# moxime/joint-vae

Measured on AMD Instinct MI355X. Metric: training_images_per_sec, higher is better.
Workload: dtype f32

## Files before the change

### include/jvae_hip.h

```cpp
#ifndef JVAE_HIP_H
#define JVAE_HIP_H

#include <stddef.h>

#ifdef __cplusplus
extern "C" {
#endif

const char* jvae_version(void);

int jvae_gemm_f32(int M, int N, int K, int batch,
                  const float* A, long sAm, long sAk, long sAb,
                  const float* B, long sBk, long sBn, long sBb,
                  float* C, long sCm, long sCn, long sCb,
                  const float* bias, int bias_mode, int flags, int splitk, void* stream);

int jvae_splitk_fold_f32(const float* part, const float* bias, float* y, int S, long MN, int N, int relu, int accumulate,
                         void* stream);

typedef struct JvaeGemmDesc {
    int M, N, K, batch;
    const float* A; long sAm, sAk, sAb;
    const float* B; long sBk, sBn, sBb;
    float* C; long sCm, sCn, sCb;
    const float* bias; int bias_mode, flags, splitk;
    int want_splits; long sCsplit; int* splits;
} JvaeGemmDesc;
int jvae_gemm_group_f32(const JvaeGemmDesc* descs, int n, void* stream);

typedef struct JvaeGemmRoute {
    int variant;
    int gx, gy, gz;
    int slices, kchunk;
    int vecA, vecB;
    int lds;
} JvaeGemmRoute;
int jvae_gemm_route(const JvaeGemmDesc* d, JvaeGemmRoute* out);
const char* jvae_gemm_variant_name(int variant);

typedef struct JvaeFoldDesc {
    const float* part; const float* bias; float* y;
    int S; long MN; int N, relu, accumulate;
} JvaeFoldDesc;
int jvae_splitk_fold_group_f32(const JvaeFoldDesc* descs, int n, void* stream);

size_t jvae_conv2d_workspace_bytes(int N, int Cin, int H, int W, int Cout, int KH, int KW, int S, int P, int OP,
                                   int transposed);
int jvae_conv2d_set_split_bf16(int mode);
int jvae_conv2d_set_split_shape16(int on);
int jvae_conv2d_out_shape(int H, int W, int KH, int KW, int S, int P, int OP, int transposed, int* OH, int* OW);
int jvae_conv2d_route(int dir, int layout, int bias, int stats, int y_f32, int aff_kind,
                      int N, int Cin, int H, int W, int Cout, int KH, int KW, int S, int P, int OP, int transposed,
                      int* kernel, int* swap, size_t* ws_bytes, int* splits, int* aff_ok);
const char* jvae_conv2d_kernel_name(int kernel);
int jvae_conv2d_fwd_f32(const float* x, const float* w, const float* bias, float* y,
                        int N, int Cin, int H, int W, int Cout, int KH, int KW, int S, int P, int OP, int transposed,
                        void* ws, size_t ws_bytes, void* stream);
int jvae_conv2d_stats_splits(int N, int Cin, int H, int W, int Cout, int KH, int KW, int S, int P, int OP, int transposed);
int jvae_conv2d_fwd_stats_f32(const float* x, const float* w, const float* bias, float* y, float* stats, int* nsplit,
                              int N, int Cin, int H, int W, int Cout, int KH, int KW, int S, int P, int OP, int transposed,
                              void* ws, size_t ws_bytes, void* stream);
int jvae_conv2d_dgrad_f32(const float* dy, const float* w, float* dx,
                          int N, int Cin, int H, int W, int Cout, int KH, int KW, int S, int P, int OP, int transposed,
                          void* ws, size_t ws_bytes, void* stream);
int jvae_conv2d_wgrad_f32(const float* x, const float* dy, float* dw, float* dbias, int accumulate,
                          int N, int Cin, int H, int W, int Cout, int KH, int KW, int S, int P, int OP, int transposed,
                          void* ws, size_t ws_bytes, void* stream);

int jvae_pack_cache_configure(void* buf, size_t bytes);
int jvae_pack_cache_begin(void* stream, long long owner, const void* const* weights, int n);
int jvae_pack_cache_end(void);
int jvae_pack_cache_pin(void);
int jvae_pack_cache_reset(void);
int jvae_pack_cache_stats(int* entries, long long* hits, long long* misses, long long* refreshes);

size_t jvae_channel_sum_workspace_bytes(int C);
int jvae_channel_sum_f32(const float* t, float* out, int N, int C, int P, int accumulate, void* ws, size_t ws_bytes,
                         void* stream);

size_t jvae_bn_workspace_bytes(int C);
int jvae_bn_plan(int N, int C, int P, int* nsplit, int* nchunk);
int jvae_image_range(int N, int parts, int j, int* nb, int* ne);
int jvae_bn_fwd_f32(const float* x, const float* gamma, const float* beta,
                    float* running_mean, float* running_var, long long* num_batches_tracked,
                    float* y, float* save_mean, float* save_invstd,
                    int N, int C, int P, float momentum, float eps, int training, int relu,
                    void* ws, size_t ws_bytes, void* stream);
int jvae_bn_fwd_ext_f32(const float* x, const float* gamma, const float* beta,
                        float* running_mean, float* running_var, long long* num_batches_tracked,
                        float* y, float* save_mean, float* save_invstd,
                        int N, int C, int P, float momentum, float eps, int training, int relu,
                        const float* ext_stats, int ext_nsplit, const float* ext_pivot,
                        void* ws, size_t ws_bytes, void* stream);
int jvae_bn_bwd_f32(const float* dy, const float* x, const float* gamma, const float* beta,
                    const float* save_mean, const float* save_invstd,
                    float* dx, float* dgamma, float* dbeta, int accumulate,
                    int N, int C, int P, int relu, void* ws, size_t ws_bytes, void* stream);
int jvae_bn_eval_bwd_f32(const float* dy, const float* x, const float* gamma, const float* beta,
                         const float* running_mean, const float* running_var, float* dx,
                         int N, int C, int P, float eps, int relu, void* stream);

int jvae_bn_finalize_f32(const float* x, const float* gamma, const float* beta,
                         float* running_mean, float* running_var, long long* num_batches_tracked,
                         float* save_mean, float* save_invstd, float* scale, float* shift,
                         int N, int C, int P, float momentum, float eps, int training,
                         const float* ext_stats, int ext_nsplit, const float* ext_pivot,
                         void* ws, size_t ws_bytes, void* stream);
int jvae_conv2d_affine_ok(int N, int Cin, int H, int W, int Cout, int KH, int KW, int S, int P, int OP, int transposed);
int jvae_conv2d_fwd_aff_f32(const float* x, const float* w, const float* bias, float* y, float* stats, int* nsplit,
                            const float* in_scale, const float* in_shift, int in_relu,
                            int N, int Cin, int H, int W, int Cout, int KH, int KW, int S, int P, int OP, int transposed,
                            void* ws, size_t ws_bytes, void* stream);
int jvae_conv2d_wgrad_aff_f32(const float* x, const float* dy, float* dw, float* dbias, int accumulate,
                              const float* in_scale, const float* in_shift, int in_relu,
                              int N, int Cin, int H, int W, int Cout, int KH, int KW, int S, int P, int OP, int transposed,
                              void* ws, size_t ws_bytes, void* stream);

int jvae_bn_sums_f32(const float* x, const float* pivot, float* sums, int N, int C, int P,
                     void* ws, size_t ws_bytes, void* stream);
int jvae_bn_fwd_sync_f32(const float* x, const float* gamma, const float* beta,
                         float* running_mean, float* running_var, long long* num_batches_tracked,
                         float* y, float* save_mean, float* save_invstd,
                         int N, int C, int P, float momentum, float eps, int relu,
                         const float* global_sums, const float* pivot, int world,
                         void* ws, size_t ws_bytes, void* stream);
int jvae_bn_bwd_sums_f32(const float* dy, const float* x, const float* gamma, const float* beta,
                         const float* save_mean, const float* save_invstd, float* local_sums,
                         int N, int C, int P, int relu, void* ws, size_t ws_bytes, void* stream);
int jvae_bn_bwd_sync_f32(const float* dy, const float* x, const float* gamma, const float* beta,
                         const float* save_mean, const float* save_invstd,
                         const float* local_sums, const float* global_sums, int world,
                         float* dx, float* dgamma, float* dbeta, int accumulate,
                         int N, int C, int P, int relu, void* stream);

int jvae_b8_pack_f32(const float* x, void* y, int N, int C, long HW, void* stream);
int jvae_b8_unpack_f32(const void* y, float* x, int N, int C, long HW, int accumulate, void* stream);
int jvae_conv2d_native_b8(int N, int Cin, int H, int W, int Cout, int KH, int KW, int S, int P, int OP, int transposed);
size_t jvae_conv2d_workspace_bytes_b8(int N, int Cin, int H, int W, int Cout, int KH, int KW, int S, int P, int OP,
                                      int transposed);
int jvae_conv2d_stats_splits_b8(int N, int Cin, int H, int W, int Cout, int KH, int KW, int S, int P, int OP, int transposed);
int jvae_conv2d_fwd_b8(const void* x, const float* w, const float* bias, void* y, int y_f32, float* stats, int* nsplit,
                       int N, int Cin, int H, int W, int Cout, int KH, int KW, int S, int P, int OP, int transposed,
                       void* ws, size_t ws_bytes, void* stream);
int jvae_conv2d_dgrad_b8(const void* dy, const float* w, void* dx,
                         int N, int Cin, int H, int W, int Cout, int KH, int KW, int S, int P, int OP, int transposed,
                         void* ws, size_t ws_bytes, void* stream);
int jvae_conv2d_wgrad_b8(const void* x, const void* dy, float* dw, float* dbias, int accumulate,
                         int N, int Cin, int H, int W, int Cout, int KH, int KW, int S, int P, int OP, int transposed,
                         void* ws, size_t ws_bytes, void* stream);
size_t jvae_bn_workspace_bytes_b8(int C);
int jvae_bn_plan_b8(int N, int C, long HW, int* nsplit, int* nchunk);
int jvae_bn_fwd_b8(const void* x, const float* gamma, const float* beta,
                   float* running_mean, float* running_var, long long* num_batches_tracked,
                   void* y, float* save_mean, float* save_invstd,
                   int N, int C, long HW, float momentum, float eps, int training, int relu,
                   const float* ext_stats, int ext_nsplit, const float* ext_pivot,
                   void* ws, size_t ws_bytes, void* stream);
int jvae_bn_bwd_b8(const void* dy, const void* x, const float* gamma, const float* beta,
                   const float* save_mean, const float* save_invstd,
                   void* dx, float* dgamma, float* dbeta, int accumulate,
                   int N, int C, long HW, int relu, void* ws, size_t ws_bytes, void* stream);
int jvae_bn_finalize_b8(const void* x, const float* gamma, const float* beta,
                        float* running_mean, float* running_var, long long* num_batches_tracked,
                        float* save_mean, float* save_invstd, float* coef,
                        int N, int C, long HW, float momentum, float eps, int training,
                        const float* ext_stats, int ext_nsplit, const float* ext_pivot,
                        void* ws, size_t ws_bytes, void* stream);
int jvae_bn_sums_b8(const void* x, const float* pivot, float* sums, int N, int C, long HW,
                    void* ws, size_t ws_bytes, void* stream);
int jvae_bn_fwd_sync_b8(const void* x, const float* gamma, const float* beta,
                        float* running_mean, float* running_var, long long* num_batches_tracked,
                        void* y, float* save_mean, float* save_invstd,
                        int N, int C, long HW, float momentum, float eps, int relu,
                        const float* global_sums, const float* pivot, int world,
                        void* ws, size_t ws_bytes, void* stream);
int jvae_bn_bwd_sums_b8(const void* dy, const void* x, const float* gamma, const float* beta,
                        const float* save_mean, const float* save_invstd, float* local_sums,
                        int N, int C, long HW, int relu, void* ws, size_t ws_bytes, void* stream);
int jvae_bn_bwd_sync_b8(const void* dy, const void* x, const float* gamma, const float* beta,
                        const float* save_mean, const float* save_invstd,
                        const float* local_sums, const float* global_sums, int world,
                        void* dx, float* dgamma, float* dbeta, int accumulate,
                        int N, int C, long HW, int relu, void* ws, size_t ws_bytes, void* stream);
int jvae_conv2d_affine_ok_b8(int N, int Cin, int H, int W, int Cout, int KH, int KW, int S, int P, int OP, int transposed);
int jvae_conv2d_fwd_aff_b8(const void* x, const float* w, const float* bias, void* y, int y_f32, float* stats, int* nsplit,
                           const float* in_scale, const float* in_shift, int in_relu,
                           int N, int Cin, int H, int W, int Cout, int KH, int KW, int S, int P, int OP, int transposed,
                           void* ws, size_t ws_bytes, void* stream);
int jvae_conv2d_wgrad_aff_b8(const void* x, const void* dy, float* dw, float* dbias, int accumulate,
                             const float* in_scale, const float* in_shift, int in_relu,
                             int N, int Cin, int H, int W, int Cout, int KH, int KW, int S, int P, int OP, int transposed,
                             void* ws, size_t ws_bytes, void* stream);
int jvae_relu_fwd_b8(const void* x, void* y, long units, void* stream);
int jvae_relu_bwd_b8(const void* dy, const void* y, void* dx, long units, void* stream);

int jvae_act_fwd_f32(const float* x, float* y, long n, int kind, void* stream);
int jvae_act_bwd_f32(const float* dy, const float* y, float* dx, long n, int kind, void* stream);

int jvae_dict_stats_f32(const float* means, float* dict, int C, int K, void* stream);
int jvae_latent_fwd_f32(const float* mu, const float* lv_raw, const float* eps, const long long* y,
                        const float* means, const float* T, const float* dict,
                        float* lv, float* z, float* kl, float* zdist, float* var_kl, float* dzdist,
                        int N, int K, int L, int C, int prior, int var_dim, float tau, float alpha, float w,
                        int sampled, int has_forced, float forced_lv, void* stream);
int jvae_latent_bwd_f32(const float* mu, const float* lv_raw, const float* lv, const float* eps, const long long* y,
                        const float* means, const float* T,
                        const float* gz, const float* g_kl, const float* g_zdist, const float* g_vkl,
                        const float* gmu_direct, const float* glv_direct,
                        float* gmu, float* glv_raw, float* gmeans, float* gT,
                        int N, int K, int L, int C, int prior, int var_dim, float tau, float alpha, float w,
                        int sampled, int has_forced, void* ws, size_t ws_bytes, void* stream);
int jvae_latent_fwd_wdev_f32(const float* mu, const float* lv_raw, const float* eps, const long long* y,
                             const float* means, const float* T, const float* dict,
                             float* lv, float* z, float* kl, float* zdist, float* var_kl, float* dzdist,
                             int N, int K, int L, int C, int prior, int var_dim, float tau, float alpha, float w,
                             int sampled, int has_forced, float forced_lv, const float* w_dev, void* stream);
int jvae_latent_bwd_wdev_f32(const float* mu, const float* lv_raw, const float* lv, const float* eps, const long long* y,
                             const float* means, const float* T,
                             const float* gz, const float* g_kl, const float* g_zdist, const float* g_vkl,
                             const float* gmu_direct, const float* glv_direct,
                             float* gmu, float* glv_raw, float* gmeans, float* gT,
                             int N, int K, int L, int C, int prior, int var_dim, float tau, float alpha, float w,
                             int sampled, int has_forced, const float* w_dev, void* ws, size_t ws_bytes, void* stream);
int jvae_latent_mixed_fwd_f32(const float* mu, const float* lv_raw, const float* eps, const long long* y,
                              const float* means_a, const float* T_a, const float* dict, const float* means_b, const float* T_b,
                              float* lv, float* z, float* kl, float* zdist, float* var_kl, float* dzdist,
                              int N, int K, int L, int split,
                              int C_a, int prior_a, int var_dim_a, float tau_a, float alpha_a,
                              int C_b, int prior_b, int var_dim_b, float tau_b, float alpha_b,
                              float w, int sampled, int has_forced, float forced_lv, void* stream);
int jvae_latent_mixed_bwd_f32(const float* mu, const float* lv_raw, const float* lv, const float* eps, const long long* y,
                              const float* means_a, const float* T_a, const float* means_b, const float* T_b,
                              const float* gz, const float* g_kl, const float* g_zdist, const float* g_vkl,
                              const float* gmu_direct, const float* glv_direct,
                              float* gmu, float* glv_raw, float* gmeans, float* gT,
                              int N, int K, int L, int split,
                              int C_a, int prior_a, int var_dim_a, float tau_a, float alpha_a,
                              int C_b, int prior_b, int var_dim_b, float tau_b, float alpha_b,
                              float w, int sampled, int has_forced, void* ws, size_t ws_bytes, void* stream);
int jvae_latent_refine_f32(float* mu, float* lv_raw, float* lv, const float* eps_cur, const float* eps_next,
                           const long long* y, const float* means, const float* T, const float* dz,
                           float* m_mu, float* v_mu, float* m_lv, float* v_lv,
                           float* z_next, float* kl, float* zdist, float* var_kl,
                           int N, int K, int L, int C, int prior, int var_dim, float tau, float alpha,
                           int sampled, int has_forced, float forced_lv, float lr, long step, int flags, void* stream);

int jvae_recon_fwd_f32(const float* x_reco, const float* x, const float* sigma, int sigma_is_log,
                       float* wmse, int L, int N, int D, void* stream);
int jvae_recon_bwd_f32(const float* x_reco, const float* x, const float* sigma, int sigma_is_log, const float* sigma_fwd,
                       const float* g_wmse, const float* wmse, float* g_x_reco, float* gsigma, int accumulate_sigma,
                       int L, int N, int D, void* ws, size_t ws_bytes, void* stream);

int jvae_mse_rows_fwd_f32(const float* rows, const float* x, float* wmse, int L, int N, int D, void* stream);
int jvae_mse_rows_bwd_f32(const float* rows, const float* x, const float* g_wmse, float* g_rows, int L, int N, int D, void* stream);

int jvae_elbo_fwd_f32(const float* wmse_s, const float* kl, const float* ce, const float* sigma, int sigma_is_log,
                      float* wmse, float* cross_x, float* total, float* mse, int L, int N, int D, float beta, float cw,
                      void* stream);
int jvae_elbo_bwd_f32(const float* g_wmse, const float* g_cx, const float* g_tot, const float* sigma, int sigma_is_log,
                      float* g_wmse_s, float* g_kl, float* g_ce, float* gsigma, int accumulate_sigma,
                      int L, int N, int D, float beta, float cw, void* ws, size_t ws_bytes, void* stream);
int jvae_elbo_fwd_wdev_f32(const float* wmse_s, const float* kl, const float* ce, const float* sigma, int sigma_is_log,
                           float* wmse, float* cross_x, float* total, float* mse, int L, int N, int D, float beta, float cw,
                           const float* cw_dev, void* stream);
int jvae_elbo_bwd_wdev_f32(const float* g_wmse, const float* g_cx, const float* g_tot, const float* sigma, int sigma_is_log,
                           float* g_wmse_s, float* g_kl, float* g_ce, float* gsigma, int accumulate_sigma,
                           int L, int N, int D, float beta, float cw, const float* cw_dev, void* ws, size_t ws_bytes,
                           void* stream);

int jvae_dropout_f32(const float* x, float* y, long n, float p, long seed, void* stream);
int jvae_dropout_dev_f32(const float* x, float* y, long n, float p, const long long* seed_dev, long salt, void* stream);

int jvae_iws_f32(const float* wmse_s, const float* eps, const float* log_var, const float* log_pz, const float* sigma,
                 int sigma_is_log, int L, int N, int K, int C, int D, float* rows, float* iws, void* stream);

int jvae_measures_f32(const float* sumsq_x, long nx, const float* wmse, const float* zdist, const float* var_kl, int N, int Nz,
                      const float* sigma, int sigma_is_log, const float* means, int C, int K, const int* flag,
                      const float* prev, int batch, float* out, void* stream);
int jvae_measures_dev_f32(const float* sumsq_x, long nx, const float* wmse, const float* zdist, const float* var_kl, int N, int Nz,
                          const float* sigma, int sigma_is_log, const float* means, int C, int K, const int* flag,
                          float* run, int* counter, void* stream);

int jvae_loss_sums_f32(const float* const* rows, const long* lens, int nrows, float* acc, void* stream);

int jvae_xent_fwd_f32(const float* logits, const long long* y, float* ce, int R, int N, int C, void* stream);
int jvae_xent_bwd_f32(const float* logits, const long long* y, const float* g_ce, float* g_logits, int R, int N, int C,
                      void* stream);

size_t jvae_sqnorm_workspace_bytes(void);
int jvae_sqnorm_accum_f32(const float* g, long n, float* acc, int reset, void* ws, size_t ws_bytes, void* stream);
int jvae_clip_scale_f32(float* g, long n, const float* sqnorm, float max_norm, void* stream);
int jvae_adam_step_f32(float* p, const float* g, float* m, float* v, long n,
                       float lr, float beta1, float beta2, float eps, float weight_decay, long step,
                       float max_norm, const float* sqnorm, int* nonfinite_flag, void* stream);
int jvae_adam_step_dev_f32(float* p, const float* g, float* m, float* v, long n, float* hyper, int advance,
                           float eps, float weight_decay, float max_norm, const float* sqnorm, int* nonfinite_flag,
                           void* stream);

int jvae_sgd_step_f32(float* p, const float* g, float* buf, long n, float lr, float momentum, int nesterov,
                      float weight_decay, int first_step, float max_norm, const float* sqnorm, int* nonfinite_flag,
                      void* stream);

int jvae_pool2d_out_shape(int H, int W, int K, int S, int P, int* OH, int* OW);
int jvae_pool2d_fwd_f32(const float* x, float* y, int* idx, long planes, int H, int W, int K, int S, int P, int mode,
                        void* stream);
int jvae_pool2d_bwd_f32(const float* dy, const int* idx, float* dx, long planes, int H, int W, int K, int S, int P,
                        int mode, void* stream);
int jvae_upsample_nearest_fwd_f32(const float* x, float* y, long planes, int H, int W, int scale, void* stream);
int jvae_upsample_nearest_bwd_f32(const float* dy, float* dx, long planes, int H, int W, int scale, void* stream);
int jvae_pool2d_fwd_b8(const void* x, void* y, int* idx, long blocks, int H, int W, int K, int S, int P, int mode, void* stream);
int jvae_pool2d_bwd_b8(const void* dy, const int* idx, void* dx, long blocks, int H, int W, int K, int S, int P, int mode,
                       void* stream);
int jvae_upsample_nearest_fwd_b8(const void* x, void* y, long blocks, int H, int W, int scale, void* stream);
int jvae_upsample_nearest_bwd_b8(const void* dy, void* dx, long blocks, int H, int W, int scale, void* stream);

int jvae_augment_u8_f32(const unsigned char* in, const unsigned char* flip, const int* dy, const int* dx,
                        float* out, int N, int C, int H, int W, int pad, int nhwc, void* stream);

int jvae_imageset_desc_words(void);
int jvae_imageset_batch_u8_f32(const unsigned char* data, const long long* idx, const long long* targets, const long long* lut,
                               const int* desc, const int* coef_h, const int* bounds_h, const int* coef_v, const int* bounds_v,
                               const unsigned char* flip, const int* dy, const int* dx, float* x, long long* y, long n, int N,
                               void* stream);

int jvae_imageset_mix_leaf_bytes(void);
int jvae_imageset_mixed_u8_f32(const void* leaves_host, const void* leaves_dev, int n_leaves, const int* leaf,
                               const long long* index, const long long* tag, const long long* pos, const float* u, int u_dims,
                               float* x, long long* tagout, long long* y, int N, int vec, void* stream);

size_t jvae_roc_workspace_bytes(int M, long n_in, long n_out);
int jvae_roc_curve_f32(const float* ins, const float* outs, const double* kept_tpr, const int* two_sided,
                       double* auc, double* kept_fpr, double* kept_tpr_out, double* thr_low, double* thr_up, int* status,
                       int M, long n_in, long n_out, int K, void* ws, size_t ws_bytes, void* stream);

size_t jvae_pr_workspace_bytes(int M, long n_in, long n_out);
int jvae_pr_metrics_f32(const float* ins, const float* outs, const int* modes, double* figures, int* status,
                        int M, long n_in, long n_out, void* ws, size_t ws_bytes, void* stream);

int jvae_scod_scores_f32(const float* const* r_src, const float* const* r_aux, const float* const* g_src,
                         const float* const* g_alt, const int* kinds, const float* weights, const long long* y_est,
                         float* out, long out_stride, int M, int C, long N, int* status, void* stream);
size_t jvae_scod_workspace_bytes(int M, long n);
int jvae_scod_curve_f32(const float* scores, const long long* y_true, const long long* y_est, float* curves, double* figures,
                        int* status, int M, long n, long n_in, void* ws, size_t ws_bytes, void* stream);

int jvae_misclass_scores_f32(const float* src, const int* kinds, const float* temps, const int* rows, float* out,
                             int R, int C, long N, long out_stride, void* stream);
size_t jvae_misclass_split_workspace_bytes(long N);
int jvae_misclass_split_f32(const float* scores, const unsigned char* mask, float* out, int* n_correct, int M, long N,
                            void* ws, size_t ws_bytes, void* stream);
int jvae_misclass_confusion_f32(const float* scores, const unsigned char* mask, const double* thr, int* tp, int* fp,
                                int M, long N, int K, void* stream);

int jvae_odin_head_f32(const float* logits, const float* temps, float* scores, float* dlogits,
                       int F, int L, int N, int C, long stride_f, long stride_l, void* stream);
int jvae_odin_perturb_f32(float* acc, const float* g, const float* x, const float* eps, float* out, long numel, int E,
                          void* stream);

int jvae_wim_scores_f32(const float* const* srcs, const float* const* alts, const float* factors, int S, const long long* y_est,
                        const int* specs, int R, float* out, long out_stride, int C, long N, int* status, void* stream);
int jvae_group_tally_f32(const float* values, const int* group, double* sums, long long* counts, int R, int N, int G,
                         void* stream);

int jvae_prior_sample_f32(const float* eps, const long long* y, const float* means, const float* T, float* z, int* status,
                          long R, int K, int C, float t, int mode, void* stream);
int jvae_image_grid_f32(const float* x_in, const float* x_out, const int* specs, const int* specs_host, int Ncol, float* grid_f32,
                        unsigned char* grid_u8, int N, int D, int H, int W, int Rr, void* stream);

int jvae_class_posterior_f32(const float* z, const float* means, const float* T, const float* log_det, const float* temps, int nT,
                             float* logp, float* P, long R, int K, int C, int var_dim, void* stream);
size_t jvae_latent_mi_workspace_bytes(int nT, int L0, long N);
int jvae_latent_mi_f32(const float* P0, const float* P1, float* Im, int nT, int C, int L0, int L1, long N, void* ws, size_t ws_bytes,
                       void* stream);
int jvae_aggregate_scores_f32(const void* const* srcs, const float* factors, int E, int mode, const float* temps, int nT, float* post,
                              float* a, float* amax, long long* argmax, int slot, int C, long N, int* status, void* stream);

size_t jvae_cascade_mse_workspace_bytes(int M, long N, long D);
int jvae_cascade_mse_f32(const float* x, const void* const* stages, int M, float* mse, int L, long N, long D, void* ws,
                         size_t ws_bytes, void* stream);
// ... 98 lines not shown
```

### joint-vae_amd/csrc/conv_api.hip

```cpp
#include "common.h"
#include "jvae_internal.h"
#include "conv_dispatch.h"

namespace {

inline ConvRoute route(const ConvGeom& g, int transposed, ConvDir dir, CallFlags f = {}) {
    return jvae_conv_route(g, transposed, dir, CONV_F32, f);
}

bool affine_ok(const ConvGeom& g, int transposed, ConvDir other, const ConvRoute& r) {
    return r.aff_ok && route(g, transposed, other, {false, false, false, 1}).aff_ok;
}

int fwd_f32(const float* x, const float* w, const float* bias, float* y, float* stats, int* nsplit, const InAff* aff,
            int N, int Cin, int H, int W, int Cout, int KH, int KW, int S, int P, int OP, int transposed,
            void* ws, size_t ws_bytes, void* stream) {
    ConvGeom g; int oh, ow;
    if (nsplit) *nsplit = 0;
    if (!jvae_make_geom(N, Cin, H, W, Cout, KH, KW, S, P, OP, transposed, &g, &oh, &ow)) return JVAE_EINVAL;
    const ConvRoute r = route(g, transposed, CONV_FWD, {bias != nullptr, stats != nullptr, false, jvae_aff_kind(aff)});
    if (aff && !affine_ok(g, transposed, CONV_WGRAD, r)) return JVAE_ENOTSUP;
    if (N == 0) return 0;
    if (jvae_ws_short(r, ws, ws_bytes)) return JVAE_EWORKSPACE;
    return jvae_conv_run_fwd(r, g, x, w, bias, y, (float*)ws, ws_bytes, (hipStream_t)stream, stats, nsplit, aff);
}

int wgrad_f32(const float* x, const float* dy, float* dw, float* dbias, int accumulate, const InAff* aff,
              int N, int Cin, int H, int W, int Cout, int KH, int KW, int S, int P, int OP, int transposed,
              void* ws, size_t ws_bytes, void* stream) {
    ConvGeom g; int oh, ow;
    if (!dw || (N > 0 && (!x || !dy))) return JVAE_EINVAL;
    if (!jvae_make_geom(N, Cin, H, W, Cout, KH, KW, S, P, OP, transposed, &g, &oh, &ow)) return JVAE_EINVAL;
    const ConvRoute r = route(g, transposed, CONV_WGRAD, {false, false, false, jvae_aff_kind(aff)});
    if (aff && !affine_ok(g, transposed, CONV_FWD, r)) return JVAE_ENOTSUP;
    if (N > 0 && jvae_ws_short(r, ws, ws_bytes)) return JVAE_EWORKSPACE;
    hipStream_t st = (hipStream_t)stream;
    if (!accumulate) {
        hipError_t e = hipMemsetAsync(dw, 0, sizeof(float) * (size_t)Cin * Cout * KH * KW, st);
        if (e != hipSuccess) return (int)e;
    }
    if (N == 0) {
        if (dbias && !accumulate) {
            hipError_t e = hipMemsetAsync(dbias, 0, sizeof(float) * (size_t)Cout, st);
            if (e != hipSuccess) return (int)e;
        }
        return 0;
    }
    int rc = jvae_conv_run_wgrad(r, g, transposed, x, dy, dw, (float*)ws, ws_bytes, st, aff);
    if (rc) return rc;
    if (dbias) rc = jvae_channel_sum(dy, dbias, N, Cout, oh * ow, accumulate, (float*)ws, ws_bytes, st);
    return rc;
}

}

extern "C" {

int jvae_conv2d_set_split_bf16(int mode) { return jvae_conv5_x3_set(mode); }
int jvae_conv2d_set_split_shape16(int on) { return jvae_conv5_x3_set_shape16(on); }

size_t jvae_conv2d_workspace_bytes(int N, int Cin, int H, int W, int Cout, int KH, int KW, int S, int P, int OP,
                                   int transposed) {
    ConvGeom g; int oh, ow;
    if (!jvae_make_geom(N, Cin, H, W, Cout, KH, KW, S, P, OP, transposed, &g, &oh, &ow)) return 0;
    return jvae_conv_ws(g, transposed);
}

int jvae_conv2d_route(int dir, int layout, int bias, int stats, int y_f32, int aff_kind,
                      int N, int Cin, int H, int W, int Cout, int KH, int KW, int S, int P, int OP, int transposed,
                      int* kernel, int* swap, size_t* ws_bytes, int* splits, int* aff_ok) {
    ConvGeom g; int oh, ow;
    if (dir != CONV_FWD && dir != CONV_DGRAD && dir != CONV_WGRAD) return JVAE_EINVAL;
    if ((layout != CONV_F32 && layout != CONV_B8) || aff_kind < 0 || aff_kind > 2) return JVAE_EINVAL;
    if (!jvae_make_geom(N, Cin, H, W, Cout, KH, KW, S, P, OP, transposed, &g, &oh, &ow)) return JVAE_EINVAL;
    const ConvRoute r = jvae_conv_route(g, transposed, (ConvDir)dir, (ConvLayout)layout,
                                        {bias != 0, stats != 0, y_f32 != 0, aff_kind});
    if (kernel) *kernel = (int)r.k;
    if (swap) *swap = r.swap ? 1 : 0;
    if (ws_bytes) *ws_bytes = r.ws;
    if (splits) *splits = r.splits;
    if (aff_ok) *aff_ok = r.aff_ok ? 1 : 0;
    return 0;
}

const char* jvae_conv2d_kernel_name(int kernel) {
    switch (kernel) {
#define JVAE_CK_NAME(k) case k: return #k;
        JVAE_CK_NAME(CK_NONE) JVAE_CK_NAME(CK_GENERIC) JVAE_CK_NAME(CK_POINT) JVAE_CK_NAME(CK_SMALLCO)
        JVAE_CK_NAME(CK_SMALLCI) JVAE_CK_NAME(CK_FWD5) JVAE_CK_NAME(CK_FWD5_X3) JVAE_CK_NAME(CK_T2) JVAE_CK_NAME(CK_T2_X3)
        JVAE_CK_NAME(CK_WG5) JVAE_CK_NAME(CK_WG5_X3) JVAE_CK_NAME(CK_B8) JVAE_CK_NAME(CK_T2_B8) JVAE_CK_NAME(CK_WG_B8)
        JVAE_CK_NAME(CK_WG_B8X) JVAE_CK_NAME(CK_SMALLCO_DG)
#undef JVAE_CK_NAME
        default: return nullptr;
    }
}

int jvae_conv2d_out_shape(int H, int W, int KH, int KW, int S, int P, int OP, int transposed, int* OH, int* OW) {
    ConvGeom g;
    if (!OH || !OW) return JVAE_EINVAL;
    return jvae_make_geom(1, 1, H, W, 1, KH, KW, S, P, OP, transposed, &g, OH, OW) ? 0 : JVAE_EINVAL;
}

int jvae_conv2d_fwd_f32(const float* x, const float* w, const float* bias, float* y,
                        int N, int Cin, int H, int W, int Cout, int KH, int KW, int S, int P, int OP, int transposed,
                        void* ws, size_t ws_bytes, void* stream) {
    if (!w || (N > 0 && (!x || !y))) return JVAE_EINVAL;
    return fwd_f32(x, w, bias, y, nullptr, nullptr, nullptr, N, Cin, H, W, Cout, KH, KW, S, P, OP, transposed, ws, ws_bytes,
                   stream);
}

int jvae_conv2d_stats_splits(int N, int Cin, int H, int W, int Cout, int KH, int KW, int S, int P, int OP, int transposed) {
    ConvGeom g; int oh, ow;
    if (!jvae_make_geom(N, Cin, H, W, Cout, KH, KW, S, P, OP, transposed, &g, &oh, &ow)) return 0;
    return route(g, transposed, CONV_FWD, {false, true, false, 0}).splits;
}

int jvae_conv2d_fwd_stats_f32(const float* x, const float* w, const float* bias, float* y, float* stats, int* nsplit,
                              int N, int Cin, int H, int W, int Cout, int KH, int KW, int S, int P, int OP, int transposed,
                              void* ws, size_t ws_bytes, void* stream) {
    if (!w || !nsplit || (N > 0 && (!x || !y))) return JVAE_EINVAL;
    return fwd_f32(x, w, bias, y, stats, nsplit, nullptr, N, Cin, H, W, Cout, KH, KW, S, P, OP, transposed, ws, ws_bytes, stream);
}

int jvae_conv2d_affine_ok(int N, int Cin, int H, int W, int Cout, int KH, int KW, int S, int P, int OP, int transposed) {
    ConvGeom g; int oh, ow;
    if (!jvae_make_geom(N, Cin, H, W, Cout, KH, KW, S, P, OP, transposed, &g, &oh, &ow)) return 0;
    return affine_ok(g, transposed, CONV_WGRAD, route(g, transposed, CONV_FWD, {false, false, false, 1})) ? 1 : 0;
}

int jvae_conv2d_fwd_aff_f32(const float* x, const float* w, const float* bias, float* y, float* stats, int* nsplit,
                            const float* in_scale, const float* in_shift, int in_relu,
                            int N, int Cin, int H, int W, int Cout, int KH, int KW, int S, int P, int OP, int transposed,
                            void* ws, size_t ws_bytes, void* stream) {
    if (!w || !in_scale || !in_shift || (N > 0 && (!x || !y))) return JVAE_EINVAL;
    if (stats && !nsplit) return JVAE_EINVAL;
    const InAff aff{in_scale, in_shift, in_relu};
    return fwd_f32(x, w, bias, y, stats, nsplit, &aff, N, Cin, H, W, Cout, KH, KW, S, P, OP, transposed, ws, ws_bytes, stream);
}

int jvae_conv2d_wgrad_aff_f32(const float* x, const float* dy, float* dw, float* dbias, int accumulate,
                              const float* in_scale, const float* in_shift, int in_relu,
                              int N, int Cin, int H, int W, int Cout, int KH, int KW, int S, int P, int OP, int transposed,
                              void* ws, size_t ws_bytes, void* stream) {
    if (!in_scale || !in_shift) return JVAE_EINVAL;
    const InAff aff{in_scale, in_shift, in_relu};
    return wgrad_f32(x, dy, dw, dbias, accumulate, &aff, N, Cin, H, W, Cout, KH, KW, S, P, OP, transposed, ws, ws_bytes, stream);
}

int jvae_conv2d_dgrad_f32(const float* dy, const float* w, float* dx,
                          int N, int Cin, int H, int W, int Cout, int KH, int KW, int S, int P, int OP, int transposed,
                          void* ws, size_t ws_bytes, void* stream) {
    ConvGeom g; int oh, ow;
    if (!w || (N > 0 && (!dy || !dx))) return JVAE_EINVAL;
    if (!jvae_make_geom(N, Cin, H, W, Cout, KH, KW, S, P, OP, transposed, &g, &oh, &ow)) return JVAE_EINVAL;
    if (N == 0) return 0;
    const ConvRoute r = route(g, transposed, CONV_DGRAD);
    if (jvae_ws_short(r, ws, ws_bytes)) return JVAE_EWORKSPACE;
    return jvae_conv_run_fwd(r, g, dy, w, nullptr, dx, (float*)ws, ws_bytes, (hipStream_t)stream);
}

int jvae_conv2d_wgrad_f32(const float* x, const float* dy, float* dw, float* dbias, int accumulate,
                          int N, int Cin, int H, int W, int Cout, int KH, int KW, int S, int P, int OP, int transposed,
                          void* ws, size_t ws_bytes, void* stream) {
    return wgrad_f32(x, dy, dw, dbias, accumulate, nullptr, N, Cin, H, W, Cout, KH, KW, S, P, OP, transposed, ws, ws_bytes, stream);
}

size_t jvae_channel_sum_workspace_bytes(int C) { return jvae_channel_sum_ws_bytes(C); }

int jvae_channel_sum_f32(const float* t, float* out, int N, int C, int P, int accumulate, void* ws, size_t ws_bytes,
                         void* stream) {
    if (!t || !out || N < 0 || C <= 0 || P <= 0) return JVAE_EINVAL;
    return jvae_channel_sum(t, out, N, C, P, accumulate, (float*)ws, ws_bytes, (hipStream_t)stream);
}

}
```

### joint-vae_amd/csrc/conv_dispatch.h

```cpp
#pragma once
#include "common.h"
#include "jvae_internal.h"

size_t jvae_conv_generic_ws(const ConvGeom& g);
int jvae_fold_fwd(const ConvGeom& g, const float* xb, const float* w, const float* bias, float* ys,
                  float* ws, size_t ws_bytes, hipStream_t st);
int jvae_fold_bwd(const ConvGeom& g, const float* ys, const float* w, const float* bias, float* xb,
                  float* ws, size_t ws_bytes, hipStream_t st);
int jvae_fold_wgrad(const ConvGeom& g, const float* xb, const float* ys, float* dw,
                    float* ws, size_t ws_bytes, hipStream_t st);
size_t jvae_channel_sum_ws_bytes(int C);
int jvae_channel_sum(const float* t, float* out, int N, int C, int P, int accumulate, float* ws, size_t ws_bytes,
                     hipStream_t st);

bool jvae_conv5_fwd_ok(int Cin, int H, int W, int Cout, int OH, int OW, int S, int P);
size_t jvae_conv5_pack_floats(int Cin, int Cout);
int jvae_conv5_fwd(const float* in, const float* w, int swap, int flip, const float* bias, float* out,
                   int N, int Cin, int H, int W, int Cout, int OW, int S, int P, float* ws, hipStream_t st,
                   float* stats = nullptr, int* nsplit = nullptr, const InAff* aff = nullptr);
int jvae_conv5_fwd_max_splits(int N, int OW);

int jvae_conv5_pack(const float* w, float* wp, int C, int O, int swap, int flip, hipStream_t st);

bool jvae_conv5_x3_ok(int Cin, int H, int W, int Cout, int OH, int OW, int S, int P);
size_t jvae_conv5_x3_pack_bytes(int Cin, int Cout);
int jvae_conv5_x3_set(int mode);
int jvae_conv5_x3_set_shape16(int on);
bool jvae_conv5_x3_enabled();
int jvae_conv5_x3_wpack(const float* w, float* ws, int C, int O, int swap, int flip, hipStream_t st);
bool jvae_convt2_x3_ok(int N, int C, int WS, int O);
int jvae_convt2_x3(const float* in, const float* w, const float* bias, float* out, int N, int C, int WS, int O, float* ws,
                   hipStream_t st, float* stats = nullptr, int* nsplit = nullptr, const InAff* aff = nullptr);
int jvae_conv5_x3_fwd(const float* in, const float* w, int swap, int flip, const float* bias, float* out,
                      int N, int Cin, int H, int W, int Cout, int OW, int S, int P, float* ws, hipStream_t st,
                      float* stats = nullptr, int* nsplit = nullptr, const InAff* aff = nullptr);

bool jvae_convt2_ok(int C, int HS, int WS, int O, int HB, int WB, int KH, int KW, int S, int P);
int jvae_convt2(const float* in, const float* wpacked, const float* bias, float* out, int N, int C, int WS, int O,
                hipStream_t st, float* stats = nullptr, int* nsplit = nullptr, const InAff* aff = nullptr);

bool jvae_conv5_smallco_ok(int Cin, int H, int W, int Cout, int KH, int KW, int S, int P);
int jvae_conv5_smallco(const float* in, const float* w, const float* bias, float* out, int N, int Cin, int W, int Cout,
                       hipStream_t st, const InAff* aff = nullptr);
int jvae_conv5_smallco_dgrad(const float* dy, const float* w, float* dx, int N, int Cy, int W, int Cx, hipStream_t st);

bool jvae_conv5_smallci_ok(int Cin, int H, int W, int Cout, int OW, int S, int P, bool dgrad_role);
int jvae_conv5_smallci(const float* in, const float* w, int swap, int flip, const float* bias, float* out,
                       int N, int Cin, int W, int Cout, float* ws, hipStream_t st, float* stats = nullptr, int* nsplit = nullptr);

bool jvae_conv5_wgrad_ok(int Ca, int HS, int WS, int Cb, int HB, int WB, int S, int P);
size_t jvae_conv5_wgrad_ws_floats(int N, int Ca, int Cb, int S, int WS);
int jvae_conv5_wgrad(const float* ps, const float* q, float* dw, int accumulate, int swapflip,
                     int N, int Ca, int WS, int Cb, int S, int P, float* ws, hipStream_t st,
                     const InAff* aff_p = nullptr, const InAff* aff_q = nullptr);

bool jvae_conv5_wgrad_x3_ok(int Ca, int HS, int WS, int Cb, int HB, int WB, int S, int P);
size_t jvae_conv5_wgrad_x3_ws_floats(int N, int Ca, int Cb, int S);
int jvae_conv5_wgrad_x3(const float* ps, const float* q, float* dw, int accumulate, int swapflip,
                        int N, int Ca, int WS, int Cb, int S, int P, float* ws, hipStream_t st,
                        const InAff* aff_p = nullptr, const InAff* aff_q = nullptr);

bool jvae_make_geom(int N, int Cin, int H, int W, int Cout, int KH, int KW, int S, int P, int OP, int transposed,
                    ConvGeom* g, int* OH, int* OW);

enum ConvDir { CONV_FWD = 1, CONV_DGRAD = 2, CONV_WGRAD = 4 };
enum ConvLayout { CONV_F32, CONV_B8 };
enum ConvKernel {
    CK_NONE,
    CK_GENERIC, CK_POINT,
    CK_SMALLCO, CK_SMALLCI, CK_FWD5, CK_FWD5_X3, CK_T2, CK_T2_X3, CK_WG5, CK_WG5_X3,
    CK_B8, CK_T2_B8, CK_WG_B8, CK_WG_B8X,
    CK_SMALLCO_DG,
};
struct CallFlags {
    bool bias, stats;
    bool y_f32;
    int aff;
};
struct ConvRoute {
    ConvKernel k;
    bool swap;
    int S, P;
    size_t ws;
    int splits;
    bool aff_ok;
};
ConvRoute jvae_conv_route(const ConvGeom& g, int transposed, ConvDir dir, ConvLayout layout, CallFlags f);
inline int jvae_aff_kind(const InAff* aff) { return !aff ? 0 : (aff->relu == JVAE_ACT_LEAKY ? 2 : 1); }
inline bool jvae_ws_short(const ConvRoute& r, const void* ws, size_t ws_bytes) { return r.ws && (!ws || ws_bytes < r.ws); }
template <class T>
inline void jvae_wgrad_operands(const ConvRoute& r, int transposed, T* x, T* dy, const InAff* aff, T** ps, T** q,
                                const InAff** aff_p, const InAff** aff_q) {
    const bool p_is_x = r.swap != (transposed != 0);
    *ps = p_is_x ? x : dy;
    *q = p_is_x ? dy : x;
    *aff_p = p_is_x ? aff : nullptr;
    *aff_q = p_is_x ? nullptr : aff;
}

size_t jvae_conv_ws(const ConvGeom& g, int transposed);
int jvae_conv_run_fwd(const ConvRoute& r, const ConvGeom& g, const float* in, const float* w, const float* bias, float* out,
                      float* ws, size_t ws_bytes, hipStream_t st, float* stats = nullptr, int* nsplit = nullptr,
                      const InAff* aff = nullptr);
int jvae_conv_run_wgrad(const ConvRoute& r, const ConvGeom& g, int transposed, const float* x, const float* dy, float* dw,
                        float* ws, size_t ws_bytes, hipStream_t st, const InAff* aff = nullptr);
```

### joint-vae_amd/csrc/conv_generic.hip

```cpp
#include "common.h"
#include "jvae_internal.h"

namespace {

__global__ __launch_bounds__(256) void unfold_kernel(const float* __restrict__ xb, float* __restrict__ col,
                                                     ConvGeom g, int n0, int nimg, long sn, long sk, long sq,
                                                     int kfast) {
    const int Kd = g.Cb * g.KH * g.KW, Ps = g.Hs * g.Ws;
    const long total = (long)nimg * Kd * Ps;
    for (long i = (long)blockIdx.x * blockDim.x + threadIdx.x; i < total; i += (long)gridDim.x * blockDim.x) {
        int n, k, q;
        if (kfast) { k = (int)(i % Kd); long r = i / Kd; n = (int)(r % nimg); q = (int)(r / nimg); }
        else       { q = (int)(i % Ps); long r = i / Ps; k = (int)(r % Kd);  n = (int)(r / Kd); }
        const int kw = k % g.KW, kh = (k / g.KW) % g.KH, cb = k / (g.KW * g.KH);
        const int hs = q / g.Ws, ws = q % g.Ws;
        const int hb = hs * g.S + kh - g.P, wb = ws * g.S + kw - g.P;
        float v = 0.f;
        if (hb >= 0 && hb < g.Hb && wb >= 0 && wb < g.Wb)
            v = xb[(((long)(n0 + n) * g.Cb + cb) * g.Hb + hb) * g.Wb + wb];
        col[(long)n * sn + (long)k * sk + (long)q * sq] = v;
    }
}

template <bool KFAST>
__global__ __launch_bounds__(256) void unfold4_kernel(const float* __restrict__ xb, float* __restrict__ col,
                                                      ConvGeom g, int n0, int nimg) {
    const unsigned Kd = g.Cb * g.KH * g.KW, Ps = g.Hs * g.Ws, KK = g.KH * g.KW;
    const unsigned inner4 = (KFAST ? Kd : Ps) / 4;
    const unsigned total = (KFAST ? Ps * (unsigned)nimg : (unsigned)nimg * Kd) * inner4;
    for (unsigned i = blockIdx.x * blockDim.x + threadIdx.x; i < total; i += gridDim.x * blockDim.x) {
        const unsigned row = i / inner4, e4 = (i - row * inner4) * 4;
        unsigned n, k, q;
        if (KFAST) { q = row / nimg; n = row - q * nimg; k = e4; }
        else       { n = row / Kd;   k = row - n * Kd;   q = e4; }
        unsigned cb = k / KK, t = k - cb * KK;
        unsigned kh = t / g.KW, kw = t - kh * g.KW;
        const unsigned hs = q / g.Ws, ws = q - hs * g.Ws;
        const float* src = xb + (long)(n0 + n) * g.Cb * g.Hb * g.Wb;
        f32x4 v;
#pragma unroll
        for (int e = 0; e < 4; ++e) {
            const int hb = (int)(hs * g.S + kh) - g.P;
            const int wb = (int)((KFAST ? ws : ws + e) * g.S + kw) - g.P;
            v[e] = (hb >= 0 && hb < g.Hb && wb >= 0 && wb < g.Wb) ? src[((long)cb * g.Hb + hb) * g.Wb + wb] : 0.f;
            if (KFAST && ++kw == (unsigned)g.KW) { kw = 0; if (++kh == (unsigned)g.KH) { kh = 0; ++cb; } }
        }
        *reinterpret_cast<f32x4*>(col + (long)i * 4) = v;
    }
}

__global__ __launch_bounds__(256) void fold_kernel(const float* __restrict__ col, float* __restrict__ xb,
                                                   const float* __restrict__ bias, ConvGeom g, int n0, int nimg,
                                                   long sn, long sk, long sq) {
    const unsigned total = (unsigned)nimg * g.Cb * g.Hb * g.Wb;
    for (unsigned i = blockIdx.x * blockDim.x + threadIdx.x; i < total; i += gridDim.x * blockDim.x) {
        unsigned r = i / (unsigned)g.Wb;
        const int wb = (int)(i - r * g.Wb);
        unsigned r2 = r / (unsigned)g.Hb;
        const int hb = (int)(r - r2 * g.Hb);
        const int n = (int)(r2 / (unsigned)g.Cb);
        const int cb = (int)(r2 - (unsigned)n * g.Cb);
        float acc = bias ? bias[cb] : 0.f;
        if (g.Hs * g.Ws < g.KH * g.KW) {
            for (int hs = 0; hs < g.Hs; ++hs) {
                const int kh = hb + g.P - hs * g.S;
                if (kh < 0 || kh >= g.KH) continue;
                for (int ws = 0; ws < g.Ws; ++ws) {
                    const int kw = wb + g.P - ws * g.S;
                    if (kw < 0 || kw >= g.KW) continue;
                    const int k = (cb * g.KH + kh) * g.KW + kw;
                    acc += col[(long)n * sn + (long)k * sk + (long)(hs * g.Ws + ws) * sq];
                }
            }
            xb[(((long)(n0 + n) * g.Cb + cb) * g.Hb + hb) * g.Wb + wb] = acc;
            continue;
        }
        for (int kh = 0; kh < g.KH; ++kh) {
            const int th = hb + g.P - kh;
            if (th < 0 || th % g.S) continue;
            const int hs = th / g.S;
            if (hs >= g.Hs) continue;
            for (int kw = 0; kw < g.KW; ++kw) {
                const int tw = wb + g.P - kw;
                if (tw < 0 || tw % g.S) continue;
                const int ws = tw / g.S;
                if (ws >= g.Ws) continue;
                const int k = (cb * g.KH + kh) * g.KW + kw;
                acc += col[(long)n * sn + (long)k * sk + (long)(hs * g.Ws + ws) * sq];
            }
        }
        xb[(((long)(n0 + n) * g.Cb + cb) * g.Hb + hb) * g.Wb + wb] = acc;
    }
}

__global__ __launch_bounds__(256) void channel_sum_kernel(const float* __restrict__ t, float* __restrict__ partial,
                                                          int N, int C, int P, int nsplit) {
    __shared__ float red[17];
    const int c = blockIdx.x, sp = blockIdx.y;
    const ImageRange ir = image_range(N, nsplit, sp);
    const int nb = ir.nb, ne = ir.ne;
    float s = 0.f;
    if ((P & 3) == 0) {
        const int P4 = P >> 2;
        const long cnt = (long)(ne - nb) * P4;
        for (long i = threadIdx.x; i < cnt; i += blockDim.x) {
            const long n = nb + i / P4, q = i % P4;
            const f32x4 v = *reinterpret_cast<const f32x4*>(t + (n * C + c) * (long)P + q * 4);
            s += (v[0] + v[1]) + (v[2] + v[3]);
        }
    } else {
        const long cnt = (long)(ne - nb) * P;
        for (long i = threadIdx.x; i < cnt; i += blockDim.x) {
            const long n = nb + i / P, q = i % P;
            s += t[(n * C + c) * (long)P + q];
        }
    }
    s = block_sum(s, red);
    if (threadIdx.x == 0) partial[(long)c * nsplit + sp] = s;
}

__global__ void channel_fold_kernel(const float* __restrict__ partial, float* __restrict__ out, int C, int nsplit,
                                    int accumulate) {
    const int c = blockIdx.x * blockDim.x + threadIdx.x;
    if (c >= C) return;
    float s = 0.f;
    for (int k = 0; k < nsplit; ++k) s += partial[(long)c * nsplit + k];
    out[c] = (accumulate ? out[c] : 0.f) + s;
}

inline int fold_slab_images(const ConvGeom& g) {
    const long per = (long)g.Cb * g.Hb * g.Wb;
    long n = ((1L << 31) - 1) / (per > 0 ? per : 1);
    if (const char* e = getenv("JVAE_FOLD_SLAB")) { const long v = atol(e); if (v > 0 && v < n) n = v; }
    return (int)(n < 1 ? 1 : (n > g.N ? (g.N > 0 ? g.N : 1) : n));
}

inline int grid_for(long total) {
    long b = (total + 255) / 256;
    return (int)(b > 8192 ? 8192 : (b < 1 ? 1 : b));
}

inline int grid_for4(long total4) {
    long b = (total4 + 255) / 256;
    return (int)(b > 16384 ? 16384 : (b < 1 ? 1 : b));
}

int launch_unfold(const float* xb, float* col, const ConvGeom& g, int n0, int nimg, bool kfast, hipStream_t st) {
    const long Kd = (long)g.Cb * g.KH * g.KW, Ps = (long)g.Hs * g.Ws, total = (long)nimg * Kd * Ps;
    const bool vec = total < (1L << 31) && (kfast ? Kd % 4 == 0 : g.Ws % 4 == 0) && ((uintptr_t)col & 15) == 0;
    if (vec && kfast)
        hipLaunchKernelGGL(unfold4_kernel<true>, dim3(grid_for4(total / 4)), dim3(256), 0, st, xb, col, g, n0, nimg);
    else if (vec)
        hipLaunchKernelGGL(unfold4_kernel<false>, dim3(grid_for4(total / 4)), dim3(256), 0, st, xb, col, g, n0, nimg);
    else if (kfast)
        hipLaunchKernelGGL(unfold_kernel, dim3(grid_for(total)), dim3(256), 0, st, xb, col, g, n0, nimg, Kd, 1L, (long)nimg * Kd, 1);
    else
        hipLaunchKernelGGL(unfold_kernel, dim3(grid_for(total)), dim3(256), 0, st, xb, col, g, n0, nimg, Kd * Ps, Ps, 1L, 0);
    JVAE_LAUNCH_CHECK();
    return 0;
}

inline bool pixel_batched(const ConvGeom& g) { return g.Hs * g.Ws <= 48; }

inline bool wgrad_joint(const ConvGeom& g) { return pixel_batched(g) && g.Hs * g.Ws > 1; }
inline int wgrad_slices(const ConvGeom& g) {
    const long Kd = (long)g.Cb * g.KH * g.KW, K = (long)g.Hs * g.Ws * g.N;
    const long tiles = (long)cdiv(g.Cs, 64) * cdiv(Kd, 64);
    for (int S = 16; S > 1; S >>= 1)
        if (tiles * S <= 2048 && K % S == 0 && K / S >= 256) return S;
    return 1;
}

inline int fwd_slices(const ConvGeom& g) {
    if (!pixel_batched(g)) return 1;
    const long Kd = (long)g.Cb * g.KH * g.KW;
    const long tiles = (long)cdiv(g.N, 64) * cdiv(g.Cs, 64) * g.Hs * g.Ws;
    if (tiles < 1 || tiles >= 512 || Kd < 1024) return 1;
    int s = (int)(1024 / tiles);
    return s > 8 ? 8 : (s < 1 ? 1 : s);
}

__global__ __launch_bounds__(256) void small_transpose_kernel(const float* __restrict__ ys, float* __restrict__ yt,
                                                              int N, int Cs, int Ps) {
    const long total = (long)N * Cs * Ps;
    for (long i = (long)blockIdx.x * blockDim.x + threadIdx.x; i < total; i += (long)gridDim.x * blockDim.x) {
        const int cs = (int)(i % Cs);
        const long r = i / Cs;
        const int n = (int)(r % N), q = (int)(r / N);
        yt[i] = ys[((long)n * Cs + cs) * Ps + q];
    }
}

inline long col_floats_per_image(const ConvGeom& g) { return (long)g.Cb * g.KH * g.KW * g.Hs * g.Ws; }

inline long wgrad_part_floats(const ConvGeom& g) { return (long)g.Cs * g.Cb * g.KH * g.KW; }

}

size_t jvae_conv_generic_ws(const ConvGeom& g) {
    const long per = (col_floats_per_image(g) + (pixel_batched(g) ? 0 : wgrad_part_floats(g))) * 4;
    long imgs = (1L << 30) / (per > 0 ? per : 1);
    if (imgs < 1) imgs = 1;
    if (imgs > g.N) imgs = g.N;
    if (pixel_batched(g)) imgs = g.N;
    size_t bytes = (size_t)(imgs * per);
    size_t extra = 0;
    if (wgrad_joint(g))
        extra = 4 * ((size_t)g.N * g.Cs * g.Hs * g.Ws + (size_t)wgrad_slices(g) * g.Cs * g.Cb * g.KH * g.KW);
    const size_t fwd_extra = fwd_slices(g) > 1 ? 4 * (size_t)fwd_slices(g) * g.N * g.Cs * g.Hs * g.Ws : 0;
    return bytes + (extra > fwd_extra ? extra : fwd_extra);
}

static int chunk_images(const ConvGeom& g, size_t ws_bytes) {
    const long per = col_floats_per_image(g) * 4;
    long imgs = (long)(ws_bytes / (size_t)(per > 0 ? per : 1));
    if (imgs > g.N) imgs = g.N;
    return (int)imgs;
}

int jvae_fold_fwd(const ConvGeom& g, const float* xb, const float* w, const float* bias, float* ys,
                  float* ws, size_t ws_bytes, hipStream_t st) {
    const int Kd = g.Cb * g.KH * g.KW, Ps = g.Hs * g.Ws;
    if (pixel_batched(g)) {
        if (ws_bytes < (size_t)col_floats_per_image(g) * 4 * g.N) return JVAE_EWORKSPACE;
        { const int rc = launch_unfold(xb, ws, g, 0, g.N, true, st); if (rc) return rc; }
        const int want = fwd_slices(g);
        if (want > 1) {
            const long colf = (long)col_floats_per_image(g) * g.N, outf = (long)g.N * g.Cs * Ps;
            if (ws_bytes < 4 * (size_t)(colf + want * outf)) return JVAE_EWORKSPACE;
            float* part = ws + colf;
            int S = 0;
            int rc = jvae_gemm_launch_part(g.N, g.Cs, Kd, Ps, ws, Kd, 1, (long)g.N * Kd, w, 1, Kd, 0,
                                           part, g.Cs, 1, (long)g.N * g.Cs, outf, want, &S, st);
            if (rc) return rc;
            return jvae_splitk_fold_qn(part, bias, ys, S, g.N, g.Cs, Ps, st);
        }
        return jvae_gemm_launch(g.N, g.Cs, Kd, Ps, ws, Kd, 1, (long)g.N * Kd, w, 1, Kd, 0,
                                ys, (long)g.Cs * Ps, Ps, 1, bias, bias ? 1 : 0, 0, 1, st);
    }
    const int chunk = chunk_images(g, ws_bytes);
    if (chunk < 1) return JVAE_EWORKSPACE;
    for (int n0 = 0; n0 < g.N; n0 += chunk) {
        const int ni = (g.N - n0 < chunk) ? g.N - n0 : chunk;
        { const int rc = launch_unfold(xb, ws, g, n0, ni, false, st); if (rc) return rc; }
        int rc = jvae_gemm_launch(g.Cs, Ps, Kd, ni, w, Kd, 1, 0, ws, Ps, 1, (long)Kd * Ps,
                                  ys + (long)n0 * g.Cs * Ps, Ps, 1, (long)g.Cs * Ps, bias, bias ? 2 : 0, 0, 1, st);
        if (rc) return rc;
    }
    return 0;
}

int jvae_fold_bwd(const ConvGeom& g, const float* ys, const float* w, const float* bias, float* xb,
                  float* ws, size_t ws_bytes, hipStream_t st) {
    const int Kd = g.Cb * g.KH * g.KW, Ps = g.Hs * g.Ws;
    if (pixel_batched(g)) {
        if (ws_bytes < (size_t)col_floats_per_image(g) * 4 * g.N) return JVAE_EWORKSPACE;
        const long colf = (long)col_floats_per_image(g) * g.N, ytf = (long)g.N * g.Cs * Ps;
        int rc;
        if (Ps > 1 && ws_bytes >= 4 * (size_t)(colf + ytf)) {
            float* yt = ws + colf;
            hipLaunchKernelGGL(small_transpose_kernel, dim3(grid_for(ytf)), dim3(256), 0, st, ys, yt, g.N, g.Cs, Ps);
            JVAE_LAUNCH_CHECK();
            rc = jvae_gemm_launch(g.N, Kd, g.Cs, Ps, yt, g.Cs, 1, (long)g.N * g.Cs, w, Kd, 1, 0,
                                  ws, Kd, 1, (long)g.N * Kd, nullptr, 0, 0, 1, st);
        } else {
            rc = jvae_gemm_launch(g.N, Kd, g.Cs, Ps, ys, (long)g.Cs * Ps, Ps, 1, w, Kd, 1, 0,
                                  ws, Kd, 1, (long)g.N * Kd, nullptr, 0, 0, 1, st);
        }
        if (rc) return rc;
        const int slab = fold_slab_images(g);
        for (int n0 = 0; n0 < g.N; n0 += slab) {
            const int ni = (g.N - n0 < slab) ? g.N - n0 : slab;
            hipLaunchKernelGGL(fold_kernel, dim3(grid_for((long)ni * g.Cb * g.Hb * g.Wb)), dim3(256), 0, st,
                               ws + (long)n0 * Kd, xb, bias, g, n0, ni, (long)Kd, 1L, (long)g.N * Kd);
            JVAE_LAUNCH_CHECK();
        }
        return 0;
    }
    const int chunk = chunk_images(g, ws_bytes);
    if (chunk < 1) return JVAE_EWORKSPACE;
    for (int n0 = 0; n0 < g.N; n0 += chunk) {
        const int ni = (g.N - n0 < chunk) ? g.N - n0 : chunk;
        int rc = jvae_gemm_launch(Kd, Ps, g.Cs, ni, w, 1, Kd, 0, ys + (long)n0 * g.Cs * Ps, Ps, 1, (long)g.Cs * Ps,
                                  ws, Ps, 1, (long)Kd * Ps, nullptr, 0, 0, 1, st);
        if (rc) return rc;
        const int slab = fold_slab_images(g);
        for (int m0 = 0; m0 < ni; m0 += slab) {
            const int mi = (ni - m0 < slab) ? ni - m0 : slab;
            hipLaunchKernelGGL(fold_kernel, dim3(grid_for((long)mi * g.Cb * g.Hb * g.Wb)), dim3(256), 0, st,
                               ws + (long)m0 * Kd * Ps, xb, bias, g, n0 + m0, mi, (long)Kd * Ps, (long)Ps, 1L);
            JVAE_LAUNCH_CHECK();
        }
    }
    return 0;
}

int jvae_fold_wgrad(const ConvGeom& g, const float* xb, const float* ys, float* dw,
                    float* ws, size_t ws_bytes, hipStream_t st) {
    const int Kd = g.Cb * g.KH * g.KW, Ps = g.Hs * g.Ws;
    if (pixel_batched(g)) {
        if (ws_bytes < (size_t)col_floats_per_image(g) * 4 * g.N) return JVAE_EWORKSPACE;
        { const int rc = launch_unfold(xb, ws, g, 0, g.N, true, st); if (rc) return rc; }
        if (wgrad_joint(g)) {
            const int S = wgrad_slices(g);
            const long colf = (long)col_floats_per_image(g) * g.N, ytf = (long)g.N * g.Cs * Ps;
            if (ws_bytes < 4 * (size_t)(colf + ytf + (long)S * g.Cs * Kd)) return JVAE_EWORKSPACE;
            float* yt = ws + colf;
            float* part = yt + ytf;
            hipLaunchKernelGGL(small_transpose_kernel, dim3(grid_for(ytf)), dim3(256), 0, st, ys, yt, g.N, g.Cs, Ps);
            JVAE_LAUNCH_CHECK();
            const long Ks = (long)Ps * g.N / S;
            int rc = jvae_gemm_launch(g.Cs, Kd, (int)Ks, S, yt, 1, g.Cs, Ks * g.Cs, ws, Kd, 1, Ks * Kd,
                                      part, Kd, 1, (long)g.Cs * Kd, nullptr, 0, 0, 1, st);
            if (rc) return rc;
            return jvae_splitk_fold(part, nullptr, dw, S, (long)g.Cs * Kd, Kd, 0, 1, st);
        }
        for (int q = 0; q < Ps; ++q) {
            int rc = jvae_gemm_launch(g.Cs, Kd, g.N, 1, ys + q, Ps, (long)g.Cs * Ps, 0, ws + (long)q * g.N * Kd, Kd, 1, 0,
                                      dw, Kd, 1, 0, nullptr, 0, 1, 1, st);
            if (rc) return rc;
        }
        return 0;
    }
    const long colf = col_floats_per_image(g), partf = wgrad_part_floats(g);
    long chunk = (long)(ws_bytes / (size_t)(4 * (colf + partf)));
    if (chunk > g.N) chunk = g.N;
    if (chunk < 1) {
        if (chunk_images(g, ws_bytes) < 1) return JVAE_EWORKSPACE;
        chunk = 1;
    }
    float* part = ws + chunk * colf;
    for (int n0 = 0; n0 < g.N; n0 += (int)chunk) {
        const int ni = (g.N - n0 < chunk) ? g.N - n0 : (int)chunk;
        { const int rc = launch_unfold(xb, ws, g, n0, ni, false, st); if (rc) return rc; }
        const float* a = ys + (long)n0 * g.Cs * Ps;
        if (ni == 1) {
            const int rc = jvae_gemm_launch(g.Cs, Kd, Ps, 1, a, Ps, 1, 0, ws, 1, Ps, 0, dw, Kd, 1, 0, nullptr, 0, 1, 1, st);
            if (rc) return rc;
            continue;
        }
        int rc = jvae_gemm_launch(g.Cs, Kd, Ps, ni, a, Ps, 1, (long)g.Cs * Ps, ws, 1, Ps, (long)Kd * Ps,
                                  part, Kd, 1, partf, nullptr, 0, 0, 1, st);
        if (rc) return rc;
        rc = jvae_splitk_fold(part, nullptr, dw, ni, partf, Kd, 0, 1, st);
        if (rc) return rc;
    }
    return 0;
}

size_t jvae_channel_sum_ws_bytes(int C) { return sizeof(float) * (size_t)(C > 0 ? C : 1) * 64; }

int jvae_channel_sum(const float* t, float* out, int N, int C, int P, int accumulate, float* ws, size_t ws_bytes,
                     hipStream_t st) {
    if (C <= 0) return 0;
    if (N <= 0) {
        if (!accumulate) {
            hipError_t e = hipMemsetAsync(out, 0, sizeof(float) * (size_t)C, st);
            if (e != hipSuccess) return (int)e;
        }
        return 0;
    }
    if (!ws || ws_bytes < jvae_channel_sum_ws_bytes(C)) return JVAE_EWORKSPACE;
    long work = (long)N * P;
    int ns = (int)(work / 4096);
    const int cap = (1024 + C - 1) / C;
    if (ns > cap) ns = cap;
    if (ns > 64) ns = 64;
    if (ns > N) ns = N;
    if (ns < 1) ns = 1;
    hipLaunchKernelGGL(channel_sum_kernel, dim3(C, ns), dim3(256), 0, st, t, ws, N, C, P, ns);
    JVAE_LAUNCH_CHECK();
    hipLaunchKernelGGL(channel_fold_kernel, dim3(cdiv(C, 64)), dim3(64), 0, st, (const float*)ws, out, C, ns, accumulate);
    JVAE_LAUNCH_CHECK();
    return 0;
}
```

### joint-vae_amd/csrc/gemm.hip

```cpp
#include <stdio.h>
#include <stdlib.h>
#include <utility>
#include "common.h"
#include "jvae_hip.h"
#include "conv_x3.h"
#include "jvae_internal.h"
#include "conv_dispatch.h"

namespace {

constexpr int BK = 32;

struct GemmP {
    const float* A; long sAm, sAk, sAb;
    const float* B; long sBk, sBn, sBb;
    float* C; long sCm, sCn, sCb;
    const float* bias;
    int bias_mode;
    int bias_div;
    int M, N, K;
    int splitk;
    int kchunk;
    int flags;
    long sCsplit;
    int vecA, vecB;
    int xcd;
};

struct TileCtx {
    int m0, n0;
    int batch, split, kbeg, kend;
    const float* A; const float* B; float* C;
    __device__ __forceinline__ TileCtx(const GemmP& p, int BM, int BN, unsigned bx, unsigned by, unsigned bz)
        : m0(by * BM), n0(bx * BN), batch(bz / p.splitk), split(bz % p.splitk), kbeg(split * p.kchunk),
          kend(min(p.K, kbeg + p.kchunk)), A(p.A + (long)batch * p.sAb), B(p.B + (long)batch * p.sBb),
          C(p.C + (long)batch * p.sCb + ((p.flags & 8) ? (long)split * p.sCsplit : 0L)) {}
};

__device__ __forceinline__ void gemm_store(const GemmP& p, float* dst, float v) {
    if (p.flags & 8) {
        *dst = v;
    } else if (p.flags & 4) {
        atomicAdd(dst, v);
    } else {
        if (p.flags & 1) v += *dst;
        if (p.flags & 2) v = fmaxf(v, 0.f);
        *dst = v;
    }
}

template <bool VEC>
__device__ __forceinline__ f32x4 load4(const float* p, long stride, int i0, int lim, bool row_ok) {
    f32x4 v = {0.f, 0.f, 0.f, 0.f};
    if (!row_ok) return v;
    if (VEC) {
        if (i0 + 3 < lim) return *reinterpret_cast<const f32x4*>(p);
    }
#pragma unroll
    for (int j = 0; j < 4; ++j)
        if (i0 + j < lim) v[j] = p[j * stride];
    return v;
}

template <bool KC, int ROWS>
struct StageMap {
    static constexpr int Q = (KC ? BK : ROWS) / 4;
    static constexpr int G = ROWS * BK / 4 / 256;
    int fq, sl;
    __device__ __forceinline__ StageMap(int tid, int g) : fq(tid % Q), sl(tid / Q + g * (256 / Q)) {}
    __device__ __forceinline__ int row(int r0) const { return KC ? r0 + sl : r0 + fq * 4; }
    __device__ __forceinline__ int k(int k0) const { return KC ? k0 + fq * 4 : k0 + sl; }
};

template <bool KC, int ROWS, bool KFIRST>
__device__ __forceinline__ f32x4 stage_load(const float* base, long sR, long sK, int rows, int vec, int tid, int g, int r0, int k0, int kend) {
    const StageMap<KC, ROWS> s(tid, g);
    const int row = s.row(r0), k = s.k(k0);
    const float* src = KFIRST ? base + (long)k * sK + (long)row * sR : base + (long)row * sR + (long)k * sK;
    if (KC) return vec ? load4<true>(src, sK, k, kend, row < rows) : load4<false>(src, sK, k, kend, row < rows);
    return vec ? load4<true>(src, sR, row, rows, k < kend) : load4<false>(src, sR, row, rows, k < kend);
}

template <int BM, int BN>
struct TileLds {
    static constexpr int LDA = BM + 4, LDB = BN + 4;
    static constexpr int BYTES = BK * (LDA + LDB) * (int)sizeof(float);
};

template <bool KC, int ROWS, int LD>
__device__ __forceinline__ void tile_lstore(float* img, int tid, int g, const f32x4& v) {
    const StageMap<KC, ROWS> s(tid, g);
    if (KC) {
#pragma unroll
        for (int j = 0; j < 4; ++j) img[(s.fq * 4 + j) * LD + s.sl] = v[j];
    } else {
        *reinterpret_cast<f32x4*>(&img[s.sl * LD + s.fq * 4]) = v;
    }
}

template <int BM, int BN, bool AK, bool BNC>
__device__ __forceinline__ void gemm_tile_body(const GemmP& p, float* __restrict__ lds, unsigned bx, unsigned by, unsigned bz,
                                               unsigned gx, unsigned gy, unsigned gz) {
    constexpr int LDA = TileLds<BM, BN>::LDA, LDB = TileLds<BM, BN>::LDB;
    constexpr int WM = BM / 2, WN = BN / 2;
    constexpr int TM = WM / 32, TN = WN / 32;
    constexpr int GA = StageMap<AK, BM>::G, GB = StageMap<!BNC, BN>::G;
    float* As = lds;
    float* Bs = lds + BK * LDA;
    (void)gx; (void)gy; (void)gz;

    const int tid = threadIdx.x, lane = tid & 63, wave = tid >> 6;
    const int wm0 = (wave >> 1) * WM, wn0 = (wave & 1) * WN;
    const TileCtx t(p, BM, BN, bx, by, bz);
    const int m0 = t.m0, n0 = t.n0, kbeg = t.kbeg, kend = t.kend;
    const float* A = t.A; const float* B = t.B; float* C = t.C;

    f32x16 acc[TM][TN];
#pragma unroll
    for (int i = 0; i < TM; ++i)
#pragma unroll
        for (int j = 0; j < TN; ++j)
#pragma unroll
            for (int r = 0; r < 16; ++r) acc[i][j][r] = 0.f;

    f32x4 ra[GA], rb[GB];

    auto gload = [&](int k0) {
#pragma unroll
        for (int g = 0; g < GA; ++g) ra[g] = stage_load<AK, BM, false>(A, p.sAm, p.sAk, p.M, p.vecA, tid, g, m0, k0, kend);
#pragma unroll
        for (int g = 0; g < GB; ++g) rb[g] = stage_load<!BNC, BN, true>(B, p.sBn, p.sBk, p.N, p.vecB, tid, g, n0, k0, kend);
    };
    auto lstore = [&]() {
#pragma unroll
        for (int g = 0; g < GA; ++g) tile_lstore<AK, BM, LDA>(As, tid, g, ra[g]);
#pragma unroll
        for (int g = 0; g < GB; ++g) tile_lstore<!BNC, BN, LDB>(Bs, tid, g, rb[g]);
    };

    const int half = lane >> 5, l31 = lane & 31;
    if (kbeg < kend) gload(kbeg);
    for (int k0 = kbeg; k0 < kend; k0 += BK) {
        __syncthreads();
        lstore();
        __syncthreads();
        if (k0 + BK < kend) gload(k0 + BK);
#pragma unroll
        for (int kk = 0; kk < BK / 2; ++kk) {
            float a[TM], b[TN];
#pragma unroll
            for (int i = 0; i < TM; ++i) a[i] = As[(2 * kk + half) * LDA + wm0 + i * 32 + l31];
#pragma unroll
            for (int j = 0; j < TN; ++j) b[j] = Bs[(2 * kk + half) * LDB + wn0 + j * 32 + l31];
#pragma unroll
            for (int i = 0; i < TM; ++i)
#pragma unroll
                for (int j = 0; j < TN; ++j)
                    acc[i][j] = __builtin_amdgcn_mfma_f32_32x32x2f32(a[i], b[j], acc[i][j], 0, 0, 0);
        }
    }

    const bool lead = (t.split == 0) && !(p.flags & 8);
#pragma unroll
    for (int i = 0; i < TM; ++i)
#pragma unroll
        for (int j = 0; j < TN; ++j) {
            const int n = n0 + wn0 + j * 32 + l31;
            if (n >= p.N) continue;
            float bn = (p.bias_mode == 1 && lead) ? p.bias[n / p.bias_div] : 0.f;
#pragma unroll
            for (int r = 0; r < 16; ++r) {
                const int m = m0 + wm0 + i * 32 + (r & 3) + 8 * (r >> 2) + 4 * half;
                if (m >= p.M) continue;
                float v = acc[i][j][r] + bn;
                if (p.bias_mode == 2 && lead) v += p.bias[m];
                gemm_store(p, C + (long)m * p.sCm + (long)n * p.sCn, v);
            }
        }
}

template <int BM, int BN, bool AK, bool BNC>
__global__ __launch_bounds__(256) void gemm_kernel(GemmP p) {
    __shared__ float lds[TileLds<BM, BN>::BYTES / sizeof(float)];
    gemm_tile_body<BM, BN, AK, BNC>(p, lds, blockIdx.x, blockIdx.y, blockIdx.z, gridDim.x, gridDim.y, gridDim.z);
}

inline bool aligned16(const void* p) { return (reinterpret_cast<uintptr_t>(p) & 15) == 0; }

typedef __bf16 gx_bf16x8 __attribute__((ext_vector_type(8)));
typedef __bf16 gx_bf16x4 __attribute__((ext_vector_type(4)));
typedef unsigned int gx_u32x2 __attribute__((ext_vector_type(2)));
typedef unsigned int gx_u32x4 __attribute__((ext_vector_type(4)));
typedef __attribute__((address_space(3))) gx_bf16x4 gx_lds_bf16x4;
__device__ __forceinline__ void gx_split4(const f32x4& v, gx_u32x2 (&out)[3]) {
#pragma unroll
    for (int j = 0; j < 2; ++j) {
        unsigned h, m, l;
        x3_split2(x3_f32x2{v[2 * j], v[2 * j + 1]}, h, m, l);
        out[0][j] = h; out[1][j] = m; out[2][j] = l;
    }
}

template <bool KC>
struct GxImg {
    static constexpr int PITCH = KC ? (BK * 2 + 16) : (64 * 2 + 64);
    static constexpr int ROWS = KC ? 64 : BK;
    static constexpr int BYTES = PITCH * ROWS;
};

template <bool AK, bool BNC, int DEPTH>
__device__ __forceinline__ void gemm_x3_body(const GemmP& p, unsigned char* __restrict__ gx_lds, unsigned bx, unsigned by, unsigned bz,
                                             unsigned gx, unsigned gy, unsigned gz) {
    using IA = GxImg<AK>;
    using IB = GxImg<!BNC>;
    constexpr int BM = 64, BN = 64, G4 = StageMap<AK, BM>::G;
    unsigned char* As = gx_lds;
    unsigned char* Bs = gx_lds + 3 * IA::BYTES;

    const int tid = threadIdx.x, lane = tid & 63, wave = tid >> 6;
    const int half = lane >> 5, l31 = lane & 31;
    const int cg = (lane >> 4) & 1, q4 = (lane & 15) >> 2, pp = lane & 3;
    const int wm0 = (wave >> 1) * 32, wn0 = (wave & 1) * 32;
    if (p.xcd) {
        const unsigned lin = (unsigned)xcd_tile(bx + gx * (by + gy * bz), gx * gy * gz);
        bx = lin % gx; by = (lin / gx) % gy; bz = lin / (gx * gy);
    }
    const TileCtx t(p, BM, BN, bx, by, bz);
    const int m0 = t.m0, n0 = t.n0, kbeg = t.kbeg, kend = t.kend;
    const float* A = t.A; const float* B = t.B; float* C = t.C;

    f32x16 acc;
#pragma unroll
    for (int r = 0; r < 16; ++r) acc[r] = 0.f;
    f32x4 ra[DEPTH][G4], rb[DEPTH][G4];

    constexpr int QK = StageMap<true, 64>::Q, QR = StageMap<false, 64>::Q;
    auto coordA = [&](int g, int k0, int* fast, int* slow) {
        if (AK) { *fast = k0 + (tid % QK) * 4; *slow = m0 + tid / QK + g * (256 / QK); }
        else    { *fast = m0 + (tid % QR) * 4; *slow = k0 + tid / QR + g * (256 / QR); }
    };
    auto coordB = [&](int g, int k0, int* fast, int* slow) {
        if (BNC) { *fast = n0 + (tid % QR) * 4; *slow = k0 + tid / QR + g * (256 / QR); }
        else     { *fast = k0 + (tid % QK) * 4; *slow = n0 + tid / QK + g * (256 / QK); }
    };
    auto okA = [&](int fast, int slow) { return AK ? (fast < kend && slow < p.M) : (fast + 3 < p.M && slow < kend); };
    auto okB = [&](int fast, int slow) { return BNC ? (fast + 3 < p.N && slow < kend) : (fast < kend && slow < p.N); };

    auto gload = [&](int st, int k0) {
#pragma unroll
        for (int g = 0; g < G4; ++g) {
            if constexpr (DEPTH > 1) {
                int f, sl;
                coordA(g, k0, &f, &sl);
                const float* sa = AK ? A + (long)sl * p.sAm + f : A + (long)sl * p.sAk + f;
                ra[st][g] = *reinterpret_cast<const f32x4*>(okA(f, sl) ? sa : A);
                coordB(g, k0, &f, &sl);
                const float* sb = BNC ? B + (long)sl * p.sBk + f : B + (long)sl * p.sBn + f;
                rb[st][g] = *reinterpret_cast<const f32x4*>(okB(f, sl) ? sb : B);
                continue;
            }
            ra[st][g] = stage_load<AK, BM, false>(A, p.sAm, p.sAk, p.M, p.vecA, tid, g, m0, k0, kend);
            rb[st][g] = stage_load<!BNC, BN, true>(B, p.sBn, p.sBk, p.N, p.vecB, tid, g, n0, k0, kend);
        }
    };
    auto lstore = [&](int st, int k0) {
#pragma unroll
        for (int g = 0; g < G4; ++g) {
            const StageMap<AK, BM> ma(tid, g);
            const StageMap<!BNC, BN> mb(tid, g);
            f32x4 va = ra[st][g], vb = rb[st][g];
            if constexpr (DEPTH > 1) {
                int f, sl;
                coordA(g, k0, &f, &sl);
                if (!okA(f, sl)) va = f32x4{0.f, 0.f, 0.f, 0.f};
                coordB(g, k0, &f, &sl);
                if (!okB(f, sl)) vb = f32x4{0.f, 0.f, 0.f, 0.f};
            }
            gx_u32x2 sa[3], sb[3];
            gx_split4(va, sa);
            gx_split4(vb, sb);
#pragma unroll
            for (int pl = 0; pl < 3; ++pl) {
                *reinterpret_cast<gx_u32x2*>(As + pl * IA::BYTES + ma.sl * IA::PITCH + ma.fq * 8) = sa[pl];
                *reinterpret_cast<gx_u32x2*>(Bs + pl * IB::BYTES + mb.sl * IB::PITCH + mb.fq * 8) = sb[pl];
            }
        }
    };
    auto frag = [&](const unsigned char* img, bool kc, int pitch, int r0, int ks) -> gx_bf16x8 {
        if (kc)
            return __builtin_bit_cast(gx_bf16x8, *reinterpret_cast<const gx_u32x4*>(img + (r0 + l31) * pitch + (ks * 16 + half * 8) * 2));
        const unsigned char* q = img + (ks * 16 + half * 8 + q4) * pitch + (r0 + cg * 16 + pp * 4) * 2;
        const gx_bf16x4 lo = __builtin_amdgcn_ds_read_tr16_b64_v4bf16((gx_lds_bf16x4*)q);
        const gx_bf16x4 hi = __builtin_amdgcn_ds_read_tr16_b64_v4bf16((gx_lds_bf16x4*)(q + 4 * pitch));
        return __builtin_shufflevector(lo, hi, 0, 1, 2, 3, 4, 5, 6, 7);
    };

    auto multiply = [&]() {
#pragma unroll
        for (int ks = 0; ks < BK / 16; ++ks) {
            gx_bf16x8 a[3], b[3];
#pragma unroll
            for (int pl = 0; pl < 3; ++pl) {
                a[pl] = frag(As + pl * IA::BYTES, AK, IA::PITCH, wm0, ks);
                b[pl] = frag(Bs + pl * IB::BYTES, !BNC, IB::PITCH, wn0, ks);
            }
            constexpr int APL[6] = {0, 2, 1, 0, 1, 0}, BPL[6] = {2, 0, 1, 1, 0, 0};
#pragma unroll
            for (int t = 0; t < 6; ++t) acc = __builtin_amdgcn_mfma_f32_32x32x16_bf16(a[APL[t]], b[BPL[t]], acc, 0, 0, 0);
        }
    };
    if constexpr (DEPTH > 1) {
#pragma unroll
        for (int d = 0; d < DEPTH; ++d) gload(d, kbeg + d * BK);
        const int nst = (kend - kbeg + BK - 1) / BK;
        int k0 = kbeg;
        for (int it = 0; it < nst / DEPTH; ++it, k0 += DEPTH * BK) {
#pragma unroll
            for (int d = 0; d < DEPTH; ++d) {
                const int kk = k0 + d * BK;
                __syncthreads();
                lstore(d, kk);
                __syncthreads();
                gload(d, kk + DEPTH * BK);
                multiply();
            }
        }
#pragma unroll
        for (int d = 0; d < DEPTH - 1; ++d) {
            const int kk = k0 + d * BK;
            if (kk < kend) {
                __syncthreads();
                lstore(d, kk);
                __syncthreads();
                multiply();
            }
        }
    } else {
        if (kbeg < kend) gload(0, kbeg);
        for (int k0 = kbeg; k0 < kend; k0 += BK) {
            __syncthreads();
            lstore(0, k0);
            __syncthreads();
            if (k0 + BK < kend) gload(0, k0 + BK);
            multiply();
        }
    }

    const bool lead = (t.split == 0) && !(p.flags & 8);
    const int n = n0 + wn0 + l31;
    if (n >= p.N) return;
    const float bn = (p.bias_mode == 1 && lead) ? p.bias[n / p.bias_div] : 0.f;
#pragma unroll
    for (int r = 0; r < 16; ++r) {
        const int m = m0 + wm0 + (r & 3) + 8 * (r >> 2) + 4 * half;
        if (m >= p.M) continue;
        float v = acc[r] + bn;
        if (p.bias_mode == 2 && lead) v += p.bias[m];
        gemm_store(p, C + (long)m * p.sCm + (long)n * p.sCn, v);
    }
}

template <bool AK, bool BNC, int DEPTH = 1>
__global__ __launch_bounds__(256, 4) void gemm_x3_kernel(GemmP p) {
    extern __shared__ __attribute__((aligned(16))) unsigned char gx_lds[];
    gemm_x3_body<AK, BNC, DEPTH>(p, gx_lds, blockIdx.x, blockIdx.y, blockIdx.z, gridDim.x, gridDim.y, gridDim.z);
}

inline bool gemm_x3_on(int K) {
    return K >= 64 && jvae_conv5_x3_enabled();
}

struct Variant {
    bool x3; int bm; bool ak, bnc; int depth;
};
constexpr int NVAR = 16, VAR_X3 = 8;
constexpr Variant VARIANTS[NVAR] = {
    {false, 64, false, false, 1}, {false, 64, false, true, 1}, {false, 64, true, false, 1}, {false, 64, true, true, 1},
    {false, 128, false, false, 1}, {false, 128, false, true, 1}, {false, 128, true, false, 1}, {false, 128, true, true, 1},
    {true, 64, false, false, 1}, {true, 64, false, false, 3}, {true, 64, false, true, 1}, {true, 64, false, true, 3},
    {true, 64, true, false, 1}, {true, 64, true, false, 3}, {true, 64, true, true, 1}, {true, 64, true, true, 3},
};
constexpr int variant_index(bool x3, int bm, bool ak, bool bnc, int depth) {
    for (int v = 0; v < NVAR; ++v) {
        const Variant& d = VARIANTS[v];
        if (d.x3 == x3 && d.bm == bm && d.ak == ak && d.bnc == bnc && d.depth == depth) return v;
    }
    return -1;
}
constexpr int variant_lds(int v) {
    const Variant& d = VARIANTS[v];
    if (!d.x3) return d.bm == 128 ? TileLds<128, 128>::BYTES : TileLds<64, 64>::BYTES;
    return 3 * ((d.ak ? GxImg<true>::BYTES : GxImg<false>::BYTES) + (d.bnc ? GxImg<false>::BYTES : GxImg<true>::BYTES));
}
constexpr int set_lds(unsigned set) {
    int lds = 0;
    for (int v = 0; v < NVAR; ++v)
        if (((set >> v) & 1u) && variant_lds(v) > lds) lds = variant_lds(v);
    return lds;
}
template <class F, int... V>
inline void with_variant_seq(int v, F&& f, std::integer_sequence<int, V...>) {
    ((v == V ? (f(std::integral_constant<int, V>{}), 0) : 0), ...);
}
template <class F>
inline void with_variant(int v, F&& f) { with_variant_seq(v, f, std::make_integer_sequence<int, NVAR>{}); }

struct GemmPlan {
    GemmP p;
    int variant;
    unsigned gx, gy, gz;
    int lds;
};

int gemm_plan(const JvaeGemmDesc& a, int bias_div, GemmPlan* pl) {
    const bool part = a.want_splits > 0;
    if (a.M <= 0 || a.N <= 0 || a.batch <= 0) return 1;
    if (!a.A || !a.B || !a.C) return JVAE_EINVAL;
    if (part ? a.K <= 0 : a.K < 0) return JVAE_EINVAL;
    if (!part && a.bias_mode && !a.bias) return JVAE_EINVAL;
    GemmP& p = pl->p;
    p.A = a.A; p.sAm = a.sAm; p.sAk = a.sAk; p.sAb = a.sAb;
    p.B = a.B; p.sBk = a.sBk; p.sBn = a.sBn; p.sBb = a.sBb;
    p.C = a.C; p.sCm = a.sCm; p.sCn = a.sCn; p.sCb = a.sCb;
    p.bias = part ? nullptr : a.bias;
    p.bias_mode = part ? 0 : a.bias_mode;
    p.bias_div = (!part && bias_div > 0) ? bias_div : 1;
    p.M = a.M; p.N = a.N; p.K = a.K;
    int splitk = part ? a.want_splits : (a.splitk < 1 ? 1 : a.splitk);
    const int ktiles = cdiv(a.K, BK);
    if (splitk > ktiles) splitk = ktiles > 0 ? ktiles : 1;
    p.kchunk = cdiv(ktiles, splitk) * BK;
    splitk = a.K > 0 ? cdiv(a.K, p.kchunk) : 1;
    p.splitk = splitk;
    if (part) {
        p.flags = 8;
        p.sCsplit = a.sCsplit;
    } else {
        p.flags = a.flags & ~8;
        p.sCsplit = 0;
        if (splitk > 1) {
            if (a.flags & 2) return JVAE_EINVAL;
            p.flags |= 4;
        }
    }
    const bool ak = (a.sAk == 1), bnc = (a.sBn == 1);
    p.vecA = aligned16(a.A) && (a.sAb % 4 == 0) && (ak ? (a.sAm % 4 == 0) : (a.sAm == 1 && a.sAk % 4 == 0));
    p.vecB = aligned16(a.B) && (a.sBb % 4 == 0) && (bnc ? (a.sBk % 4 == 0) : (a.sBk == 1 && a.sBn % 4 == 0));
    p.xcd = 0;
    int bm = 64;
    if (gemm_x3_on(a.K)) {
        p.xcd = 1;
        const bool deep = p.vecA && p.vecB && p.K % 4 == 0 && (ak || p.M % 4 == 0) && (!bnc || p.N % 4 == 0);
        pl->variant = variant_index(true, 64, ak, bnc, deep ? 3 : 1);
    } else {
        const long tiles128 = (long)cdiv(a.M, 128) * cdiv(a.N, 128) * a.batch * splitk;
        if (!part && a.M > 64 && a.N > 64 && tiles128 >= 512) bm = 128;
        pl->variant = variant_index(false, bm, ak, bnc, 1);
    }
    pl->gx = cdiv(a.N, bm); pl->gy = cdiv(a.M, bm); pl->gz = (unsigned)a.batch * splitk;
    pl->lds = variant_lds(pl->variant);
    return part && !a.splits ? JVAE_EINVAL : 0;
}

template <typename F>
int set_lds_once(F kernel, int lds, bool* done) {
    if (!*done) {
        hipError_t e = hipFuncSetAttribute(reinterpret_cast<const void*>(kernel), hipFuncAttributeMaxDynamicSharedMemorySize, lds);
        if (e != hipSuccess) return (int)e;
        *done = true;
    }
    return 0;
}

template <int V>
int launch_variant(const GemmPlan& pl, hipStream_t st) {
    constexpr Variant d = VARIANTS[V];
    if constexpr (d.x3) {
        static bool attr_set = false;
        if (int rc = set_lds_once(&gemm_x3_kernel<d.ak, d.bnc, d.depth>, variant_lds(V), &attr_set)) return rc;
        hipLaunchKernelGGL((gemm_x3_kernel<d.ak, d.bnc, d.depth>), dim3(pl.gx, pl.gy, pl.gz), dim3(256), pl.lds, st, pl.p);
    } else {
        hipLaunchKernelGGL((gemm_kernel<d.bm, d.bm, d.ak, d.bnc>), dim3(pl.gx, pl.gy, pl.gz), dim3(256), 0, st, pl.p);
    }
    JVAE_LAUNCH_CHECK();
    return 0;
}

int launch_plan(const GemmPlan& pl, hipStream_t st) {
    int rc = JVAE_EINVAL;
    with_variant(pl.variant, [&](auto V) { rc = launch_variant<decltype(V)::value>(pl, st); });
    return rc;
}

constexpr int GROUP_MAX = 8;
struct GemmRec {
    GemmP p;
    int variant;
    unsigned gx, gy, gz;
    unsigned first;
};
struct GemmGroup {
    GemmRec rec[GROUP_MAX];
};

template <class G>
__device__ __forceinline__ unsigned group_record(const G& g, unsigned* local) {
    unsigned r = 0;
#pragma unroll
    for (unsigned i = 1; i < GROUP_MAX; ++i)
        if (blockIdx.x >= g.rec[i].first) r = i;
    *local = blockIdx.x - g.rec[r].first;
    return r;
}
template <class G>
void pad_records(G* g, int cnt) {
    for (int i = cnt; i < GROUP_MAX; ++i) { g->rec[i] = g->rec[0]; g->rec[i].first = 0xffffffffu; }
}

struct GroupTile { unsigned r, bx, by, bz; bool live; };
__device__ __forceinline__ GroupTile group_tile(const GemmGroup& g) {
    unsigned local;
    GroupTile t;
    t.r = group_record(g, &local);
    const GemmRec& rc = g.rec[t.r];
    t.live = local < rc.gx * rc.gy * rc.gz;
    t.bx = local % rc.gx; t.by = (local / rc.gx) % rc.gy; t.bz = local / (rc.gx * rc.gy);
    return t;
}

template <unsigned SET, int V>
__device__ __forceinline__ bool group_case(const GemmRec& rc, unsigned char* lds, const GroupTile& t) {
    constexpr Variant d = VARIANTS[V];
    if constexpr ((SET >> V) & 1u) {
        if (rc.variant == V) {
            if constexpr (d.x3) gemm_x3_body<d.ak, d.bnc, d.depth>(rc.p, lds, t.bx, t.by, t.bz, rc.gx, rc.gy, rc.gz);
            else gemm_tile_body<d.bm, d.bm, d.ak, d.bnc>(rc.p, reinterpret_cast<float*>(lds), t.bx, t.by, t.bz, rc.gx, rc.gy, rc.gz);
            return true;
        }
    }
    return false;
}
template <unsigned SET, bool STOP, int... V>
__device__ __forceinline__ void group_cases(const GemmGroup& g, unsigned char* lds, std::integer_sequence<int, V...>) {
    const GroupTile t = group_tile(g);
    if (!t.live) return;
    if constexpr (STOP) (void)(group_case<SET, V>(g.rec[t.r], lds, t) || ...);
    else (group_case<SET, V>(g.rec[t.r], lds, t), ...);
}

constexpr unsigned tile_set(bool big) {
    unsigned set = 0;
    for (int v = 0; v < VAR_X3; ++v)
        if (big || VARIANTS[v].bm == 64) set |= 1u << v;
    return set;
}
template <bool BIG>
__global__ __launch_bounds__(256) void gemm_group_tile_kernel(GemmGroup g) {
    extern __shared__ __attribute__((aligned(16))) unsigned char grp_lds[];
    group_cases<tile_set(BIG), true>(g, grp_lds, std::make_integer_sequence<int, NVAR>{});
}

constexpr unsigned x3_bit(bool ak, bool bnc, int depth) { return 1u << (variant_index(true, 64, ak, bnc, depth) - VAR_X3); }
constexpr unsigned X3_FWD = x3_bit(true, false, 3), X3_BWD = x3_bit(true, true, 3) | x3_bit(false, true, 3), X3_ALL = 0xffu;

template <unsigned MASK>
__global__ __launch_bounds__(256, 4) void gemm_group_x3_kernel(GemmGroup g) {
    extern __shared__ __attribute__((aligned(16))) unsigned char grp_lds[];
    group_cases<(MASK << VAR_X3), false>(g, grp_lds, std::make_integer_sequence<int, NVAR>{});
}

template <unsigned SET, class K>
int launch_group_set(K kernel, const GemmGroup& g, unsigned total, int lds, hipStream_t st) {
    static bool attr_set = false;
    if (int rc = set_lds_once(kernel, set_lds(SET), &attr_set)) return rc;
    hipLaunchKernelGGL(kernel, dim3(total), dim3(256), lds, st, g);
    JVAE_LAUNCH_CHECK();
    return 0;
}
template <bool BIG>
int launch_group_tile(const GemmGroup& g, unsigned total, int lds, hipStream_t st) {
    return launch_group_set<tile_set(BIG)>(&gemm_group_tile_kernel<BIG>, g, total, lds, st);
}
template <unsigned MASK>
int launch_group_x3(const GemmGroup& g, unsigned total, int lds, hipStream_t st) {
    return launch_group_set<(MASK << VAR_X3)>(&gemm_group_x3_kernel<MASK>, g, total, lds, st);
}

int launch_group_kind(const GemmPlan* plans, int n, bool x3, hipStream_t st) {
    GemmGroup g;
    int cnt = 0, lds = 0, last = -1;
    unsigned set = 0;
    unsigned long total = 0;
    for (int i = 0; i < n; ++i) {
        if (VARIANTS[plans[i].variant].x3 != x3) continue;
        GemmRec& rc = g.rec[cnt++];
        rc.p = plans[i].p; rc.variant = plans[i].variant;
        rc.gx = plans[i].gx; rc.gy = plans[i].gy; rc.gz = plans[i].gz;
        rc.first = (unsigned)total;
        total += ((unsigned long)rc.gx * rc.gy * rc.gz + 7) & ~7ul;
        if (total > 0x7fffffffUL) return JVAE_ENOTSUP;
        if (plans[i].lds > lds) lds = plans[i].lds;
        set |= 1u << rc.variant;
        last = i;
    }
    if (cnt == 0) return 0;
    if (cnt == 1) return launch_plan(plans[last], st);
    pad_records(&g, cnt);
    if (x3) {
        const unsigned mask = set >> VAR_X3;
        if ((mask & ~X3_FWD) == 0) return launch_group_x3<X3_FWD>(g, (unsigned)total, lds, st);
        if ((mask & ~X3_BWD) == 0) return launch_group_x3<X3_BWD>(g, (unsigned)total, lds, st);
        return launch_group_x3<X3_ALL>(g, (unsigned)total, lds, st);
    }
    if (set & ~tile_set(false)) return launch_group_tile<true>(g, (unsigned)total, lds, st);
    return launch_group_tile<false>(g, (unsigned)total, lds, st);
}

int launch_group(const GemmPlan* plans, int n, hipStream_t st) {
    if (int rc = launch_group_kind(plans, n, true, st)) return rc;
    return launch_group_kind(plans, n, false, st);
}

void plan_out_range(const GemmPlan& pl, uintptr_t* lo, uintptr_t* hi) {
    const GemmP& p = pl.p;
    const long batch = pl.gz / p.splitk;
    long neg = 0, pos = 0;
    auto span = [&](long stride, long count) {
        const long d = stride * (count - 1);
        if (d < 0) neg += d; else pos += d;
    };
    span(p.sCm, p.M); span(p.sCn, p.N); span(p.sCb, batch);
    if (p.flags & 8) span(p.sCsplit, p.splitk);
    *lo = reinterpret_cast<uintptr_t>(p.C + neg);
    *hi = reinterpret_cast<uintptr_t>(p.C + pos) + sizeof(float) - 1;
}

int plan_and_launch(const JvaeGemmDesc& d, int bias_div, hipStream_t st) {
    if (d.splits) *d.splits = 0;
    GemmPlan pl;
    const int rc = gemm_plan(d, bias_div, &pl);
    if (rc) return rc < 0 ? rc : 0;
    if (d.splits) *d.splits = pl.p.splitk;
    return launch_plan(pl, st);
}

}

int jvae_gemm_launch(int M, int N, int K, int batch,
                     const float* A, long sAm, long sAk, long sAb,
                     const float* B, long sBk, long sBn, long sBb,
                     float* C, long sCm, long sCn, long sCb,
                     const float* bias, int bias_mode, int flags, int splitk, hipStream_t st) {
    return jvae_gemm_launch_ex(M, N, K, batch, A, sAm, sAk, sAb, B, sBk, sBn, sBb, C, sCm, sCn, sCb, bias, bias_mode, 1,
                               flags, splitk, st);
}

int jvae_gemm_launch_ex(int M, int N, int K, int batch,
                        const float* A, long sAm, long sAk, long sAb,
                        const float* B, long sBk, long sBn, long sBb,
                        float* C, long sCm, long sCn, long sCb,
                        const float* bias, int bias_mode, int bias_div, int flags, int splitk, hipStream_t st) {
    JvaeGemmDesc d = {};
    d.M = M; d.N = N; d.K = K; d.batch = batch;
    d.A = A; d.sAm = sAm; d.sAk = sAk; d.sAb = sAb;
    d.B = B; d.sBk = sBk; d.sBn = sBn; d.sBb = sBb;
    d.C = C; d.sCm = sCm; d.sCn = sCn; d.sCb = sCb;
    d.bias = bias; d.bias_mode = bias_mode; d.flags = flags; d.splitk = splitk;
    return plan_and_launch(d, bias_div, st);
}

int jvae_gemm_launch_part(int M, int N, int K, int batch,
                          const float* A, long sAm, long sAk, long sAb,
                          const float* B, long sBk, long sBn, long sBb,
                          float* part, long sCm, long sCn, long sCb, long sCsplit, int want_splits, int* splits,
                          hipStream_t st) {
    JvaeGemmDesc d = {};
    d.M = M; d.N = N; d.K = K; d.batch = batch;
    d.A = A; d.sAm = sAm; d.sAk = sAk; d.sAb = sAb;
    d.B = B; d.sBk = sBk; d.sBn = sBn; d.sBb = sBb;
    d.C = part; d.sCm = sCm; d.sCn = sCn; d.sCb = sCb;
    d.want_splits = want_splits < 1 ? 1 : want_splits; d.sCsplit = sCsplit; d.splits = splits;
    return plan_and_launch(d, 1, st);
}

extern "C" int jvae_gemm_group_f32(const JvaeGemmDesc* descs, int n, void* stream) {
    if (n == 0) return 0;
    if (n < 0 || !descs) return JVAE_EINVAL;
    if (n > GROUP_MAX) return JVAE_ENOTSUP;
    GemmPlan plans[GROUP_MAX];
    uintptr_t lo[GROUP_MAX], hi[GROUP_MAX];
    int* splits[GROUP_MAX];
    int cnt = 0;
    for (int i = 0; i < n; ++i) {
        const JvaeGemmDesc& d = descs[i];
        if (d.splits) *d.splits = 0;
        const int rc = gemm_plan(d, 1, &plans[cnt]);
        if (rc < 0) return rc;
        if (rc) continue;
        plan_out_range(plans[cnt], &lo[cnt], &hi[cnt]);
        for (int j = 0; j < cnt; ++j)
            if (lo[cnt] <= hi[j] && lo[j] <= hi[cnt]) return JVAE_EINVAL;
        splits[cnt++] = d.splits;
    }
    for (int k = 0; k < cnt; ++k)
        if (splits[k]) *splits[k] = plans[k].p.splitk;
    return launch_group(plans, cnt, (hipStream_t)stream);
}

__device__ __forceinline__ void splitk_fold_body(const float* __restrict__ part, const float* __restrict__ bias, float* __restrict__ y,
                                                 int S, long MN, int N, int relu, int accumulate, int bias_div, unsigned block,
                                                 unsigned blocks) {
    for (long i = (long)block * blockDim.x + threadIdx.x; i < MN; i += (long)blocks * blockDim.x) {
        float v = bias ? bias[(i / bias_div) % N] : 0.f;
        for (int s = 0; s < S; ++s) v += part[(long)s * MN + i];
        if (accumulate) v += y[i];
        y[i] = relu ? fmaxf(v, 0.f) : v;
    }
}

__global__ __launch_bounds__(256) void splitk_fold_kernel(const float* __restrict__ part, const float* __restrict__ bias,
                                                          float* __restrict__ y, int S, long MN, int N, int relu,
                                                          int accumulate, int bias_div) {
    splitk_fold_body(part, bias, y, S, MN, N, relu, accumulate, bias_div, blockIdx.x, gridDim.x);
}

struct FoldRec {
    const float* part; const float* bias; float* y;
    long MN;
    int S, N, relu, accumulate, bias_div;
    unsigned first, blocks;
};
struct FoldGroup {
    FoldRec rec[GROUP_MAX];
};

__global__ __launch_bounds__(256) void splitk_fold_group_kernel(FoldGroup g) {
    unsigned local;
    const FoldRec& rc = g.rec[group_record(g, &local)];
    splitk_fold_body(rc.part, rc.bias, rc.y, rc.S, rc.MN, rc.N, rc.relu, rc.accumulate, rc.bias_div, local, rc.blocks);
}

inline int fold_blocks(long elems) { return (int)((elems + 255) / 256 > 4096 ? 4096 : (elems + 255) / 256); }

__global__ __launch_bounds__(256) void splitk_fold_qn_kernel(const float* __restrict__ part, const float* __restrict__ bias,
                                                             float* __restrict__ y, int S, int N, int Cs, int Ps) {
    const long total = (long)Ps * N * Cs;
    for (long i = (long)blockIdx.x * blockDim.x + threadIdx.x; i < total; i += (long)gridDim.x * blockDim.x) {
        const int cs = (int)(i % Cs);
        const long r = i / Cs;
        const int n = (int)(r % N), q = (int)(r / N);
        float v = bias ? bias[cs] : 0.f;
        for (int s = 0; s < S; ++s) v += part[(long)s * total + i];
        y[((long)n * Cs + cs) * Ps + q] = v;
    }
}

int jvae_splitk_fold_qn(const float* part, const float* bias, float* y, int S, int N, int Cs, int Ps, hipStream_t st) {
    const long total = (long)Ps * N * Cs;
    if (total == 0) return 0;
    hipLaunchKernelGGL(splitk_fold_qn_kernel, dim3(fold_blocks(total)), dim3(256), 0, st, part, bias, y, S, N, Cs, Ps);
    JVAE_LAUNCH_CHECK();
    return 0;
}

int jvae_splitk_fold(const float* part, const float* bias, float* y, int S, long MN, int N, int relu, int accumulate,
                     hipStream_t st, int bias_div) {
    if (MN == 0) return 0;
    hipLaunchKernelGGL(splitk_fold_kernel, dim3(fold_blocks(MN)), dim3(256), 0, st, part, bias, y, S, MN, N, relu, accumulate,
                       bias_div > 0 ? bias_div : 1);
    JVAE_LAUNCH_CHECK();
    return 0;
}

extern "C" int jvae_splitk_fold_f32(const float* part, const float* bias, float* y, int S, long MN, int N, int relu,
                                    int accumulate, void* stream) {
    if (!part || !y || S < 1 || MN < 0 || N < 1) return JVAE_EINVAL;
    return jvae_splitk_fold(part, bias, y, S, MN, N, relu, accumulate, (hipStream_t)stream);
}

extern "C" int jvae_splitk_fold_group_f32(const JvaeFoldDesc* descs, int n, void* stream) {
    if (n == 0) return 0;
    if (n < 0 || !descs) return JVAE_EINVAL;
    if (n > GROUP_MAX) return JVAE_ENOTSUP;
    FoldGroup g;
    int cnt = 0, last = -1;
    unsigned total = 0;
    for (int i = 0; i < n; ++i) {
        const JvaeFoldDesc& d = descs[i];
        if (!d.part || !d.y || d.S < 1 || d.MN < 0 || d.N < 1) return JVAE_EINVAL;
        for (int j = 0; j < i; ++j) {
            const JvaeFoldDesc& e = descs[j];
            if (d.MN > 0 && e.MN > 0 && d.y < e.y + e.MN && e.y < d.y + d.MN) return JVAE_EINVAL;
        }
        if (d.MN == 0) continue;
        FoldRec& rc = g.rec[cnt++];
        rc.part = d.part; rc.bias = d.bias; rc.y = d.y; rc.MN = d.MN;
        rc.S = d.S; rc.N = d.N; rc.relu = d.relu; rc.accumulate = d.accumulate; rc.bias_div = 1;
        rc.first = total; rc.blocks = (unsigned)fold_blocks(d.MN);
        total += rc.blocks;
        last = i;
    }
    if (cnt == 0) return 0;
    if (cnt == 1) {
        const JvaeFoldDesc& d = descs[last];
        return jvae_splitk_fold(d.part, d.bias, d.y, d.S, d.MN, d.N, d.relu, d.accumulate, (hipStream_t)stream);
    }
    pad_records(&g, cnt);
    hipLaunchKernelGGL(splitk_fold_group_kernel, dim3(total), dim3(256), 0, (hipStream_t)stream, g);
    JVAE_LAUNCH_CHECK();
    return 0;
}

extern "C" int jvae_gemm_f32(int M, int N, int K, int batch,
                             const float* A, long sAm, long sAk, long sAb,
                             const float* B, long sBk, long sBn, long sBb,
                             float* C, long sCm, long sCn, long sCb,
                             const float* bias, int bias_mode, int flags, int splitk, void* stream) {
    return jvae_gemm_launch(M, N, K, batch, A, sAm, sAk, sAb, B, sBk, sBn, sBb, C, sCm, sCn, sCb,
                            bias, bias_mode, flags, splitk, (hipStream_t)stream);
}

extern "C" int jvae_gemm_route(const JvaeGemmDesc* d, JvaeGemmRoute* out) {
    if (!d || !out) return JVAE_EINVAL;
    *out = JvaeGemmRoute{-1, 0, 0, 0, 0, 0, 0, 0, 0};
    GemmPlan pl;
    const int rc = gemm_plan(*d, 1, &pl);
    if (rc) return rc < 0 ? rc : 0;
    *out = JvaeGemmRoute{pl.variant, (int)pl.gx, (int)pl.gy, (int)pl.gz, pl.p.splitk, pl.p.kchunk, pl.p.vecA, pl.p.vecB, pl.lds};
    return 0;
}

extern "C" const char* jvae_gemm_variant_name(int variant) {
    struct Names {
        char s[NVAR][16];
        Names() {
            for (int v = 0; v < NVAR; ++v) {
                const Variant& d = VARIANTS[v];
                const char *a = d.ak ? "AK" : "AM", *b = d.bnc ? "BN" : "BK";
                if (d.x3) snprintf(s[v], sizeof s[v], "X3_%s_%s_D%d", a, b, d.depth);
                else snprintf(s[v], sizeof s[v], "TILE%d_%s_%s", d.bm, a, b);
            }
        }
    };
    static const Names names;
    return (variant >= 0 && variant < NVAR) ? names.s[variant] : nullptr;
}
```

### joint-vae_amd/csrc/jvae_internal.h

```cpp
#pragma once
#include <hip/hip_runtime.h>
#include <type_traits>
#include "common.h"

int jvae_gemm_launch(int M, int N, int K, int batch,
                     const float* A, long sAm, long sAk, long sAb,
                     const float* B, long sBk, long sBn, long sBb,
                     float* C, long sCm, long sCn, long sCb,
                     const float* bias, int bias_mode, int flags, int splitk, hipStream_t st);

int jvae_gemm_launch_ex(int M, int N, int K, int batch,
                        const float* A, long sAm, long sAk, long sAb,
                        const float* B, long sBk, long sBn, long sBb,
                        float* C, long sCm, long sCn, long sCb,
                        const float* bias, int bias_mode, int bias_div, int flags, int splitk, hipStream_t st);

int jvae_splitk_fold_qn(const float* part, const float* bias, float* y, int S, int N, int Cs, int Ps, hipStream_t st);
int jvae_splitk_fold(const float* part, const float* bias, float* y, int S, long MN, int N, int relu, int accumulate,
                     hipStream_t st, int bias_div = 1);

int jvae_gemm_launch_part(int M, int N, int K, int batch,
                          const float* A, long sAm, long sAk, long sAb,
                          const float* B, long sBk, long sBn, long sBb,
                          float* part, long sCm, long sCn, long sCb, long sCsplit, int want_splits, int* splits,
                          hipStream_t st);

struct InAff { const float* sc; const float* sh; int relu; };

inline int jvae_aff_inst(const InAff& a) { return !a.sc ? 0 : (a.relu == JVAE_ACT_LEAKY ? 2 : 1); }
template <class F>
inline void jvae_with_aff(int inst, F&& f) {
    if (inst == 2) f(std::integral_constant<int, 2>{});
    else if (inst == 1) f(std::integral_constant<int, 1>{});
    else f(std::integral_constant<int, 0>{});
}
template <class K>
inline int jvae_aff_lds_attr(bool& done, int bytes, K&& kernel) {
    for (int inst = 0; inst < 3 && !done; ++inst) {
        hipError_t e = hipSuccess;
        jvae_with_aff(inst, [&](auto A) {
            e = hipFuncSetAttribute(reinterpret_cast<const void*>(kernel(A)), hipFuncAttributeMaxDynamicSharedMemorySize, bytes);
        });
        if (e != hipSuccess) return (int)e;
    }
    done = true;
    return 0;
}

struct ConvGeom {
    int N;
    int Cb, Hb, Wb;
    int Cs, Hs, Ws;
    int KH, KW, S, P;
};

int jvae_wgrad_slab_reduce(const float* slab, float* dw, int G, int Ca, int Cb, int accumulate, int swapflip, hipStream_t st,
                           int tapmajor = 0, int taps = 25);
```

### joint-vae_amd/jvae_hip/lib.py

```python
import ctypes
import os
from ctypes import c_char_p, c_float, c_int, c_long, c_longlong, c_size_t, c_void_p, POINTER

import torch

_HERE = os.path.dirname(os.path.abspath(__file__))
LIB_PATH = os.environ.get('JVAE_HIP_LIB') or os.path.join(_HERE, 'libjvae_hip.so')

_lib = None

P = c_void_p


class GemmDesc(ctypes.Structure):
    _fields_ = ([('M', c_int), ('N', c_int), ('K', c_int), ('batch', c_int)]
                + [('A', P), ('sAm', c_long), ('sAk', c_long), ('sAb', c_long)]
                + [('B', P), ('sBk', c_long), ('sBn', c_long), ('sBb', c_long)]
                + [('C', P), ('sCm', c_long), ('sCn', c_long), ('sCb', c_long)]
                + [('bias', P), ('bias_mode', c_int), ('flags', c_int), ('splitk', c_int)]
                + [('want_splits', c_int), ('sCsplit', c_long), ('splits', POINTER(c_int))])


class FoldDesc(ctypes.Structure):
    _fields_ = [('part', P), ('bias', P), ('y', P), ('S', c_int), ('MN', c_long), ('N', c_int), ('relu', c_int),
                ('accumulate', c_int)]


class GemmRoute(ctypes.Structure):
    _fields_ = [(n, c_int) for n in ('variant', 'gx', 'gy', 'gz', 'slices', 'kchunk', 'vecA', 'vecB', 'lds')]


_SIGS = {
    'jvae_version': (c_char_p, []),
    'jvae_gemm_route': (c_int, [POINTER(GemmDesc), POINTER(GemmRoute)]),
    'jvae_gemm_variant_name': (c_char_p, [c_int]),
    'jvae_gemm_f32': (c_int, [c_int] * 4 + [P, c_long, c_long, c_long] * 3 + [P, c_int, c_int, c_int, P]),
    'jvae_splitk_fold_f32': (c_int, [P, P, P, c_int, c_long, c_int, c_int, c_int, P]),
    'jvae_gemm_group_f32': (c_int, [POINTER(GemmDesc), c_int, P]),
    'jvae_splitk_fold_group_f32': (c_int, [POINTER(FoldDesc), c_int, P]),
    'jvae_conv2d_workspace_bytes': (c_size_t, [c_int] * 11),
    'jvae_conv2d_set_split_bf16': (c_int, [c_int]),
    'jvae_conv2d_set_split_shape16': (c_int, [c_int]),
    'jvae_conv2d_out_shape': (c_int, [c_int] * 8 + [POINTER(c_int), POINTER(c_int)]),
    'jvae_conv2d_route': (c_int, [c_int] * 17 + [POINTER(c_int), POINTER(c_int), POINTER(c_size_t), POINTER(c_int), POINTER(c_int)]),
    'jvae_conv2d_kernel_name': (c_char_p, [c_int]),
    'jvae_conv2d_fwd_f32': (c_int, [P, P, P, P] + [c_int] * 11 + [P, c_size_t, P]),
    'jvae_conv2d_stats_splits': (c_int, [c_int] * 11),
    'jvae_conv2d_fwd_stats_f32': (c_int, [P, P, P, P, P, POINTER(c_int)] + [c_int] * 11 + [P, c_size_t, P]),
    'jvae_conv2d_dgrad_f32': (c_int, [P, P, P] + [c_int] * 11 + [P, c_size_t, P]),
    'jvae_conv2d_wgrad_f32': (c_int, [P, P, P, P, c_int] + [c_int] * 11 + [P, c_size_t, P]),
    'jvae_b8_pack_f32': (c_int, [P, P, c_int, c_int, c_long, P]),
    'jvae_b8_unpack_f32': (c_int, [P, P, c_int, c_int, c_long, c_int, P]),
    'jvae_conv2d_native_b8': (c_int, [c_int] * 11),
    'jvae_conv2d_workspace_bytes_b8': (c_size_t, [c_int] * 11),
    'jvae_conv2d_stats_splits_b8': (c_int, [c_int] * 11),
    'jvae_conv2d_fwd_b8': (c_int, [P, P, P, P, c_int, P, POINTER(c_int)] + [c_int] * 11 + [P, c_size_t, P]),
    'jvae_conv2d_dgrad_b8': (c_int, [P, P, P] + [c_int] * 11 + [P, c_size_t, P]),
    'jvae_conv2d_wgrad_b8': (c_int, [P, P, P, P, c_int] + [c_int] * 11 + [P, c_size_t, P]),
    'jvae_bn_workspace_bytes_b8': (c_size_t, [c_int]),
    'jvae_bn_plan_b8': (c_int, [c_int, c_int, c_long, POINTER(c_int), POINTER(c_int)]),
    'jvae_bn_fwd_b8': (c_int, [P] * 9 + [c_int, c_int, c_long, c_float, c_float, c_int, c_int, P, c_int, P, P, c_size_t, P]),
    'jvae_bn_bwd_b8': (c_int, [P] * 9 + [c_int, c_int, c_int, c_long, c_int, P, c_size_t, P]),
    'jvae_bn_finalize_b8': (c_int, [P] * 9 + [c_int, c_int, c_long, c_float, c_float, c_int, P, c_int, P, P, c_size_t, P]),
    'jvae_bn_sums_b8': (c_int, [P, P, P, c_int, c_int, c_long, P, c_size_t, P]),
    'jvae_bn_fwd_sync_b8': (c_int, [P] * 9 + [c_int, c_int, c_long, c_float, c_float, c_int, P, P, c_int, P, c_size_t, P]),
    'jvae_bn_bwd_sums_b8': (c_int, [P] * 7 + [c_int, c_int, c_long, c_int, P, c_size_t, P]),
    'jvae_bn_bwd_sync_b8': (c_int, [P] * 8 + [c_int, P, P, P, c_int, c_int, c_int, c_long, c_int, P, c_size_t, P]),
    'jvae_conv2d_affine_ok_b8': (c_int, [c_int] * 11),
    'jvae_conv2d_fwd_aff_b8': (c_int, [P, P, P, P, c_int, P, POINTER(c_int), P, P, c_int] + [c_int] * 11 + [P, c_size_t, P]),
    'jvae_conv2d_wgrad_aff_b8': (c_int, [P, P, P, P, c_int, P, P, c_int] + [c_int] * 11 + [P, c_size_t, P]),
    'jvae_relu_fwd_b8': (c_int, [P, P, c_long, P]),
    'jvae_relu_bwd_b8': (c_int, [P, P, P, c_long, P]),
    'jvae_bn_finalize_f32': (c_int, [P] * 10 + [c_int, c_int, c_int, c_float, c_float, c_int, P, c_int, P, P, c_size_t, P]),
    'jvae_conv2d_affine_ok': (c_int, [c_int] * 11),
    'jvae_conv2d_fwd_aff_f32': (c_int, [P, P, P, P, P, POINTER(c_int), P, P, c_int] + [c_int] * 11 + [P, c_size_t, P]),
    'jvae_conv2d_wgrad_aff_f32': (c_int, [P, P, P, P, c_int, P, P, c_int] + [c_int] * 11 + [P, c_size_t, P]),
    'jvae_pack_cache_configure': (c_int, [P, c_size_t]),
    'jvae_pack_cache_begin': (c_int, [P, c_longlong, P, c_int]),
    'jvae_pack_cache_end': (c_int, []),
    'jvae_pack_cache_pin': (c_int, []),
    'jvae_pack_cache_reset': (c_int, []),
    'jvae_pack_cache_stats': (c_int, [POINTER(c_int), POINTER(c_longlong), POINTER(c_longlong), POINTER(c_longlong)]),
    'jvae_channel_sum_workspace_bytes': (c_size_t, [c_int]),
    'jvae_channel_sum_f32': (c_int, [P, P, c_int, c_int, c_int, c_int, P, c_size_t, P]),
    'jvae_bn_workspace_bytes': (c_size_t, [c_int]),
    'jvae_bn_plan': (c_int, [c_int, c_int, c_int, POINTER(c_int), POINTER(c_int)]),
    'jvae_image_range': (c_int, [c_int, c_int, c_int, POINTER(c_int), POINTER(c_int)]),
    'jvae_bn_fwd_f32': (c_int, [P] * 9 + [c_int, c_int, c_int, c_float, c_float, c_int, c_int, P, c_size_t, P]),
    'jvae_bn_fwd_ext_f32': (c_int, [P] * 9 + [c_int, c_int, c_int, c_float, c_float, c_int, c_int, P, c_int, P, P, c_size_t, P]),
    'jvae_bn_sums_f32': (c_int, [P, P, P, c_int, c_int, c_int, P, c_size_t, P]),
    'jvae_bn_fwd_sync_f32': (c_int, [P] * 9 + [c_int, c_int, c_int, c_float, c_float, c_int, P, P, c_int, P, c_size_t, P]),
    'jvae_bn_bwd_sums_f32': (c_int, [P] * 7 + [c_int, c_int, c_int, c_int, P, c_size_t, P]),
    'jvae_bn_bwd_sync_f32': (c_int, [P] * 8 + [c_int, P, P, P, c_int, c_int, c_int, c_int, c_int, P]),
    'jvae_bn_bwd_f32': (c_int, [P] * 9 + [c_int, c_int, c_int, c_int, c_int, P, c_size_t, P]),
    'jvae_bn_eval_bwd_f32': (c_int, [P] * 7 + [c_int, c_int, c_int, c_float, c_int, P]),
    'jvae_act_fwd_f32': (c_int, [P, P, c_long, c_int, P]),
    'jvae_act_bwd_f32': (c_int, [P, P, P, c_long, c_int, P]),
    'jvae_dict_stats_f32': (c_int, [P, P, c_int, c_int, P]),
    'jvae_latent_fwd_f32': (c_int, [P] * 13 + [c_int] * 6 + [c_float] * 3 + [c_int, c_int, c_float, P]),
    'jvae_latent_bwd_f32': (c_int, [P] * 17 + [c_int] * 6 + [c_float] * 3 + [c_int, c_int, P, c_size_t, P]),
    'jvae_latent_fwd_wdev_f32': (c_int, [P] * 13 + [c_int] * 6 + [c_float] * 3 + [c_int, c_int, c_float, P, P]),
    'jvae_latent_bwd_wdev_f32': (c_int, [P] * 17 + [c_int] * 6 + [c_float] * 3 + [c_int, c_int, P, P, c_size_t, P]),
    'jvae_latent_mixed_fwd_f32': (c_int, [P] * 15 + [c_int] * 4 + ([c_int] * 3 + [c_float] * 2) * 2
                                  + [c_float, c_int, c_int, c_float, P]),
    'jvae_latent_mixed_bwd_f32': (c_int, [P] * 19 + [c_int] * 4 + ([c_int] * 3 + [c_float] * 2) * 2
                                  + [c_float, c_int, c_int, P, c_size_t, P]),
    'jvae_latent_refine_f32': (c_int, [P] * 17 + [c_int] * 6 + [c_float] * 2 + [c_int, c_int, c_float, c_float, c_long, c_int, P]),
    'jvae_recon_fwd_f32':(c_int, [P, P, P, c_int, P, c_int, c_int, c_int, P]),
    'jvae_recon_bwd_f32': (c_int, [P, P, P, c_int, P, P, P, P, P, c_int, c_int, c_int, c_int, P, c_size_t, P]),
    'jvae_mse_rows_fwd_f32': (c_int, [P, P, P, c_int, c_int, c_int, P]),
    'jvae_mse_rows_bwd_f32': (c_int, [P, P, P, P, c_int, c_int, c_int, P]),
    'jvae_elbo_fwd_f32': (c_int, [P, P, P, P, c_int, P, P, P, P, c_int, c_int, c_int, c_float, c_float, P]),
    'jvae_elbo_bwd_f32': (c_int, [P, P, P, P, c_int, P, P, P, P, c_int, c_int, c_int, c_int, c_float, c_float, P, c_size_t, P]),
    'jvae_elbo_fwd_wdev_f32': (c_int, [P, P, P, P, c_int, P, P, P, P, c_int, c_int, c_int, c_float, c_float, P, P]),
    'jvae_elbo_bwd_wdev_f32': (c_int, [P, P, P, P, c_int, P, P, P, P, c_int, c_int, c_int, c_int, c_float, c_float, P, P, c_size_t, P]),
    'jvae_measures_dev_f32': (c_int, [P, c_long, P, P, P, c_int, c_int, P, c_int, P, c_int, c_int, P, P, P, P]),
    'jvae_loss_sums_f32': (c_int, [P, P, c_int, P, P]),
    'jvae_measures_f32': (c_int, [P, c_long, P, P, P, c_int, c_int, P, c_int, P, c_int, c_int, P, P, c_int, P, P]),
    'jvae_dropout_f32': (c_int, [P, P, c_long, c_float, c_long, P]),
    'jvae_dropout_dev_f32': (c_int, [P, P, c_long, c_float, P, c_long, P]),
    'jvae_iws_f32': (c_int, [P, P, P, P, P, c_int, c_int, c_int, c_int, c_int, c_int, P, P, P]),
    'jvae_xent_fwd_f32': (c_int, [P, P, P, c_int, c_int, c_int, P]),
    'jvae_xent_bwd_f32': (c_int, [P, P, P, P, c_int, c_int, c_int, P]),
    'jvae_augment_u8_f32': (c_int, [P, P, P, P, P, c_int, c_int, c_int, c_int, c_int, c_int, P]),
    'jvae_imageset_desc_words': (c_int, []),
    'jvae_imageset_batch_u8_f32': (c_int, [P] * 4 + [POINTER(c_int)] + [P] * 9 + [c_long, c_int, P]),
    'jvae_imageset_mix_leaf_bytes': (c_int, []),
    'jvae_imageset_mixed_u8_f32': (c_int, [P, P, c_int] + [P] * 5 + [c_int] + [P] * 3 + [c_int, c_int, P]),
    'jvae_sqnorm_workspace_bytes': (c_size_t, []),
    'jvae_sqnorm_accum_f32': (c_int, [P, c_long, P, c_int, P, c_size_t, P]),
    'jvae_clip_scale_f32': (c_int, [P, c_long, P, c_float, P]),
    'jvae_adam_step_dev_f32': (c_int, [P, P, P, P, c_long, P, c_int, c_float, c_float, c_float, P, P, P]),
    'jvae_adam_step_f32': (c_int, [P, P, P, P, c_long] + [c_float] * 5 + [c_long, c_float, P, P, P]),
    'jvae_sgd_step_f32': (c_int, [P, P, P, c_long, c_float, c_float, c_int, c_float, c_int, c_float, P, P, P]),
    'jvae_pool2d_out_shape': (c_int, [c_int] * 5 + [POINTER(c_int), POINTER(c_int)]),
    'jvae_pool2d_fwd_f32': (c_int, [P, P, P, c_long] + [c_int] * 6 + [P]),
    'jvae_pool2d_bwd_f32': (c_int, [P, P, P, c_long] + [c_int] * 6 + [P]),
    'jvae_upsample_nearest_fwd_f32': (c_int, [P, P, c_long, c_int, c_int, c_int, P]),
    'jvae_upsample_nearest_bwd_f32': (c_int, [P, P, c_long, c_int, c_int, c_int, P]),
    'jvae_pool2d_fwd_b8': (c_int, [P, P, P, c_long] + [c_int] * 6 + [P]),
    'jvae_pool2d_bwd_b8': (c_int, [P, P, P, c_long] + [c_int] * 6 + [P]),
    'jvae_upsample_nearest_fwd_b8': (c_int, [P, P, c_long, c_int, c_int, c_int, P]),
    'jvae_upsample_nearest_bwd_b8': (c_int, [P, P, c_long, c_int, c_int, c_int, P]),
    'jvae_roc_workspace_bytes': (c_size_t, [c_int, c_long, c_long]),
    'jvae_roc_curve_f32': (c_int, [P] * 10 + [c_int, c_long, c_long, c_int, P, c_size_t, P]),
    'jvae_pr_workspace_bytes': (c_size_t, [c_int, c_long, c_long]),
    'jvae_pr_metrics_f32': (c_int, [P] * 5 + [c_int, c_long, c_long, P, c_size_t, P]),
    'jvae_scod_scores_f32': (c_int, [P] * 8 + [c_long, c_int, c_int, c_long, P, P]),
    'jvae_scod_workspace_bytes': (c_size_t, [c_int, c_long]),
    'jvae_scod_curve_f32': (c_int, [P] * 6 + [c_int, c_long, c_long, P, c_size_t, P]),
    'jvae_misclass_scores_f32': (c_int, [P] * 5 + [c_int, c_int, c_long, c_long, P]),
    'jvae_misclass_split_workspace_bytes': (c_size_t, [c_long]),
    'jvae_misclass_split_f32': (c_int, [P, P, P, P, c_int, c_long, P, c_size_t, P]),
    'jvae_misclass_confusion_f32': (c_int, [P] * 5 + [c_int, c_long, c_int, P]),
    'jvae_odin_head_f32': (c_int, [P, P, P, P, c_int, c_int, c_int, c_int, c_long, c_long, P]),
    'jvae_odin_perturb_f32': (c_int, [P, P, P, P, P, c_long, c_int, P]),
    'jvae_wim_scores_f32': (c_int, [P, P, P, c_int, P, P, c_int, P, c_long, c_int, c_long, P, P]),
    'jvae_group_tally_f32': (c_int, [P, P, P, P, c_int, c_int, c_int, P]),
    'jvae_prior_sample_f32': (c_int, [P] * 6 + [c_long, c_int, c_int, c_float, c_int, P]),
    'jvae_image_grid_f32': (c_int, [P, P, P, P, c_int, P, P] + [c_int] * 5 + [P]),
    'jvae_class_posterior_f32': (c_int, [P] * 5 + [c_int, P, P, c_long, c_int, c_int, c_int, P]),
    'jvae_latent_mi_workspace_bytes': (c_size_t, [c_int, c_int, c_long]),
    'jvae_latent_mi_f32': (c_int, [P, P, P, c_int, c_int, c_int, c_int, c_long, P, c_size_t, P]),
    'jvae_aggregate_scores_f32': (c_int, [P, P, c_int, c_int, P, c_int, P, P, P, P, c_int, c_int, c_long, P, P]),
    'jvae_cascade_mse_workspace_bytes': (c_size_t, [c_int, c_long, c_long]),
    'jvae_cascade_mse_f32': (c_int, [P, P, c_int, P, c_int, c_long, c_long, P, c_size_t, P]),
    'jvae_iterate_prior_f32': (c_int, [P, P, c_int, c_int, c_long, P]),
    'jvae_latent_moments_workspace_bytes': (c_size_t, [c_int, c_int, c_int]),
    'jvae_latent_moments_f32': (c_int, [P, P, P, P, P, c_int, c_int, c_int, P, c_size_t, P]),
    'jvae_nearest_centroid_f32': (c_int, [P, P, P, P, c_long, c_int, c_int, P]),
    'jvae_histogram_f32': (c_int, [P, P, P, P, P, c_long, c_int, c_int, P]),
    'jvae_pairwise_sqdist_f32': (c_int, [P, P, c_int, c_int, P]),
    'jvae_tsne_affinities_workspace_bytes': (c_size_t, [c_int]),
    'jvae_tsne_affinities_f32': (c_int, [P, P, P, P, c_float, c_int, P, c_size_t, P]),
    'jvae_tsne_gradient_workspace_bytes': (c_size_t, [c_int]),
    'jvae_tsne_gradient_f32': (c_int, [P, P, P, c_float, c_int, P, P, c_size_t, P]),
    'jvae_tsne_update_f32': (c_int, [P, P, P, P, c_float, c_float, c_int, P, P]),
    'jvae_pca_moments_workspace_bytes': (c_size_t, [c_long, c_int]),
    'jvae_pca_moments_f32': (c_int, [P, P, P, c_long, c_int, P, c_size_t, P]),
    'jvae_project_f32': (c_int, [P, P, P, P, c_long, c_int, c_int, P]),
    'jvae_knn_sqnorms_f32': (c_int, [P, P, c_long, c_int, P]),
    'jvae_knn_workspace_bytes': (c_size_t, [c_long, c_long, c_int, c_int, c_int]),
    'jvae_knn_f32': (c_int, [P] * 6 + [c_long, c_long, c_int, c_int, c_int, c_int, P, P, c_size_t, P]),
    'jvae_maha_moments_workspace_bytes': (c_size_t, [c_long, c_int, c_int]),
    'jvae_maha_moments_f32': (c_int, [P, P, c_long, c_int, c_int] + [P] * 6 + [P, c_size_t, P]),
    'jvae_maha_scores_f32': (c_int, [P] * 10 + [c_long, c_int, c_int, c_int, P, P]),
    'jvae_image_code_length_f32': (c_int, [P, c_long, c_int, c_int, c_int, P, c_long, P, P, P, P, P]),
    'jvae_kde_partition': (c_int, []),
    'jvae_kde_fit_workspace_bytes': (c_size_t, [c_long, c_int]),
    'jvae_kde_fit_f32': (c_int, [P, c_long, c_int, P] + [P] * 7 + [P, c_size_t, P]),
    'jvae_kde_workspace_bytes': (c_size_t, [c_long, c_long, c_int]),
    'jvae_kde_logdensity_f32': (c_int, [P] * 7 + [c_long, c_long, c_int, P, P, P, c_size_t, P]),
    'jvae_ssim_f32': (c_int, [P, P, c_long, c_long, c_int, c_int, c_int, P, P, P, P, P]),
    'jvae_ssim_strip_rows': (c_int, [c_int, c_int]),
    'jvae_aggpost_partition': (c_int, []),
    'jvae_aggpost_padded_rows': (c_long, [c_long]),
    'jvae_aggpost_prepare_f32': (c_int, [P] * 6 + [c_long, c_int, P]),
    'jvae_aggpost_workspace_bytes': (c_size_t, [c_long, c_long, c_int, c_int]),
    'jvae_aggpost_logdensity_f32': (c_int, [P] * 9 + [c_long, c_long, c_int, c_int, P, P, c_size_t, P]),
    'jvae_iw_bound_fwd_f32': (c_int, [P] * 8 + [c_int] * 3 + [c_float] + [c_int] * 5 + [P] * 5),
    'jvae_iw_bound_bwd_workspace_bytes': (c_size_t, [c_int, c_int]),
    'jvae_iw_bound_bwd_f32': (c_int, [P] * 7 + [c_int] * 3 + [c_float] + [c_int] * 5 + [P] * 7 + [c_size_t, P]),
    'jvae_tc_joint_partition': (c_int, []),
    'jvae_tc_keep_bytes': (c_size_t, [c_int] * 3),
    'jvae_tc_fwd_workspace_bytes': (c_size_t, [c_int] * 3),
    'jvae_tc_bwd_workspace_bytes': (c_size_t, [c_int] * 2),
    'jvae_tc_objective_fwd_f32': (c_int, [P] * 8 + [c_int] + [c_float] * 3 + [c_int] * 4 + [P] * 5 + [c_size_t, P, c_size_t, P]),
    'jvae_tc_objective_bwd_f32': (c_int, [P] * 7 + [c_int] + [c_float] * 3 + [c_int] * 4 + [P, c_size_t] + [P] * 6 + [c_size_t, P]),
    'jvae_semi_keep_bytes': (c_size_t, [c_int] * 2),
    'jvae_semi_fwd_workspace_bytes': (c_size_t, [c_int] * 2),
    'jvae_semi_class_marginal_fwd_f32': (c_int, [P] * 6 + [c_int, c_float] + [c_int] * 3 + [P] * 7 + [c_size_t, P, c_size_t, P]),
    'jvae_semi_class_marginal_bwd_f32': (c_int, [P] * 6 + [c_int, c_float] + [c_int] * 3 + [P, c_size_t] + [P] * 6),
}


class JvaeHipError(RuntimeError):
    pass


def load():
    global _lib
    if _lib is not None:
        return _lib
    if not os.path.exists(LIB_PATH):
        raise JvaeHipError(f'{LIB_PATH} is missing: build it with `python -c "import __graft_entry__ as g; g.build()"` '
                           'or `make -C joint-vae_amd/csrc` (there is no CPU/PyTorch fallback)')
    lib = ctypes.CDLL(LIB_PATH)
    for name, (res, args) in _SIGS.items():
        fn = getattr(lib, name)
        fn.restype = res
        fn.argtypes = args
    _lib = lib
    return lib


def exported_symbols():
    return list(_SIGS)


_ERR = {-1: 'invalid argument', -2: 'unsupported configuration', -3: 'workspace too small'}


def check(rc, what):
    if rc != 0:
        msg = _ERR.get(rc, f'hipError_t {rc}')
        raise JvaeHipError(f'{what} failed: {msg}')


_raw_stream = getattr(torch._C, '_cuda_getCurrentRawStream', None)


def stream_ptr(device_index=None):
    if _raw_stream is not None:
        return _raw_stream(torch.cuda.current_device() if device_index is None else device_index)
    return torch.cuda.current_stream().cuda_stream


def ptr(t):
    if t is None:
        return None
    if not t.is_cuda:
        raise JvaeHipError('jvae_hip ops need tensors resident on the GPU (no CPU fallback); got device '
                           + str(t.device))
    if not t.is_contiguous():
        raise JvaeHipError('jvae_hip ops need contiguous tensors')
    return t.data_ptr()


_workspaces = {}
_side_streams = {}


def side_stream(device):
    idx = device.index if device.index is not None else torch.cuda.current_device()
    st = _side_streams.get(idx)
    if st is None:
        _side_streams[idx] = st = torch.cuda.Stream(device=idx)
    return st


def join_side_stream(device=None):
    for idx, st in _side_streams.items():
        if device is None or device.index in (None, idx):
            torch.cuda.current_stream(idx).wait_stream(st)


def workspace(nbytes, device):
    idx = device.index if device.index is not None else torch.cuda.current_device()
    key = (idx, stream_ptr(idx))
    ws = _workspaces.get(key)
    if ws is None or ws.numel() < nbytes:
        _workspaces[key] = ws = torch.empty(max(int(nbytes), 1 << 20), dtype=torch.uint8, device=device)
    return ws


PACK_CACHE_BYTES = int(os.environ.get('JVAE_PACK_CACHE_MB', '64')) << 20
_pack_cache = {}
span_depth = 0
span_hold = 0


def pack_cache_begin(weights, device):
    if not PACK_CACHE_BYTES:
        return
    lib = load()
    idx = device.index if device.index is not None else torch.cuda.current_device()
    if idx not in _pack_cache:
        if _pack_cache:
            check(lib.jvae_pack_cache_configure(None, 0), 'jvae_pack_cache_configure')
            _pack_cache[idx] = None
        else:
            buf = torch.empty(PACK_CACHE_BYTES + 256, dtype=torch.uint8, device=device)
            off = (-buf.data_ptr()) % 256
            _pack_cache[idx] = buf
            check(lib.jvae_pack_cache_configure(buf.data_ptr() + off, PACK_CACHE_BYTES), 'jvae_pack_cache_configure')
    if _pack_cache[idx] is None:
        return
    addrs = tuple(w.data_ptr() for w in weights)
    arr = (ctypes.c_void_p * max(len(addrs), 1))(*addrs)
    check(lib.jvae_pack_cache_begin(stream_ptr(idx), hash(addrs), arr, len(addrs)), 'jvae_pack_cache_begin')


def pack_cache_end():
    if _lib is not None and _pack_cache:
        _lib.jvae_pack_cache_end()


def pack_cache_pin():
    if _lib is not None and _pack_cache and PACK_CACHE_BYTES:
        _lib.jvae_pack_cache_pin()


def pack_cache_stats():
    lib = load()
    e, h, m, r = c_int(), c_longlong(), c_longlong(), c_longlong()
    lib.jvae_pack_cache_stats(ctypes.byref(e), ctypes.byref(h), ctypes.byref(m), ctypes.byref(r))
    return {'entries': e.value, 'hits': h.value, 'misses': m.value, 'refreshes': r.value}
```

### joint-vae_amd/jvae_hip/ops.py

```python
import collections
import contextlib
import ctypes
import math
from ctypes import byref, c_int, c_size_t

import numpy as np
import torch

from . import lib as L

RELU, SIGMOID, IDENT, LEAKY = 1, 2, 0, 3
BN_ACT = {IDENT: 0, RELU: 1, LEAKY: 2}
OVERLAP_WGRAD = True
ACT_KIND = {'relu': RELU, 'sigmoid': SIGMOID, 'linear': IDENT, 'leaky': LEAKY, None: IDENT}


def _c(t):
    return t if t.is_contiguous() else t.contiguous()


def _f32(t, what):
    if t.dtype != torch.float32:
        raise L.JvaeHipError(f'{what}: fp32 expected, got {t.dtype}')
    return t


def _grad_slot(param):
    if param is None or not isinstance(param, torch.nn.Parameter):
        return None
    g = param.grad
    if g is None or not g.is_contiguous() or g.dtype != torch.float32 or g.shape != param.shape or not g.is_cuda:
        return None
    return g


def _join_after_backward():
    torch.autograd.Variable._execution_engine.queue_callback(L.join_side_stream)


def _close_span_after_backward():
    if not L.span_hold:
        torch.autograd.Variable._execution_engine.queue_callback(L.pack_cache_end)


def gemm(M, N, K, A, sA, B, sB, C, sC, bias=None, bias_mode=0, flags=0, splitk=1, batch=1):
    lib = L.load()
    rc = lib.jvae_gemm_f32(M, N, K, batch, L.ptr(A), *sA, L.ptr(B), *sB, L.ptr(C), *sC,
                           L.ptr(bias), bias_mode, flags, splitk, L.stream_ptr())
    L.check(rc, 'jvae_gemm_f32')


def gemm_desc(M, N, K, A, sA, B, sB, C, sC, bias=None, bias_mode=0, flags=0, splitk=1, batch=1):
    return (M, N, K, batch, A, sA, B, sB, C, sC, bias, bias_mode, flags, splitk)


def _fill_gemm_desc(d, rec, ptr):
    M, N, K, batch, A, sA, B, sB, C, sC, bias, bias_mode, flags, splitk = rec
    d.M, d.N, d.K, d.batch = M, N, K, batch
    d.A, (d.sAm, d.sAk, d.sAb) = ptr(A), sA
    d.B, (d.sBk, d.sBn, d.sBb) = ptr(B), sB
    d.C, (d.sCm, d.sCn, d.sCb) = ptr(C), sC
    d.bias, d.bias_mode, d.flags, d.splitk = ptr(bias), bias_mode, flags, splitk


def gemm_group(descs):
    lib = L.load()
    arr = (L.GemmDesc * max(len(descs), 1))()
    for d, rec in zip(arr, descs):
        _fill_gemm_desc(d, rec, L.ptr)
    L.check(lib.jvae_gemm_group_f32(arr, len(descs), L.stream_ptr()), 'jvae_gemm_group_f32')


GemmRoute = collections.namedtuple('GemmRoute', 'variant grid slices kchunk vecA vecB lds')


def gemm_route(M, N, K, A, sA, B, sB, C, sC, bias=None, bias_mode=0, flags=0, splitk=1, batch=1, want_splits=0, sCsplit=0):
    lib = L.load()
    addr = lambda t: t if t is None or isinstance(t, int) else t.data_ptr()
    d, r, made = L.GemmDesc(), L.GemmRoute(), c_int(0)
    _fill_gemm_desc(d, gemm_desc(M, N, K, A, sA, B, sB, C, sC, bias, bias_mode, flags, splitk, batch), addr)
    d.want_splits, d.sCsplit = want_splits, sCsplit
    if want_splits > 0:
        d.splits = ctypes.pointer(made)
    L.check(lib.jvae_gemm_route(byref(d), byref(r)), 'jvae_gemm_route')
    name = lib.jvae_gemm_variant_name(r.variant)
    return GemmRoute(name.decode() if name is not None else None, (r.gx, r.gy, r.gz), r.slices, r.kchunk, bool(r.vecA), bool(r.vecB),
                     r.lds)


def splitk_fold_group(jobs):
    lib = L.load()
    arr = (L.FoldDesc * max(len(jobs), 1))()
    for d, (part, bias, y, S, MN, N, relu, accumulate) in zip(arr, jobs):
        d.part, d.bias, d.y = L.ptr(part), L.ptr(bias), L.ptr(y)
        d.S, d.MN, d.N, d.relu, d.accumulate = S, MN, N, relu, accumulate
    L.check(lib.jvae_splitk_fold_group_f32(arr, len(jobs), L.stream_ptr()), 'jvae_splitk_fold_group_f32')


def _run_products(descs, folds):
    if len(descs) == 1:
        M, N, K, batch, A, sA, B, sB, C, sC, bias, bias_mode, flags, splitk = descs[0]
        gemm(M, N, K, A, sA, B, sB, C, sC, bias=bias, bias_mode=bias_mode, flags=flags, splitk=splitk, batch=batch)
    elif descs:
        gemm_group(descs)
    if len(folds) == 1:
        part, bias, y, S, MN, N, relu, accumulate = folds[0]
        L.check(L.load().jvae_splitk_fold_f32(L.ptr(part), L.ptr(bias), L.ptr(y), S, MN, N, relu, accumulate, L.stream_ptr()),
                'jvae_splitk_fold_f32')
    elif folds:
        splitk_fold_group(folds)


def channel_sum(t, N, C, P, out=None, accumulate=False):
    lib = L.load()
    if out is None:
        out = torch.empty(C, device=t.device, dtype=torch.float32)
    ws = L.workspace(lib.jvae_channel_sum_workspace_bytes(C), t.device)
    L.check(lib.jvae_channel_sum_f32(L.ptr(t), L.ptr(out), N, C, P, int(accumulate), L.ptr(ws), ws.numel(), L.stream_ptr()),
            'channel_sum')
    return out


def _linear_split(R, O, I):
    tiles = ((R + 63) // 64) * ((O + 63) // 64)
    if tiles >= 128 or I < 512:
        return 1
    for S in (32, 16, 8, 4, 2):
        if tiles * S <= 1024 and I % S == 0 and I // S >= 128:
            return S
    return 1


class _Linear(torch.autograd.Function):

    @staticmethod
    def forward(ctx, x, w, b, act):
        x2 = _c(_f32(x, 'linear').reshape(-1, x.shape[-1]))
        w_in = w
        w = _c(w)
        O = w.shape[0]
        descs, folds = [], []
        y = _linear_fwd_products(x2, w, b, act, descs, folds)
        _run_products(descs, folds)
        if act in (SIGMOID, LEAKY):
            L.check(L.load().jvae_act_fwd_f32(L.ptr(y), L.ptr(y), y.numel(), act, L.stream_ptr()), 'act_fwd')
        ctx.save_for_backward(x2, w, y if act != IDENT else None)
        ctx.act = act
        ctx.has_bias = b is not None
        ctx.xshape = x.shape
        ctx.w_ref, ctx.b_ref = w_in, b
        return y.reshape(*x.shape[:-1], O)

    @staticmethod
    def backward(ctx, gy):
        x2, w, y = ctx.saved_tensors
        lib = L.load()
        R, I = x2.shape
        O = w.shape[0]
        gy = _c(gy.reshape(R, O))
        if ctx.act != IDENT:
            g = torch.empty_like(gy)
            L.check(lib.jvae_act_bwd_f32(L.ptr(gy), L.ptr(y), L.ptr(g), gy.numel(), ctx.act, L.stream_ptr()), 'act_bwd')
            gy = g
        descs, folds = [], []
        gx, gw = _linear_bwd_products(gy, x2, w, ctx.w_ref, ctx.needs_input_grad[0], ctx.needs_input_grad[1], descs, folds)
        _run_products(descs, folds)
        if gx is not None:
            gx = gx.reshape(ctx.xshape)
        gb = _linear_bias_grad(gy, ctx.b_ref) if ctx.has_bias and ctx.needs_input_grad[2] else None
        return gx, gw, gb, None


def _linear_fwd_products(x2, w, b, act, descs, folds):
    R, I = x2.shape
    O = w.shape[0]
    y = torch.empty((R, O), device=x2.device, dtype=torch.float32)
    S = _linear_split(R, O, I)
    if S > 1:
        part = torch.empty((S, R, O), device=x2.device, dtype=torch.float32)
        Ks = I // S
        descs.append(gemm_desc(R, O, Ks, x2, (I, 1, Ks), w, (1, I, Ks), part, (O, 1, R * O), batch=S))
        folds.append((part, b, y, S, R * O, O, int(act == RELU), 0))
    else:
        descs.append(gemm_desc(R, O, I, x2, (I, 1, 0), w, (1, I, 0), y, (O, 1, 0), bias=b, bias_mode=1 if b is not None else 0,
                               flags=2 if act == RELU else 0))
    return y


def _linear_bwd_products(gy, x2, w, w_ref, need_x, need_w, descs, folds):
    R, I = x2.shape
    O = w.shape[0]
    gx = gw = None
    if need_x:
        gx = torch.empty((R, I), device=gy.device, dtype=torch.float32)
        descs.append(gemm_desc(R, I, O, gy, (O, 1, 0), w, (I, 1, 0), gx, (I, 1, 0)))
    if need_w:
        slot = _grad_slot(w_ref)
        gw = slot if slot is not None else torch.zeros((O, I), device=gy.device, dtype=torch.float32)
        S = _linear_split(O, I, R)
        if S > 1:
            part = torch.empty((S, O, I), device=gy.device, dtype=torch.float32)
            Rs = R // S
            descs.append(gemm_desc(O, I, Rs, gy, (1, O, Rs * O), x2, (I, 1, Rs * I), part, (I, 1, O * I), batch=S))
            folds.append((part, None, gw, S, O * I, I, 0, 1))
        else:
            descs.append(gemm_desc(O, I, R, gy, (1, O, 0), x2, (I, 1, 0), gw, (I, 1, 0), flags=1))
        if slot is not None:
            gw = None
    return gx, gw


def _linear_bias_grad(gy, b_ref):
    R, O = gy.shape
    slot = _grad_slot(b_ref)
    if slot is not None:
        channel_sum(gy, R, O, 1, out=slot, accumulate=True)
        return None
    return channel_sum(gy, R, O, 1)


def linear(x, w, b=None, act=IDENT):
    return _Linear.apply(x, w, b, act)


class _LinearPair(torch.autograd.Function):

    @staticmethod
    def forward(ctx, x, w0, b0, w1, b1):
        x2 = _c(_f32(x, 'linear_pair').reshape(-1, x.shape[-1]))
        ws = (_c(w0), _c(w1))
        descs, folds = [], []
        ys = [_linear_fwd_products(x2, w, b, IDENT, descs, folds) for w, b in zip(ws, (b0, b1))]
        _run_products(descs, folds)
        ctx.save_for_backward(x2, *ws)
        ctx.xshape = x.shape
        ctx.refs = ((w0, b0), (w1, b1))
        ctx.set_materialize_grads(False)
        return tuple(y.reshape(*x.shape[:-1], y.shape[1]) for y in ys)

    @staticmethod
    def backward(ctx, g0, g1):
        x2, *ws = ctx.saved_tensors
        R = x2.shape[0]
        descs, folds = [], []
        out = []
        gxs = []
        gys = []
        for h, g in enumerate((g0, g1)):
            if g is None:
                out += [None, None]
                gys.append(None)
                continue
            gy = _c(g.reshape(R, ws[h].shape[0]))
            gx, gw = _linear_bwd_products(gy, x2, ws[h], ctx.refs[h][0], ctx.needs_input_grad[0], ctx.needs_input_grad[1 + 2 * h],
                                          descs, folds)
            if gx is not None:
                gxs.append(gx)
            out += [gw, None]
            gys.append(gy)
        _run_products(descs, folds)
        for h, gy in enumerate(gys):
            b_ref = ctx.refs[h][1]
            if gy is not None and b_ref is not None and ctx.needs_input_grad[2 + 2 * h]:
                out[1 + 2 * h] = _linear_bias_grad(gy, b_ref)
        gx = None
        if gxs:
            gx = (gxs[0] if len(gxs) == 1 else torch.add(gxs[0], gxs[1])).reshape(ctx.xshape)
        return (gx, *out)


def linear_pair(x, w0, b0, w1, b1):
    if w0 is w1:
        return linear(x, w0, b0), linear(x, w1, b1)
    return _LinearPair.apply(x, w0, b0, w1, b1)


_GEOM_CACHE = {}


def _geom_query(name, geom):
    key = (name, geom)
    r = _GEOM_CACHE.get(key)
    if r is None:
        _GEOM_CACHE[key] = r = getattr(L.load(), name)(*geom)
    return r


class ConvSpec:
    __slots__ = ('cin', 'cout', 'k', 's', 'p', 'op', 'transposed')

    def __init__(self, cin, cout, k, s, p, op=0, transposed=False):
        self.cin, self.cout, self.k, self.s, self.p, self.op, self.transposed = cin, cout, k, s, p, op, bool(transposed)

    def out_hw(self, H, W):
        key = ('hw', self.k, self.s, self.p, self.op, self.transposed, H, W)
        r = _GEOM_CACHE.get(key)
        if r is None:
            oh, ow = c_int(), c_int()
            rc = L.load().jvae_conv2d_out_shape(H, W, self.k, self.k, self.s, self.p, self.op, int(self.transposed),
                                                byref(oh), byref(ow))
            L.check(rc, 'jvae_conv2d_out_shape')
            _GEOM_CACHE[key] = r = (oh.value, ow.value)
        return r

    def geom(self, N, H, W):
        return (N, self.cin, H, W, self.cout, self.k, self.k, self.s, self.p, self.op, int(self.transposed))


def _conv_ws(geom, device):
    nbytes = _geom_query('jvae_conv2d_workspace_bytes', geom)
    ws = L.workspace(nbytes, device)
    return ws, ws.numel()


def conv_fwd_raw(x, w, b, spec):
    N, _, H, W = x.shape
    oh, ow = spec.out_hw(H, W)
    y = torch.empty((N, spec.cout, oh, ow), device=x.device, dtype=torch.float32)
    geom = spec.geom(N, H, W)
    ws, nb = _conv_ws(geom, x.device)
    rc = L.load().jvae_conv2d_fwd_f32(L.ptr(x), L.ptr(w), L.ptr(b), L.ptr(y), *geom, L.ptr(ws), nb, L.stream_ptr())
    L.check(rc, 'jvae_conv2d_fwd_f32')
    return y


def conv_fwd_stats_raw(x, w, b, spec):
    lib = L.load()
    N, _, H, W = x.shape
    geom = spec.geom(N, H, W)
    cap = _geom_query('jvae_conv2d_stats_splits', geom)
    if cap <= 0:
        return conv_fwd_raw(x, w, b, spec), None, 0
    oh, ow = spec.out_hw(H, W)
    y = torch.empty((N, spec.cout, oh, ow), device=x.device, dtype=torch.float32)
    stats = torch.empty((spec.cout * cap * 2,), device=x.device, dtype=torch.float32)
    ws, nb = _conv_ws(geom, x.device)
    ns = c_int(0)
    rc = lib.jvae_conv2d_fwd_stats_f32(L.ptr(x), L.ptr(w), L.ptr(b), L.ptr(y), L.ptr(stats), byref(ns), *geom,
                                       L.ptr(ws), nb, L.stream_ptr())
    L.check(rc, 'jvae_conv2d_fwd_stats_f32')
    return y, (stats if ns.value > 0 else None), ns.value


def conv_affine_ok(spec, N, H, W):
    return bool(_geom_query('jvae_conv2d_affine_ok', spec.geom(N, H, W)))


ConvRoute = collections.namedtuple('ConvRoute', 'kernel swap ws splits aff_ok')
ROUTE_DIR = {'fwd': 1, 'dgrad': 2, 'wgrad': 4}
ROUTE_LAYOUT = {'f32': 0, 'b8': 1}


def conv_route(spec, N, H, W, direction, layout='f32', bias=False, stats=False, y_f32=False, aff=0):
    lib = L.load()
    k, sw, ns, ok, ws = c_int(), c_int(), c_int(), c_int(), c_size_t()
    rc = lib.jvae_conv2d_route(ROUTE_DIR[direction], ROUTE_LAYOUT[layout], int(bias), int(stats), int(y_f32), int(aff),
                               *spec.geom(N, H, W), byref(k), byref(sw), byref(ws), byref(ns), byref(ok))
    L.check(rc, 'jvae_conv2d_route')
    return ConvRoute(lib.jvae_conv2d_kernel_name(k.value).decode(), bool(sw.value), ws.value, ns.value, bool(ok.value))


class LaunchProbe:

    def __init__(self, match):
        self.match, self.events, self.armed = match, [], False

    def times_ms(self):
        return [a.elapsed_time(b) for a, b in self.events]


FWD_AFF_PROBE = None


def conv_fwd_aff_raw(x, w, b, spec, aff, want_stats):
    lib = L.load()
    N, _, H, W = x.shape
    geom = spec.geom(N, H, W)
    oh, ow = spec.out_hw(H, W)
    y = torch.empty((N, spec.cout, oh, ow), device=x.device, dtype=torch.float32)
    stats, ns = None, c_int(0)
    if want_stats:
        cap = _geom_query('jvae_conv2d_stats_splits', geom)
        if cap > 0:
            stats = torch.empty((spec.cout * cap * 2,), device=x.device, dtype=torch.float32)
    ws, nb = _conv_ws(geom, x.device)
    probe = FWD_AFF_PROBE
    timed = probe is not None and probe.armed and probe.match(spec, N, H)
    if timed:
        ev = (torch.cuda.Event(enable_timing=True), torch.cuda.Event(enable_timing=True))
        ev[0].record()
    rc = lib.jvae_conv2d_fwd_aff_f32(L.ptr(x), L.ptr(w), L.ptr(b), L.ptr(y), L.ptr(stats), byref(ns),
                                     L.ptr(aff[0]), L.ptr(aff[1]), int(aff[2]), *geom, L.ptr(ws), nb, L.stream_ptr())
    if timed:
        ev[1].record()
        probe.events.append(ev)
    L.check(rc, 'jvae_conv2d_fwd_aff_f32')
    return y, (stats if ns.value > 0 else None), ns.value


def conv_dgrad_raw(gy, w, spec, xshape):
    N, _, H, W = xshape
    gx = torch.empty(xshape, device=gy.device, dtype=torch.float32)
    geom = spec.geom(N, H, W)
    ws, nb = _conv_ws(geom, gy.device)
    rc = L.load().jvae_conv2d_dgrad_f32(L.ptr(gy), L.ptr(w), L.ptr(gx), *geom, L.ptr(ws), nb, L.stream_ptr())
    L.check(rc, 'jvae_conv2d_dgrad_f32')
    return gx


def conv_wgrad_raw(x, gy, spec, wshape, want_bias, w_slot=None, b_slot=None, aff=None):
    N, _, H, W = x.shape
    inplace = w_slot is not None and (b_slot is not None or not want_bias)
    gw = w_slot if inplace else torch.empty(wshape, device=x.device, dtype=torch.float32)
    gb = None
    if want_bias:
        gb = b_slot if inplace else torch.empty(spec.cout, device=x.device, dtype=torch.float32)
    geom = spec.geom(N, H, W)
    ws, nb = _conv_ws(geom, x.device)
    if aff is not None:
        rc = L.load().jvae_conv2d_wgrad_aff_f32(L.ptr(x), L.ptr(gy), L.ptr(gw), L.ptr(gb), int(inplace),
                                                L.ptr(aff[0]), L.ptr(aff[1]), int(aff[2]), *geom, L.ptr(ws), nb,
                                                L.stream_ptr())
    else:
        rc = L.load().jvae_conv2d_wgrad_f32(L.ptr(x), L.ptr(gy), L.ptr(gw), L.ptr(gb), int(inplace), *geom, L.ptr(ws), nb,
                                            L.stream_ptr())
    L.check(rc, 'jvae_conv2d_wgrad_f32')
    return (None, None) if inplace else (gw, gb)


FWD, DGRAD, WGRAD = 1, 2, 4


class Layout:
    sfx = '_f32'
    ws_sfx = ''
    acts = BN_ACT

    def dims(self, x, C):
        N, C = x.shape[0], x.shape[1]
        return N, C, x.numel() // max(N * C, 1)

    def coef_width(self, C):
        return C

    def prep(self, x, what):
        return _c(_f32(x, what))

    def to_f32(self, t, C):
        return t

    def from_f32(self, t):
        return t

    def native(self, spec, N, H, W):
        return FWD | DGRAD | WGRAD

    def affine_ok(self, spec, N, H, W):
        return conv_affine_ok(spec, N, H, W)

    def conv_fwd(self, x, w, b, spec, want_stats, aff, out_f32):
        if aff is not None:
            return conv_fwd_aff_raw(x, w, b, spec, aff, want_stats)
        if want_stats:
            return conv_fwd_stats_raw(x, w, b, spec)
        return conv_fwd_raw(x, w, b, spec), None, 0

    def conv_dgrad(self, gy, w, spec, N, H, W):
        return conv_dgrad_raw(gy, w, spec, (N, spec.cin, H, W))

    def conv_wgrad(self, *args):
        return conv_wgrad_raw(*args)

    def bn(self, name, *args, ws=None):
        name += self.sfx
        extra = () if ws is None else (L.ptr(ws), ws.numel())
        L.check(getattr(L.load(), name)(*args, *extra, L.stream_ptr()), name)

    def bn_workspace(self, C, device):
        return L.workspace(getattr(L.load(), 'jvae_bn_workspace_bytes' + self.ws_sfx)(C), device)

    def bn_fwd(self, *args, ext, ws):
        if ext[0] is None:
            self.bn('jvae_bn_fwd', *args, ws=ws)
        else:
            self.bn('jvae_bn_fwd_ext', *args, *ext, ws=ws)

    def coef_args(self, coef):
        return L.ptr(coef[0]), L.ptr(coef[1])

    def bn_bwd_sync(self, *args, ws):
        self.bn('jvae_bn_bwd_sync', *args)


F32 = Layout()


def layout_of(t):
    return _b8.B8 if _b8.is_b8(t) else F32


class _Conv(torch.autograd.Function):

    @staticmethod
    def forward(ctx, x, w, b, spec, dead_bias, stats_out, aff, out_f32):
        lay = layout_of(x)
        x = lay.prep(x, 'conv')
        if not L.span_depth:
            L.pack_cache_end()
        ctx.w_ref, ctx.b_ref = w, b
        w = _c(w)
        native = lay.native(spec, x.shape[0], x.shape[2], x.shape[3])
        if aff is not None and (native & (FWD | WGRAD)) != FWD | WGRAD:
            raise L.JvaeHipError('a deferred BatchNorm needs native forward and weight-gradient kernels (conv_affine_ok)')
        want_stats = stats_out is not None
        if native & FWD:
            y, st, ns = lay.conv_fwd(x, w, b, spec, want_stats, aff, out_f32)
        else:
            y, st, ns = F32.conv_fwd(lay.to_f32(x, spec.cin), w, b, spec, want_stats, None, False)
            y = y if out_f32 else lay.from_f32(y)
        if want_stats:
            stats_out['stats'], stats_out['nsplit'], stats_out['pivot'] = st, ns, b
        ctx.save_for_backward(x, w)
        ctx.lay, ctx.native, ctx.spec, ctx.out_f32, ctx.aff = lay, native, spec, out_f32, aff
        ctx.has_bias = b is not None
        ctx.dead_bias = dead_bias
        return y

    @staticmethod
    def backward(ctx, gy):
        x, w = ctx.saved_tensors
        lay, spec = ctx.lay, ctx.spec
        N, H, W = x.shape[0], x.shape[2], x.shape[3]
        gys = {F32 if ctx.out_f32 else lay: _c(gy)}

        def gy_in(want):
            if want not in gys:
                have, g = next(iter(gys.items()))
                gys[want] = want.from_f32(g) if have is F32 else have.to_f32(g, spec.cout)
            return gys[want]
        gx = gw = gb = None
        _close_span_after_backward()
        want_b = ctx.has_bias and ctx.needs_input_grad[2] and not ctx.dead_bias
        wgrad = ctx.needs_input_grad[1] or want_b
        on_side = False
        if wgrad:
            w_slot = _grad_slot(ctx.w_ref)
            b_slot = _grad_slot(ctx.b_ref) if want_b else None
            on_side = (OVERLAP_WGRAD and ctx.needs_input_grad[0] and w_slot is not None
                       and (b_slot is not None or not want_b))
        if ctx.needs_input_grad[0]:
            dl = lay if ctx.native & DGRAD else F32
            gyd = gy_in(dl)
        if on_side:
            side = L.side_stream(x.device)
            side.wait_stream(torch.cuda.current_stream(x.device))
        if ctx.needs_input_grad[0]:
            gx = dl.conv_dgrad(gyd, w, spec, N, H, W)
            gx = gx if dl is lay else lay.from_f32(gx)
        if wgrad:
            with torch.cuda.stream(side) if on_side else contextlib.nullcontext():
                wl = lay if ctx.native & WGRAD else F32
                xw = x if wl is lay else lay.to_f32(x, spec.cin)
                gw, gb = wl.conv_wgrad(xw, gy_in(wl), spec, w.shape, want_b, w_slot, b_slot, ctx.aff)
            if on_side:
                for t in (x, xw, *gys.values(), *(ctx.aff[:2] if ctx.aff is not None else ())):
                    t.record_stream(side)
                _join_after_backward()
# ... 2650 lines not shown
```

Baseline: 141,300.

## Add implicit-unfold mapped GEMM for convs and grouped channel-sum for linear pairs

```diff
diff --git a/include/jvae_hip.h b/include/jvae_hip.h
--- a/include/jvae_hip.h
+++ b/include/jvae_hip.h
@@ -48,6 +48,7 @@
                                    int transposed);
 int jvae_conv2d_set_split_bf16(int mode);
 int jvae_conv2d_set_split_shape16(int on);
+int jvae_conv2d_set_implicit_unfold(int on);
 int jvae_conv2d_out_shape(int H, int W, int KH, int KW, int S, int P, int OP, int transposed, int* OH, int* OW);
 int jvae_conv2d_route(int dir, int layout, int bias, int stats, int y_f32, int aff_kind,
                       int N, int Cin, int H, int W, int Cout, int KH, int KW, int S, int P, int OP, int transposed,
@@ -75,6 +76,11 @@
 int jvae_pack_cache_stats(int* entries, long long* hits, long long* misses, long long* refreshes);
 
 size_t jvae_channel_sum_workspace_bytes(int C);
+typedef struct JvaeChanSumDesc {
+    const float* t; float* out;
+    int N, C, P, accumulate;
+} JvaeChanSumDesc;
+int jvae_channel_sum_group_f32(const JvaeChanSumDesc* descs, int n, void* ws, size_t ws_bytes, void* stream);
 int jvae_channel_sum_f32(const float* t, float* out, int N, int C, int P, int accumulate, void* ws, size_t ws_bytes,
                          void* stream);
 
diff --git a/joint-vae_amd/csrc/conv_api.hip b/joint-vae_amd/csrc/conv_api.hip
--- a/joint-vae_amd/csrc/conv_api.hip
+++ b/joint-vae_amd/csrc/conv_api.hip
@@ -58,6 +58,7 @@
 
 int jvae_conv2d_set_split_bf16(int mode) { return jvae_conv5_x3_set(mode); }
 int jvae_conv2d_set_split_shape16(int on) { return jvae_conv5_x3_set_shape16(on); }
+int jvae_conv2d_set_implicit_unfold(int on) { return jvae_conv_generic_set_implicit(on); }
 
 size_t jvae_conv2d_workspace_bytes(int N, int Cin, int H, int W, int Cout, int KH, int KW, int S, int P, int OP,
                                    int transposed) {
@@ -173,4 +174,13 @@
     return jvae_channel_sum(t, out, N, C, P, accumulate, (float*)ws, ws_bytes, (hipStream_t)stream);
 }
 
+int jvae_channel_sum_group_f32(const JvaeChanSumDesc* descs, int n, void* ws, size_t ws_bytes, void* stream) {
+    if (n == 0) return 0;
+    if (n < 0 || !descs) return JVAE_EINVAL;
+    if (n > 8) return JVAE_ENOTSUP;
+    for (int i = 0; i < n; ++i)
+        if (!descs[i].t || !descs[i].out || descs[i].N < 0 || descs[i].C <= 0 || descs[i].P <= 0) return JVAE_EINVAL;
+    return jvae_channel_sum_group(descs, n, (float*)ws, ws_bytes, (hipStream_t)stream);
 }
+
+}
diff --git a/joint-vae_amd/csrc/conv_dispatch.h b/joint-vae_amd/csrc/conv_dispatch.h
--- a/joint-vae_amd/csrc/conv_dispatch.h
+++ b/joint-vae_amd/csrc/conv_dispatch.h
@@ -1,4 +1,5 @@
 #pragma once
+#include "jvae_hip.h"
 #include "common.h"
 #include "jvae_internal.h"
 
@@ -9,7 +10,9 @@
                   float* ws, size_t ws_bytes, hipStream_t st);
 int jvae_fold_wgrad(const ConvGeom& g, const float* xb, const float* ys, float* dw,
                     float* ws, size_t ws_bytes, hipStream_t st);
+int jvae_conv_generic_set_implicit(int on);
 size_t jvae_channel_sum_ws_bytes(int C);
+int jvae_channel_sum_group(const JvaeChanSumDesc* descs, int n, float* ws, size_t ws_bytes, hipStream_t st);
 int jvae_channel_sum(const float* t, float* out, int N, int C, int P, int accumulate, float* ws, size_t ws_bytes,
                      hipStream_t st);
 
diff --git a/joint-vae_amd/csrc/conv_generic.hip b/joint-vae_amd/csrc/conv_generic.hip
--- a/joint-vae_amd/csrc/conv_generic.hip
+++ b/joint-vae_amd/csrc/conv_generic.hip
@@ -1,4 +1,5 @@
 #include "common.h"
+#include "jvae_hip.h"
 #include "jvae_internal.h"
 
 namespace {
@@ -93,10 +94,8 @@
     }
 }
 
-__global__ __launch_bounds__(256) void channel_sum_kernel(const float* __restrict__ t, float* __restrict__ partial,
-                                                          int N, int C, int P, int nsplit) {
-    __shared__ float red[17];
-    const int c = blockIdx.x, sp = blockIdx.y;
+__device__ __forceinline__ void channel_sum_body(const float* __restrict__ t, float* __restrict__ partial, int N, int C, int P,
+                                                 int nsplit, int c, int sp, float* red) {
     const ImageRange ir = image_range(N, nsplit, sp);
     const int nb = ir.nb, ne = ir.ne;
     float s = 0.f;
@@ -119,13 +118,51 @@
     if (threadIdx.x == 0) partial[(long)c * nsplit + sp] = s;
 }
 
-__global__ void channel_fold_kernel(const float* __restrict__ partial, float* __restrict__ out, int C, int nsplit,
-                                    int accumulate) {
-    const int c = blockIdx.x * blockDim.x + threadIdx.x;
+__global__ __launch_bounds__(256) void channel_sum_kernel(const float* __restrict__ t, float* __restrict__ partial,
+                                                          int N, int C, int P, int nsplit) {
+    __shared__ float red[17];
+    channel_sum_body(t, partial, N, C, P, nsplit, blockIdx.x, blockIdx.y, red);
+}
+
+__device__ __forceinline__ void channel_fold_body(const float* __restrict__ partial, float* __restrict__ out, int C, int nsplit,
+                                                  int accumulate, int c) {
     if (c >= C) return;
     float s = 0.f;
     for (int k = 0; k < nsplit; ++k) s += partial[(long)c * nsplit + k];
     out[c] = (accumulate ? out[c] : 0.f) + s;
+}
+
+__global__ void channel_fold_kernel(const float* __restrict__ partial, float* __restrict__ out, int C, int nsplit,
+                                    int accumulate) {
+    channel_fold_body(partial, out, C, nsplit, accumulate, blockIdx.x * blockDim.x + threadIdx.x);
+}
+
+constexpr int CS_GROUP_MAX = 8;
+struct ChanSumRec {
+    const float* t; float* partial; float* out;
+    int N, C, P, nsplit, accumulate;
+    unsigned first, ffirst;
+};
+struct ChanSumGroup { ChanSumRec rec[CS_GROUP_MAX]; };
+
+__global__ __launch_bounds__(256) void channel_sum_group_kernel(ChanSumGroup g) {
+    __shared__ float red[17];
+    unsigned r = 0;
+#pragma unroll
+    for (unsigned i = 1; i < CS_GROUP_MAX; ++i)
+        if (blockIdx.x >= g.rec[i].first) r = i;
+    const ChanSumRec& rc = g.rec[r];
+    const unsigned local = blockIdx.x - rc.first;
+    channel_sum_body(rc.t, rc.partial, rc.N, rc.C, rc.P, rc.nsplit, (int)(local % rc.C), (int)(local / rc.C), red);
+}
+
+__global__ void channel_fold_group_kernel(ChanSumGroup g) {
+    unsigned r = 0;
+#pragma unroll
+    for (unsigned i = 1; i < CS_GROUP_MAX; ++i)
+        if (blockIdx.x >= g.rec[i].ffirst) r = i;
+    const ChanSumRec& rc = g.rec[r];
+    channel_fold_body(rc.partial, rc.out, rc.C, rc.nsplit, rc.accumulate, (int)((blockIdx.x - rc.ffirst) * blockDim.x + threadIdx.x));
 }
 
 inline int fold_slab_images(const ConvGeom& g) {
@@ -193,6 +230,21 @@
 
 inline long col_floats_per_image(const ConvGeom& g) { return (long)g.Cb * g.KH * g.KW * g.Hs * g.Ws; }
 
+int g_implicit = 1;
+constexpr bool MAP_FWD = false, MAP_DGRAD = false, MAP_WGRAD = false;
+inline bool use_map(bool kept) { return g_implicit == 2 || (g_implicit == 1 && kept); }
+
+inline JvaeGemmDesc dense_desc(int M, int N, int K, int batch, const float* A, long sAm, long sAk, long sAb,
+                               const float* B, long sBk, long sBn, long sBb, float* C, long sCm, long sCn, long sCb) {
+    JvaeGemmDesc d = {};
+    d.M = M; d.N = N; d.K = K; d.batch = batch;
+    d.A = A; d.sAm = sAm; d.sAk = sAk; d.sAb = sAb;
+    d.B = B; d.sBk = sBk; d.sBn = sBn; d.sBb = sBb;
+    d.C = C; d.sCm = sCm; d.sCn = sCn; d.sCb = sCb;
+    d.splitk = 1;
+    return d;
+}
+
 inline long wgrad_part_floats(const ConvGeom& g) { return (long)g.Cs * g.Cb * g.KH * g.KW; }
 
 }
@@ -223,18 +275,36 @@
     const int Kd = g.Cb * g.KH * g.KW, Ps = g.Hs * g.Ws;
     if (pixel_batched(g)) {
         if (ws_bytes < (size_t)col_floats_per_image(g) * 4 * g.N) return JVAE_EWORKSPACE;
-        { const int rc = launch_unfold(xb, ws, g, 0, g.N, true, st); if (rc) return rc; }
+        GemmOperandMap mx;
+        bool mapped = use_map(MAP_FWD) && jvae_gemm_map_unfold(g, xb, (unsigned)g.N, &mx);
         const int want = fwd_slices(g);
         if (want > 1) {
             const long colf = (long)col_floats_per_image(g) * g.N, outf = (long)g.N * g.Cs * Ps;
             if (ws_bytes < 4 * (size_t)(colf + want * outf)) return JVAE_EWORKSPACE;
             float* part = ws + colf;
             int S = 0;
-            int rc = jvae_gemm_launch_part(g.N, g.Cs, Kd, Ps, ws, Kd, 1, (long)g.N * Kd, w, 1, Kd, 0,
+            int rc = JVAE_ENOTSUP;
+            if (mapped) {
+                JvaeGemmDesc d = dense_desc(g.N, g.Cs, Kd, Ps, ws, Kd, 1, (long)g.N * Kd, w, 1, Kd, 0, part, g.Cs, 1, (long)g.N * g.Cs);
+                d.want_splits = want; d.sCsplit = outf; d.splits = &S;
+                rc = jvae_gemm_launch_mapped(d, &mx, nullptr, st);
+            }
+            if (rc == JVAE_ENOTSUP) {
+                rc = launch_unfold(xb, ws, g, 0, g.N, true, st);
+                if (rc) return rc;
+                rc = jvae_gemm_launch_part(g.N, g.Cs, Kd, Ps, ws, Kd, 1, (long)g.N * Kd, w, 1, Kd, 0,
                                            part, g.Cs, 1, (long)g.N * g.Cs, outf, want, &S, st);
+            }
             if (rc) return rc;
             return jvae_splitk_fold_qn(part, bias, ys, S, g.N, g.Cs, Ps, st);
         }
+        if (mapped) {
+            JvaeGemmDesc d = dense_desc(g.N, g.Cs, Kd, Ps, ws, Kd, 1, (long)g.N * Kd, w, 1, Kd, 0, ys, (long)g.Cs * Ps, Ps, 1);
+            d.bias = bias; d.bias_mode = bias ? 1 : 0;
+            const int rc = jvae_gemm_launch_mapped(d, &mx, nullptr, st);
+            if (rc != JVAE_ENOTSUP) return rc;
+        }
+        { const int rc = launch_unfold(xb, ws, g, 0, g.N, true, st); if (rc) return rc; }
         return jvae_gemm_launch(g.N, g.Cs, Kd, Ps, ws, Kd, 1, (long)g.N * Kd, w, 1, Kd, 0,
                                 ys, (long)g.Cs * Ps, Ps, 1, bias, bias ? 1 : 0, 0, 1, st);
     }
@@ -259,10 +329,17 @@
         int rc;
         if (Ps > 1 && ws_bytes >= 4 * (size_t)(colf + ytf)) {
             float* yt = ws + colf;
-            hipLaunchKernelGGL(small_transpose_kernel, dim3(grid_for(ytf)), dim3(256), 0, st, ys, yt, g.N, g.Cs, Ps);
-            JVAE_LAUNCH_CHECK();
-            rc = jvae_gemm_launch(g.N, Kd, g.Cs, Ps, yt, g.Cs, 1, (long)g.N * g.Cs, w, Kd, 1, 0,
-                                  ws, Kd, 1, (long)g.N * Kd, nullptr, 0, 0, 1, st);
+            GemmOperandMap my;
+            rc = JVAE_ENOTSUP;
+            if (use_map(MAP_DGRAD) && jvae_gemm_map_rows(g, ys, (unsigned)g.N, &my))
+                rc = jvae_gemm_launch_mapped(dense_desc(g.N, Kd, g.Cs, Ps, yt, g.Cs, 1, (long)g.N * g.Cs, w, Kd, 1, 0,
+                                                        ws, Kd, 1, (long)g.N * Kd), &my, nullptr, st);
+            if (rc == JVAE_ENOTSUP) {
+                hipLaunchKernelGGL(small_transpose_kernel, dim3(grid_for(ytf)), dim3(256), 0, st, ys, yt, g.N, g.Cs, Ps);
+                JVAE_LAUNCH_CHECK();
+                rc = jvae_gemm_launch(g.N, Kd, g.Cs, Ps, yt, g.Cs, 1, (long)g.N * g.Cs, w, Kd, 1, 0,
+                                      ws, Kd, 1, (long)g.N * Kd, nullptr, 0, 0, 1, st);
+            }
         } else {
             rc = jvae_gemm_launch(g.N, Kd, g.Cs, Ps, ys, (long)g.Cs * Ps, Ps, 1, w, Kd, 1, 0,
                                   ws, Kd, 1, (long)g.N * Kd, nullptr, 0, 0, 1, st);
@@ -300,21 +377,30 @@
     const int Kd = g.Cb * g.KH * g.KW, Ps = g.Hs * g.Ws;
     if (pixel_batched(g)) {
         if (ws_bytes < (size_t)col_floats_per_image(g) * 4 * g.N) return JVAE_EWORKSPACE;
-        { const int rc = launch_unfold(xb, ws, g, 0, g.N, true, st); if (rc) return rc; }
         if (wgrad_joint(g)) {
             const int S = wgrad_slices(g);
             const long colf = (long)col_floats_per_image(g) * g.N, ytf = (long)g.N * g.Cs * Ps;
             if (ws_bytes < 4 * (size_t)(colf + ytf + (long)S * g.Cs * Kd)) return JVAE_EWORKSPACE;
             float* yt = ws + colf;
             float* part = yt + ytf;
-            hipLaunchKernelGGL(small_transpose_kernel, dim3(grid_for(ytf)), dim3(256), 0, st, ys, yt, g.N, g.Cs, Ps);
-            JVAE_LAUNCH_CHECK();
             const long Ks = (long)Ps * g.N / S;
-            int rc = jvae_gemm_launch(g.Cs, Kd, (int)Ks, S, yt, 1, g.Cs, Ks * g.Cs, ws, Kd, 1, Ks * Kd,
+            GemmOperandMap my, mx;
+            int rc = JVAE_ENOTSUP;
+            if (use_map(MAP_WGRAD) && jvae_gemm_map_rows(g, ys, (unsigned)Ks, &my) && jvae_gemm_map_unfold(g, xb, (unsigned)Ks, &mx))
+                rc = jvae_gemm_launch_mapped(dense_desc(g.Cs, Kd, (int)Ks, S, yt, 1, g.Cs, Ks * g.Cs, ws, Kd, 1, Ks * Kd,
+                                                        part, Kd, 1, (long)g.Cs * Kd), &my, &mx, st);
+            if (rc == JVAE_ENOTSUP) {
+                rc = launch_unfold(xb, ws, g, 0, g.N, true, st);
+                if (rc) return rc;
+                hipLaunchKernelGGL(small_transpose_kernel, dim3(grid_for(ytf)), dim3(256), 0, st, ys, yt, g.N, g.Cs, Ps);
+                JVAE_LAUNCH_CHECK();
+                rc = jvae_gemm_launch(g.Cs, Kd, (int)Ks, S, yt, 1, g.Cs, Ks * g.Cs, ws, Kd, 1, Ks * Kd,
                                       part, Kd, 1, (long)g.Cs * Kd, nullptr, 0, 0, 1, st);
+            }
             if (rc) return rc;
             return jvae_splitk_fold(part, nullptr, dw, S, (long)g.Cs * Kd, Kd, 0, 1, st);
         }
+        { const int rc = launch_unfold(xb, ws, g, 0, g.N, true, st); if (rc) return rc; }
         for (int q = 0; q < Ps; ++q) {
             int rc = jvae_gemm_launch(g.Cs, Kd, g.N, 1, ys + q, Ps, (long)g.Cs * Ps, 0, ws + (long)q * g.N * Kd, Kd, 1, 0,
                                       dw, Kd, 1, 0, nullptr, 0, 1, 1, st);
@@ -348,7 +434,24 @@
     return 0;
 }
 
+int jvae_conv_generic_set_implicit(int on) {
+    const int old = g_implicit;
+    g_implicit = (on == 0 || on == 2) ? on : 1;
+    return old;
+}
+
 size_t jvae_channel_sum_ws_bytes(int C) { return sizeof(float) * (size_t)(C > 0 ? C : 1) * 64; }
+
+static int channel_sum_splits(int N, int C, int P) {
+    long work = (long)N * P;
+    int ns = (int)(work / 4096);
+    const int cap = (1024 + C - 1) / C;
+    if (ns > cap) ns = cap;
+    if (ns > 64) ns = 64;
+    if (ns > N) ns = N;
+    if (ns < 1) ns = 1;
+    return ns;
+}
 
 int jvae_channel_sum(const float* t, float* out, int N, int C, int P, int accumulate, float* ws, size_t ws_bytes,
                      hipStream_t st) {
@@ -361,16 +464,45 @@
         return 0;
     }
     if (!ws || ws_bytes < jvae_channel_sum_ws_bytes(C)) return JVAE_EWORKSPACE;
-    long work = (long)N * P;
-    int ns = (int)(work / 4096);
-    const int cap = (1024 + C - 1) / C;
-    if (ns > cap) ns = cap;
-    if (ns > 64) ns = 64;
-    if (ns > N) ns = N;
-    if (ns < 1) ns = 1;
+    const int ns = channel_sum_splits(N, C, P);
     hipLaunchKernelGGL(channel_sum_kernel, dim3(C, ns), dim3(256), 0, st, t, ws, N, C, P, ns);
     JVAE_LAUNCH_CHECK();
     hipLaunchKernelGGL(channel_fold_kernel, dim3(cdiv(C, 64)), dim3(64), 0, st, (const float*)ws, out, C, ns, accumulate);
     JVAE_LAUNCH_CHECK();
     return 0;
 }
+
+int jvae_channel_sum_group(const JvaeChanSumDesc* descs, int n, float* ws, size_t ws_bytes, hipStream_t st) {
+    size_t need = 0;
+    bool plain = n < 2;
+    for (int i = 0; i < n; ++i) {
+        need += jvae_channel_sum_ws_bytes(descs[i].C);
+        plain = plain || descs[i].N <= 0;
+        for (int j = 0; j < i; ++j)
+            if (descs[i].out < descs[j].out + descs[j].C && descs[j].out < descs[i].out + descs[i].C) return JVAE_EINVAL;
+    }
+    if (!ws || ws_bytes < need) return JVAE_EWORKSPACE;
+    ChanSumGroup g;
+    unsigned total = 0, ftotal = 0;
+    float* part = ws;
+    for (int i = 0; i < n; ++i) {
+        const JvaeChanSumDesc& d = descs[i];
+        const size_t bytes = jvae_channel_sum_ws_bytes(d.C);
+        if (plain) {
+            if (int rc = jvae_channel_sum(d.t, d.out, d.N, d.C, d.P, d.accumulate, part, bytes, st)) return rc;
+        } else {
+            const int ns = channel_sum_splits(d.N, d.C, d.P);
+            g.rec[i] = ChanSumRec{d.t, part, d.out, d.N, d.C, d.P, ns, d.accumulate, total, ftotal};
+            total += (unsigned)d.C * ns;
+            ftotal += (unsigned)cdiv(d.C, 64);
+        }
+        part += bytes / sizeof(float);
+    }
+    if (plain) return 0;
+    for (int i = n; i < CS_GROUP_MAX; ++i) { g.rec[i] = g.rec[0]; g.rec[i].first = g.rec[i].ffirst = 0xffffffffu; }
+    hipLaunchKernelGGL(channel_sum_group_kernel, dim3(total), dim3(256), 0, st, g);
+    JVAE_LAUNCH_CHECK();
+    hipLaunchKernelGGL(channel_fold_group_kernel, dim3(ftotal), dim3(64), 0, st, g);
+    JVAE_LAUNCH_CHECK();
+    return 0;
+}
diff --git a/joint-vae_amd/csrc/gemm.hip b/joint-vae_amd/csrc/gemm.hip
--- a/joint-vae_amd/csrc/gemm.hip
+++ b/joint-vae_amd/csrc/gemm.hip
@@ -81,6 +81,45 @@
     return vec ? load4<true>(src, sR, row, rows, k < kend) : load4<false>(src, sR, row, rows, k < kend);
 }
 
+__device__ float map_zero[4] = {0.f, 0.f, 0.f, 0.f};
+
+template <int KIND>
+__device__ __forceinline__ f32x4 map_load4(const GemmOperandMap& m, unsigned batch, int rloc, int rlim, int c0, int clim) {
+    const bool rok = rloc < rlim;
+    const unsigned r = rok ? batch * m.rpb + (unsigned)rloc : 0u;
+    const unsigned q = m.nimg.div(r), n = r - q * m.nimg.d;
+    const float* img = m.src + n * m.img;
+    f32x4 v;
+    if (KIND == GEMM_MAP_ROWS) {
+#pragma unroll
+        for (int e = 0; e < 4; ++e) {
+            const bool ok = rok && c0 + e < clim;
+            v[e] = *(ok ? img + ((unsigned)(c0 + e) * m.Ps + q) : map_zero);
+        }
+    } else {
+        const unsigned hs = m.ws.div(q), ws = q - hs * m.ws.d;
+        unsigned cb = m.kk.div((unsigned)c0);
+        const unsigned t = (unsigned)c0 - cb * m.kk.d;
+        unsigned kh = m.kw.div(t), kw = t - kh * m.kw.d;
+        const int h0 = (int)(hs * m.S) - m.P, w0 = (int)(ws * m.S) - m.P;
+#pragma unroll
+        for (int e = 0; e < 4; ++e) {
+            const int hb = h0 + (int)kh, wb = w0 + (int)kw;
+            const bool ok = rok && c0 + e < clim && (unsigned)hb < (unsigned)m.Hb && (unsigned)wb < (unsigned)m.Wb;
+            v[e] = *(ok ? img + (((int)cb * m.Hb + hb) * m.Wb + wb) : map_zero);
+            if (++kw == m.kw.d) { kw = 0; if (++kh == m.KH) { kh = 0; ++cb; } }
+        }
+    }
+    return v;
+}
+
+template <int KIND, bool KC, int ROWS>
+__device__ __forceinline__ f32x4 map_stage(const GemmOperandMap& m, unsigned batch, int rows, int tid, int g, int r0, int k0, int kend) {
+    const StageMap<KC, ROWS> s(tid, g);
+    const int row = s.row(r0), k = s.k(k0);
+    return KC ? map_load4<KIND>(m, batch, row, rows, k, kend) : map_load4<KIND>(m, batch, k, kend, row, rows);
+}
+
 template <int BM, int BN>
 struct TileLds {
     static constexpr int LDA = BM + 4, LDB = BN + 4;
@@ -98,9 +137,10 @@
     }
 }
 
-template <int BM, int BN, bool AK, bool BNC>
+template <int BM, int BN, bool AK, bool BNC, int MA = GEMM_MAP_NONE, int MB = GEMM_MAP_NONE>
 __device__ __forceinline__ void gemm_tile_body(const GemmP& p, float* __restrict__ lds, unsigned bx, unsigned by, unsigned bz,
-                                               unsigned gx, unsigned gy, unsigned gz) {
+                                               unsigned gx, unsigned gy, unsigned gz, const GemmOperandMap* ma = nullptr,
+                                               const GemmOperandMap* mb = nullptr) {
     constexpr int LDA = TileLds<BM, BN>::LDA, LDB = TileLds<BM, BN>::LDB;
     constexpr int WM = BM / 2, WN = BN / 2;
     constexpr int TM = WM / 32, TN = WN / 32;
@@ -127,9 +167,15 @@
 
     auto gload = [&](int k0) {
 #pragma unroll
-        for (int g = 0; g < GA; ++g) ra[g] = stage_load<AK, BM, false>(A, p.sAm, p.sAk, p.M, p.vecA, tid, g, m0, k0, kend);
-#pragma unroll
-        for (int g = 0; g < GB; ++g) rb[g] = stage_load<!BNC, BN, true>(B, p.sBn, p.sBk, p.N, p.vecB, tid, g, n0, k0, kend);
+        for (int g = 0; g < GA; ++g) {
+            if constexpr (MA != GEMM_MAP_NONE) ra[g] = map_stage<MA, AK, BM>(*ma, t.batch, p.M, tid, g, m0, k0, kend);
+            else ra[g] = stage_load<AK, BM, false>(A, p.sAm, p.sAk, p.M, p.vecA, tid, g, m0, k0, kend);
+        }
+#pragma unroll
+        for (int g = 0; g < GB; ++g) {
+            if constexpr (MB != GEMM_MAP_NONE) rb[g] = map_stage<MB, !BNC, BN>(*mb, t.batch, p.N, tid, g, n0, k0, kend);
+            else rb[g] = stage_load<!BNC, BN, true>(B, p.sBn, p.sBk, p.N, p.vecB, tid, g, n0, k0, kend);
+        }
     };
     auto lstore = [&]() {
 #pragma unroll
@@ -185,6 +231,12 @@
     gemm_tile_body<BM, BN, AK, BNC>(p, lds, blockIdx.x, blockIdx.y, blockIdx.z, gridDim.x, gridDim.y, gridDim.z);
 }
 
+template <int BM, int BN, bool AK, bool BNC, int MA, int MB>
+__global__ __launch_bounds__(256) void gemm_map_kernel(GemmP p, GemmOperandMap ma, GemmOperandMap mb) {
+    __shared__ float lds[TileLds<BM, BN>::BYTES / sizeof(float)];
+    gemm_tile_body<BM, BN, AK, BNC, MA, MB>(p, lds, blockIdx.x, blockIdx.y, blockIdx.z, gridDim.x, gridDim.y, gridDim.z, &ma, &mb);
+}
+
 inline bool aligned16(const void* p) { return (reinterpret_cast<uintptr_t>(p) & 15) == 0; }
 
 typedef __bf16 gx_bf16x8 __attribute__((ext_vector_type(8)));
@@ -208,9 +260,10 @@
     static constexpr int BYTES = PITCH * ROWS;
 };
 
-template <bool AK, bool BNC, int DEPTH>
+template <bool AK, bool BNC, int DEPTH, int MA = GEMM_MAP_NONE, int MB = GEMM_MAP_NONE>
 __device__ __forceinline__ void gemm_x3_body(const GemmP& p, unsigned char* __restrict__ gx_lds, unsigned bx, unsigned by, unsigned bz,
-                                             unsigned gx, unsigned gy, unsigned gz) {
+                                             unsigned gx, unsigned gy, unsigned gz, const GemmOperandMap* ma = nullptr,
+                                             const GemmOperandMap* mb = nullptr) {
     using IA = GxImg<AK>;
     using IB = GxImg<!BNC>;
     constexpr int BM = 64, BN = 64, G4 = StageMap<AK, BM>::G;
@@ -252,15 +305,25 @@
             if constexpr (DEPTH > 1) {
                 int f, sl;
                 coordA(g, k0, &f, &sl);
-                const float* sa = AK ? A + (long)sl * p.sAm + f : A + (long)sl * p.sAk + f;
-                ra[st][g] = *reinterpret_cast<const f32x4*>(okA(f, sl) ? sa : A);
+                if constexpr (MA != GEMM_MAP_NONE) {
+                    ra[st][g] = AK ? map_load4<MA>(*ma, t.batch, sl, p.M, f, kend) : map_load4<MA>(*ma, t.batch, sl, kend, f, p.M);
+                } else {
+                    const float* sa = AK ? A + (long)sl * p.sAm + f : A + (long)sl * p.sAk + f;
+                    ra[st][g] = *reinterpret_cast<const f32x4*>(okA(f, sl) ? sa : A);
+                }
                 coordB(g, k0, &f, &sl);
-                const float* sb = BNC ? B + (long)sl * p.sBk + f : B + (long)sl * p.sBn + f;
-                rb[st][g] = *reinterpret_cast<const f32x4*>(okB(f, sl) ? sb : B);
+                if constexpr (MB != GEMM_MAP_NONE) {
+                    rb[st][g] = BNC ? map_load4<MB>(*mb, t.batch, sl, kend, f, p.N) : map_load4<MB>(*mb, t.batch, sl, p.N, f, kend);
+                } else {
+                    const float* sb = BNC ? B + (long)sl * p.sBk + f : B + (long)sl * p.sBn + f;
+                    rb[st][g] = *reinterpret_cast<const f32x4*>(okB(f, sl) ? sb : B);
+                }
                 continue;
             }
-            ra[st][g] = stage_load<AK, BM, false>(A, p.sAm, p.sAk, p.M, p.vecA, tid, g, m0, k0, kend);
-            rb[st][g] = stage_load<!BNC, BN, true>(B, p.sBn, p.sBk, p.N, p.vecB, tid, g, n0, k0, kend);
+            if constexpr (MA != GEMM_MAP_NONE) ra[st][g] = map_stage<MA, AK, BM>(*ma, t.batch, p.M, tid, g, m0, k0, kend);
+            else ra[st][g] = stage_load<AK, BM, false>(A, p.sAm, p.sAk, p.M, p.vecA, tid, g, m0, k0, kend);
+            if constexpr (MB != GEMM_MAP_NONE) rb[st][g] = map_stage<MB, !BNC, BN>(*mb, t.batch, p.N, tid, g, n0, k0, kend);
+            else rb[st][g] = stage_load<!BNC, BN, true>(B, p.sBn, p.sBk, p.N, p.vecB, tid, g, n0, k0, kend);
         }
     };
     auto lstore = [&](int st, int k0) {
@@ -272,9 +335,9 @@
             if constexpr (DEPTH > 1) {
                 int f, sl;
                 coordA(g, k0, &f, &sl);
-                if (!okA(f, sl)) va = f32x4{0.f, 0.f, 0.f, 0.f};
+                if (MA == GEMM_MAP_NONE && !okA(f, sl)) va = f32x4{0.f, 0.f, 0.f, 0.f};
                 coordB(g, k0, &f, &sl);
-                if (!okB(f, sl)) vb = f32x4{0.f, 0.f, 0.f, 0.f};
+                if (MB == GEMM_MAP_NONE && !okB(f, sl)) vb = f32x4{0.f, 0.f, 0.f, 0.f};
             }
             gx_u32x2 sa[3], sb[3];
             gx_split4(va, sa);
@@ -364,6 +427,12 @@
 __global__ __launch_bounds__(256, 4) void gemm_x3_kernel(GemmP p) {
     extern __shared__ __attribute__((aligned(16))) unsigned char gx_lds[];
     gemm_x3_body<AK, BNC, DEPTH>(p, gx_lds, blockIdx.x, blockIdx.y, blockIdx.z, gridDim.x, gridDim.y, gridDim.z);
+}
+
+template <bool AK, bool BNC, int DEPTH, int MA, int MB>
+__global__ __launch_bounds__(256, 4) void gemm_x3_map_kernel(GemmP p, GemmOperandMap ma, GemmOperandMap mb) {
+    extern __shared__ __attribute__((aligned(16))) unsigned char gx_lds[];
+    gemm_x3_body<AK, BNC, DEPTH, MA, MB>(p, gx_lds, blockIdx.x, blockIdx.y, blockIdx.z, gridDim.x, gridDim.y, gridDim.z, &ma, &mb);
 }
 
 inline bool gemm_x3_on(int K) {
@@ -492,6 +561,31 @@
     return rc;
 }
 
+template <bool AK, bool BNC, int MA, int MB>
+int launch_mapped_as(const GemmPlan& pl, const GemmOperandMap& ma, const GemmOperandMap& mb, hipStream_t st) {
+    const Variant& d = VARIANTS[pl.variant];
+    const dim3 grid(pl.gx, pl.gy, pl.gz);
+    if (d.x3) {
+        auto run = [&](auto kernel, bool* attr_set) {
+            if (int rc = set_lds_once(kernel, pl.lds, attr_set)) return rc;
+            hipLaunchKernelGGL(kernel, grid, dim3(256), pl.lds, st, pl.p, ma, mb);
+            return 0;
+        };
+        static bool set1 = false, set3 = false;
+        const int rc = d.depth == 3 ? run(&gemm_x3_map_kernel<AK, BNC, 3, MA, MB>, &set3) : run(&gemm_x3_map_kernel<AK, BNC, 1, MA, MB>, &set1);
+        if (rc) return rc;
+    } else if (d.bm == 128) {
+        hipLaunchKernelGGL((gemm_map_kernel<128, 128, AK, BNC, MA, MB>), grid, dim3(256), 0, st, pl.p, ma, mb);
+    } else {
+        hipLaunchKernelGGL((gemm_map_kernel<64, 64, AK, BNC, MA, MB>), grid, dim3(256), 0, st, pl.p, ma, mb);
+    }
+    JVAE_LAUNCH_CHECK();
+    return 0;
+}
+
+inline MapDiv map_div(unsigned d) { return MapDiv{d, d > 1 ? (unsigned)(((1ul << 32) + d - 1) / d) : 0u}; }
+inline bool div_ok(unsigned long xmax, unsigned d) { return xmax * d < (1ul << 32); }
+
 constexpr int GROUP_MAX = 8;
 struct GemmRec {
     GemmP p;
@@ -644,6 +738,42 @@
     return launch_plan(pl, st);
 }
 
+}
+
+bool jvae_gemm_map_unfold(const ConvGeom& g, const float* xb, unsigned rpb, GemmOperandMap* m) {
+    const unsigned long Ps = (unsigned long)g.Hs * g.Ws, KK = (unsigned long)g.KH * g.KW, Kd = KK * g.Cb;
+    const unsigned long img = (unsigned long)g.Cb * g.Hb * g.Wb;
+    if (g.N < 1 || img * g.N >= (1ul << 31) || Ps * g.N >= (1ul << 31) || Kd >= (1ul << 30)) return false;
+    if (!div_ok(Ps * g.N, g.N) || !div_ok(Ps, g.Ws) || !div_ok(Kd + 4096, (unsigned)KK) || !div_ok(KK, g.KW)) return false;
+    *m = GemmOperandMap{xb, GEMM_MAP_UNFOLD, rpb, map_div(g.N), map_div(g.Ws), map_div((unsigned)KK), map_div(g.KW), (unsigned)g.KH,
+                        g.S, g.P, g.Hb, g.Wb, (unsigned)img, 0u};
+    return true;
+}
+
+bool jvae_gemm_map_rows(const ConvGeom& g, const float* ys, unsigned rpb, GemmOperandMap* m) {
+    const unsigned long Ps = (unsigned long)g.Hs * g.Ws, img = Ps * g.Cs;
+    if (g.N < 1 || img * g.N >= (1ul << 31) || !div_ok(Ps * g.N, g.N)) return false;
+    *m = GemmOperandMap{ys, GEMM_MAP_ROWS, rpb, map_div(g.N), MapDiv{1, 0}, MapDiv{1, 0}, MapDiv{1, 0}, 1u, 1, 0, 1, 1,
+                        (unsigned)img, (unsigned)Ps};
+    return true;
+}
+
+int jvae_gemm_launch_mapped(const JvaeGemmDesc& d, const GemmOperandMap* ma, const GemmOperandMap* mb, hipStream_t st) {
+    if (d.splits) *d.splits = 0;
+    GemmPlan pl;
+    const int rc = gemm_plan(d, 1, &pl);
+    if (rc < 0) return rc;
+    const GemmOperandMap none = {};
+    const int ka = ma ? ma->kind : GEMM_MAP_NONE, kb = mb ? mb->kind : GEMM_MAP_NONE;
+    const bool ak = d.sAk == 1, bnc = d.sBn == 1;
+    const int form = (ka == GEMM_MAP_UNFOLD && !kb && ak && !bnc) ? 0 : (ka == GEMM_MAP_ROWS && !kb && ak && bnc) ? 1
+                   : (ka == GEMM_MAP_ROWS && kb == GEMM_MAP_UNFOLD && !ak && bnc) ? 2 : -1;
+    if (form < 0) return JVAE_ENOTSUP;
+    if (rc) return 0;
+    if (d.splits) *d.splits = pl.p.splitk;
+    if (form == 0) return launch_mapped_as<true, false, GEMM_MAP_UNFOLD, GEMM_MAP_NONE>(pl, *ma, none, st);
+    if (form == 1) return launch_mapped_as<true, true, GEMM_MAP_ROWS, GEMM_MAP_NONE>(pl, *ma, none, st);
+    return launch_mapped_as<false, true, GEMM_MAP_ROWS, GEMM_MAP_UNFOLD>(pl, *ma, *mb, st);
 }
 
 int jvae_gemm_launch(int M, int N, int K, int batch,
diff --git a/joint-vae_amd/csrc/jvae_internal.h b/joint-vae_amd/csrc/jvae_internal.h
--- a/joint-vae_amd/csrc/jvae_internal.h
+++ b/joint-vae_amd/csrc/jvae_internal.h
@@ -24,6 +24,35 @@
                           const float* B, long sBk, long sBn, long sBb,
                           float* part, long sCm, long sCn, long sCb, long sCsplit, int want_splits, int* splits,
                           hipStream_t st);
+
+enum { GEMM_MAP_NONE = 0, GEMM_MAP_UNFOLD = 1, GEMM_MAP_ROWS = 2 };
+struct MapDiv {
+    unsigned d, m;
+    __host__ __device__ __forceinline__ unsigned div(unsigned x) const {
+#if defined(__HIP_DEVICE_COMPILE__)
+        return d == 1 ? x : __umulhi(x, m);
+#else
+        return x / d;
+#endif
+    }
+};
+struct GemmOperandMap {
+    const float* src;
+    int kind;
+    unsigned rpb;
+    MapDiv nimg;
+    MapDiv ws, kk, kw;
+    unsigned KH;
+    int S, P, Hb, Wb;
+    unsigned img;
+    unsigned Ps;
+};
+struct ConvGeom;
+bool jvae_gemm_map_unfold(const ConvGeom& g, const float* xb, unsigned rpb, GemmOperandMap* m);
+bool jvae_gemm_map_rows(const ConvGeom& g, const float* ys, unsigned rpb, GemmOperandMap* m);
+
+struct JvaeGemmDesc;
+int jvae_gemm_launch_mapped(const JvaeGemmDesc& d, const GemmOperandMap* ma, const GemmOperandMap* mb, hipStream_t st);
 
 struct InAff { const float* sc; const float* sh; int relu; };
 
diff --git a/joint-vae_amd/jvae_hip/lib.py b/joint-vae_amd/jvae_hip/lib.py
--- a/joint-vae_amd/jvae_hip/lib.py
+++ b/joint-vae_amd/jvae_hip/lib.py
@@ -24,6 +24,10 @@
 class FoldDesc(ctypes.Structure):
     _fields_ = [('part', P), ('bias', P), ('y', P), ('S', c_int), ('MN', c_long), ('N', c_int), ('relu', c_int),
                 ('accumulate', c_int)]
+
+
+class ChanSumDesc(ctypes.Structure):
+    _fields_ = [('t', P), ('out', P), ('N', c_int), ('C', c_int), ('P', c_int), ('accumulate', c_int)]
 
 
 class GemmRoute(ctypes.Structure):
@@ -41,6 +45,7 @@
     'jvae_conv2d_workspace_bytes': (c_size_t, [c_int] * 11),
     'jvae_conv2d_set_split_bf16': (c_int, [c_int]),
     'jvae_conv2d_set_split_shape16': (c_int, [c_int]),
+    'jvae_conv2d_set_implicit_unfold': (c_int, [c_int]),
     'jvae_conv2d_out_shape': (c_int, [c_int] * 8 + [POINTER(c_int), POINTER(c_int)]),
     'jvae_conv2d_route': (c_int, [c_int] * 17 + [POINTER(c_int), POINTER(c_int), POINTER(c_size_t), POINTER(c_int), POINTER(c_int)]),
     'jvae_conv2d_kernel_name': (c_char_p, [c_int]),
@@ -83,6 +88,7 @@
     'jvae_pack_cache_stats': (c_int, [POINTER(c_int), POINTER(c_longlong), POINTER(c_longlong), POINTER(c_longlong)]),
     'jvae_channel_sum_workspace_bytes': (c_size_t, [c_int]),
     'jvae_channel_sum_f32': (c_int, [P, P, c_int, c_int, c_int, c_int, P, c_size_t, P]),
+    'jvae_channel_sum_group_f32': (c_int, [POINTER(ChanSumDesc), c_int, P, c_size_t, P]),
     'jvae_bn_workspace_bytes': (c_size_t, [c_int]),
     'jvae_bn_plan': (c_int, [c_int, c_int, c_int, POINTER(c_int), POINTER(c_int)]),
     'jvae_image_range': (c_int, [c_int, c_int, c_int, POINTER(c_int), POINTER(c_int)]),
diff --git a/joint-vae_amd/jvae_hip/ops.py b/joint-vae_amd/jvae_hip/ops.py
--- a/joint-vae_amd/jvae_hip/ops.py
+++ b/joint-vae_amd/jvae_hip/ops.py
@@ -119,6 +119,17 @@
     L.check(lib.jvae_channel_sum_f32(L.ptr(t), L.ptr(out), N, C, P, int(accumulate), L.ptr(ws), ws.numel(), L.stream_ptr()),
             'channel_sum')
     return out
+
+
+def channel_sum_group(items):
+    lib = L.load()
+    outs = [out if out is not None else torch.empty(C, device=t.device, dtype=torch.float32) for t, N, C, P, out, acc in items]
+    ws = L.workspace(sum(lib.jvae_channel_sum_workspace_bytes(it[2]) for it in items), items[0][0].device)
+    descs = (L.ChanSumDesc * len(items))()
+    for d, (t, N, C, P, _, acc), out in zip(descs, items, outs):
+        d.t, d.out, d.N, d.C, d.P, d.accumulate = L.ptr(t), L.ptr(out), N, C, P, int(acc)
+    L.check(lib.jvae_channel_sum_group_f32(descs, len(items), L.ptr(ws), ws.numel(), L.stream_ptr()), 'channel_sum_group')
+    return outs
 
 
 def _linear_split(R, O, I):
@@ -259,10 +270,18 @@
             out += [gw, None]
             gys.append(gy)
         _run_products(descs, folds)
+        sums = []
         for h, gy in enumerate(gys):
             b_ref = ctx.refs[h][1]
             if gy is not None and b_ref is not None and ctx.needs_input_grad[2 + 2 * h]:
-                out[1 + 2 * h] = _linear_bias_grad(gy, b_ref)
+                slot = _grad_slot(b_ref)
+                sums.append((h, slot, (gy, R, gy.shape[1], 1, slot, slot is not None)))
+        if len(sums) == 2 and (sums[0][1] is None or sums[0][1] is not sums[1][1]):
+            for (h, slot, _), o in zip(sums, channel_sum_group([s[2] for s in sums])):
+                out[1 + 2 * h] = None if slot is not None else o
+        else:
+            for h, _, _ in sums:
+                out[1 + 2 * h] = _linear_bias_grad(gys[h], ctx.refs[h][1])
         gx = None
         if gxs:
             gx = (gxs[0] if len(gxs) == 1 else torch.add(gxs[0], gxs[1])).reshape(ctx.xshape)
```

Result: no change. 141,100 (-0.2%).
